# sina-behnam/RTSDS

Measured on AMD Instinct MI355X. Metric: images/sec/node (train step) + inference FPS@1024x512, BiSeNet 19-cls, higher is better.
Workload: dtype bf16; 1 GPU; configs[1]: BiSeNet-R18 seg-only train step (train.py:65-113); model=BiSeNet-ResNet18, global_batch=8, per_gpu_batch=8, image=3x512x1024, num_classes=19, parallelism=dp1

## Files before the change

include/rtsds_hip.h:

```cpp
#ifndef RTSDS_HIP_H
#define RTSDS_HIP_H
#include <stddef.h>
#include <stdint.h>
#ifdef __cplusplus
extern "C" {
#endif

enum { RTSDS_F32 = 0, RTSDS_BF16 = 1, RTSDS_F16 = 2  };
enum {
  RTSDS_OK = 0,
  RTSDS_ERR_SHAPE = 1,
  RTSDS_ERR_UNSUPPORTED = 2,
  RTSDS_ERR_LAUNCH = 3,
  RTSDS_ERR_WORKSPACE = 4
};
enum { RTSDS_ACT_NONE = 0, RTSDS_ACT_RELU = 1, RTSDS_ACT_LEAKY = 2, RTSDS_ACT_SIGMOID = 3 };
#define RTSDS_ACCUMULATE 0x100
#define RTSDS_INPUT_PADDED 0x400
#define RTSDS_WEIGHT_PACKED 0x800

typedef struct {
  int n, h, w, c;
  int ho, wo, k;
  int kh, kw;
  int sh, sw;
  int ph, pw;
  int dh, dw;
  int dtype;
} rtsds_conv_desc;


size_t rtsds_conv2d_fwd_workspace(const rtsds_conv_desc* d);
int rtsds_conv2d_input_pitch(const rtsds_conv_desc* d);
int rtsds_conv2d_fwd_stats_tiles(const rtsds_conv_desc* d);
int rtsds_conv2d_fwd(const rtsds_conv_desc* d, const void* x, const void* w, const float* bias,
                     void* y, int act, float* bn_stats, void* ws, size_t ws_bytes, void* stream);
int rtsds_conv2d_fwd_bn(const rtsds_conv_desc* d, const void* x, const void* w, const float* scale,
                        const float* shift, const void* res, void* y, int act, void* ws, size_t ws_bytes,
                        void* stream);
int rtsds_conv2d_fwd_bn_ld(const rtsds_conv_desc* d, const void* x, const void* w, const float* scale,
                           const float* shift, void* y, long ldy, int act, void* ws, size_t ws_bytes, void* stream);
int rtsds_conv2d_fwd_bn_maxpool(const rtsds_conv_desc* d, const void* x, const void* w, const float* scale,
                                const float* shift, void* y, int act, int hp, int wp, int pool_pad, void* ws,
                                size_t ws_bytes, void* stream);
size_t rtsds_conv2d_dgrad_workspace(const rtsds_conv_desc* d);
size_t rtsds_conv2d_dgrad_pack_bytes(const rtsds_conv_desc* d);
int rtsds_conv2d_dgrad_pack_many(int count, const rtsds_conv_desc* descs, const void* const* w, void* const* wt,
                                 void* stream);
int rtsds_conv2d_dgrad(const rtsds_conv_desc* d, const void* dy, const void* w, void* dx,
                       int accumulate, void* ws, size_t ws_bytes, void* stream);
int rtsds_conv2d_dgrad_act(const rtsds_conv_desc* d, const void* dy, const void* w, void* dx, const void* x_act,
                           int act, void* ws, size_t ws_bytes, void* stream);
int rtsds_conv2d_dgrad_bnstats_tiles(const rtsds_conv_desc* d);
int rtsds_conv2d_dgrad_bnstats(const rtsds_conv_desc* d, const void* dy, const void* w, void* dx, const void* bn_x,
                               const float* gamma, const float* beta, const float* save_mean, const float* save_invstd,
                               int act, float* part, void* ws, size_t ws_bytes, void* stream);
size_t rtsds_conv2d_wgrad_workspace(const rtsds_conv_desc* d);
int rtsds_conv2d_wgrad(const rtsds_conv_desc* d, const void* x, const void* dy, float* dw,
                       float* dbias, int accumulate, void* ws, size_t ws_bytes, void* stream);
typedef struct {
  const float* slab;
  float* dw;
  long slab_stride;
  int nv;
  int cv, cp;
  int splits, accumulate;
} rtsds_split_reduce_desc;
int rtsds_conv2d_wgrad_deferred(const rtsds_conv_desc* d, const void* x, const void* dy, float* dw,
                                float* dbias, int accumulate, void* ws, size_t ws_bytes,
                                rtsds_split_reduce_desc* pending, void* stream);
int rtsds_split_reduce_many(int n, const rtsds_split_reduce_desc* descs, void* stream);
size_t rtsds_imgconv_bn_wgrad_workspace(const rtsds_conv_desc* d);
int rtsds_imgconv_bn_wgrad(const rtsds_conv_desc* d, const void* x, const void* bn_dy, const void* bn_x,
                           const float* coef, int act, float* dw, int accumulate, void* ws, size_t ws_bytes,
                           void* stream);
int rtsds_imgconv_bn_wgrad_deferred(const rtsds_conv_desc* d, const void* x, const void* bn_dy, const void* bn_x,
                                    const float* coef, int act, float* dw, int accumulate, void* ws,
                                    size_t ws_bytes, rtsds_split_reduce_desc* pending, void* stream);

size_t rtsds_bn_workspace(long rows, int c);
int rtsds_bn_fwd(const void* x, const void* res, void* y, long rows, int c, const float* gamma,
                 const float* beta, float* running_mean, float* running_var,
                 long long* num_batches_tracked, float* save_mean,
                 float* save_invstd, float momentum, float eps, int training, int act,
                 const float* stats_part, int stats_nrb, int dtype, void* ws, size_t ws_bytes,
                 void* stream);
int rtsds_bn_fwd_ld(const void* x, const void* res, void* y, long ldy, long rows, int c,
                    const float* gamma, const float* beta, float* running_mean, float* running_var,
                    long long* num_batches_tracked, float* save_mean, float* save_invstd,
                    float momentum, float eps, int training, int act, const float* stats_part,
                    int stats_nrb, int dtype, void* ws, size_t ws_bytes, void* stream);
int rtsds_bn_fold(const float* gamma, const float* beta, const float* running_mean,
                  const float* running_var, const float* conv_bias, float eps, int c, float* scale,
                  float* shift, void* stream);
int rtsds_bn_bwd(const void* dy, const void* x, const void* y, void* dx, void* dres,
                 float* dgamma, float* dbeta, long rows, int c, const float* gamma,
                 const float* beta, const float* save_mean, const float* save_invstd, int training, int act,
                 int accumulate_params, int dtype, void* ws, size_t ws_bytes, void* stream);
int rtsds_bn_bwd_ld(const void* dy, long ldy, const void* x, const void* y, void* dx, void* dres,
                    float* dgamma, float* dbeta, long rows, int c, const float* gamma,
                    const float* beta, const float* save_mean, const float* save_invstd, int training,
                    int act, int accumulate_params, int dtype, void* ws, size_t ws_bytes, void* stream);
int rtsds_bn_bwd_coef(const void* dy, const void* x, float* dgamma, float* dbeta, float* coef, long rows, int c,
                      const float* gamma, const float* beta, const float* save_mean, const float* save_invstd,
                      int training, int act, int accumulate_params, int dtype, void* ws, size_t ws_bytes,
                      void* stream);
int rtsds_bn_bwd_part(const void* dy, const void* x, void* dx, float* dgamma, float* dbeta, long rows, int c,
                      const float* gamma, const float* beta, const float* save_mean, const float* save_invstd,
                      int training, int act, int accumulate_params, const float* part, int nrb, int dtype, void* ws,
                      size_t ws_bytes, void* stream);

int rtsds_bn_relu_maxpool_fwd(const void* x, void* y, uint8_t* idx, int n, int h, int w, int c, int ho, int wo,
                              int p, const float* gamma, const float* beta, float* running_mean,
                              float* running_var, long long* num_batches_tracked, float* save_mean,
                              float* save_invstd, float momentum, float eps, int training,
                              const float* stats_part, int stats_nrb, int dtype, void* ws, size_t ws_bytes,
                              void* stream);
int rtsds_bn_relu_maxpool_bwd(const void* dy_pool, const uint8_t* idx, const void* x, void* dx, float* dgamma,
                              float* dbeta, int n, int h, int w, int c, int ho, int wo, int p,
                              const float* gamma, const float* beta, const float* save_mean,
                              const float* save_invstd, int training, int accumulate_params, int dtype,
                              void* ws, size_t ws_bytes, void* stream);

int rtsds_nchw_to_nhwc(const float* x, void* y, int n, int c, int h, int w, int dtype, void* stream);
int rtsds_nchw_to_nhwc_pad(const float* x, void* y, int n, int c, int h, int w, int pitch, int dtype, void* stream);
int rtsds_cast(const void* src, int src_dtype, void* dst, int dst_dtype, long n, void* stream);
int rtsds_copy_channels(const void* src, int src_ld, int src_off, void* dst, int dst_ld, int dst_off,
                        long rows, int cnt, int accumulate, int dtype, void* stream);

int rtsds_act_fwd(const void* x, void* y, long n, int act, int dtype, void* stream);
int rtsds_act_bwd(const void* dy, const void* y, void* dx, long n, int act, float alpha, int dtype,
                  void* stream);

int rtsds_maxpool_fwd(const void* x, void* y, uint8_t* idx, int n, int h, int w, int c, int ho,
                      int wo, int k, int s, int p, int dtype, void* stream);
int rtsds_maxpool_bwd(const void* dy, const uint8_t* idx, void* dx, int n, int h, int w, int c,
                      int ho, int wo, int k, int s, int p, int dtype, void* stream);
size_t rtsds_gap_workspace(int n, long hw, int c);
int rtsds_gap_fwd(const void* x, void* y, int n, long hw, int c, int dtype, void* ws, size_t ws_bytes,
                  void* stream);
int rtsds_gap_bwd(const void* dy, void* dx, int n, long hw, int c, int accumulate, int dtype, void* stream);

size_t rtsds_ffm_head_eval_workspace(int n, long hw, int c);
int rtsds_ffm_head_eval(const void* f, const void* w1, const float* b1, const void* w2, const float* b2,
                        const void* w3, const float* b3, void* out, int n, long hw, int c, int dtype, void* ws,
                        size_t ws_bytes, void* stream);
int rtsds_chscale_fwd(const void* x, const void* a, void* y, int n, long hw, int c, int mode,
                      int dtype, void* stream);
int rtsds_chscale_bwd(const void* dy, const void* x, const void* a, void* dx, void* da, int n,
                      long hw, int c, int mode, int dtype, void* ws, size_t ws_bytes, void* stream);
int rtsds_chscale2_fwd(const void* x, const void* a, const void* b, void* y, int n, long hw, int c,
                       int dtype, void* stream);
int rtsds_chscale2_bwd(const void* dy, const void* x, const void* a, const void* b, void* dx, void* da,
                       void* db, int n, long hw, int c, int dtype, void* ws, size_t ws_bytes, void* stream);

int rtsds_bilinear_fwd(const void* x, void* y, int n, int hi, int wi, int c, int ho, int wo,
                       float scale_h, float scale_w, int y_ld, int y_off, int dtype, void* stream);
int rtsds_bilinear_fwd_scaled(const void* x, const void* s1, const void* s2, void* y, int n, int hi, int wi,
                              int c, int ho, int wo, float scale_h, float scale_w, int y_ld, int y_off,
                              int dtype, void* stream);
size_t rtsds_bilinear_bwd_workspace(int n, int hi, int wi, int c, int ho, int wo);
int rtsds_bilinear_bwd(const void* dy, void* dx, int n, int hi, int wi, int c, int ho, int wo,
                       float scale_h, float scale_w, int dy_ld, int dy_off, int dtype, void* ws,
                       size_t ws_bytes, void* stream);

int rtsds_adaptive_avgpool_fwd(const void* x, void* y, int n, int hi, int wi, int c, int ho, int wo,
                               int dtype, void* stream);
int rtsds_adaptive_avgpool_bwd(const void* dy, void* dx, int n, int hi, int wi, int c, int ho, int wo,
                               int dtype, void* stream);

int rtsds_softmax_fwd(const void* x, long sn, long sc, long shw, void* y, int y_ld, int n, long hw,
                      int c, int dtype, void* stream);
int rtsds_softmax_bwd(const void* dy, const void* y, int ld, void* dx, long sn, long sc, long shw,
                      int n, long hw, int c, int dtype, void* stream);
size_t rtsds_ce_workspace(void);
int rtsds_ce_finish(const void* ws, float* loss, void* stream);
int rtsds_ce_fwd(const void* x, long sn, long sc, long shw, const int64_t* target, float* loss, int n,
                 long hw, int c, int ignore_index, int dtype, void* ws, size_t ws_bytes, void* stream);
int rtsds_ce_bwd(const void* x, long sn, long sc, long shw, const int64_t* target,
                 const float* grad_loss, const float* count, void* dx, int n, long hw, int c,
                 int ignore_index, int dtype, void* stream);
int rtsds_bce_fwd(const float* x, const float* target, float* loss, int n, void* stream);
int rtsds_bce_bwd(const float* x, const float* target, const float* grad_loss, float* dx, int n,
                  void* stream);

int rtsds_adam_step(float* param, const void* grad, float* exp_avg, float* exp_avg_sq,
                    void* bf16_shadow, long n, float lr, float beta1, float beta2, float eps,
                    float weight_decay, int step, float grad_scale, int grad_dtype, void* stream);

int rtsds_adam_step_dev(float* param, const void* grad, float* exp_avg, float* exp_avg_sq,
                        void* bf16_shadow, long n, const float* hyper, float beta1, float beta2,
                        float eps, float weight_decay, float grad_scale, int grad_dtype, void* stream);

int rtsds_sgd_step(float* param, const void* grad, float* momentum_buf, void* bf16_shadow,
                   long n, const float* hyper, float lr, float momentum, float dampening,
                   float weight_decay, int nesterov, int first, float grad_scale, int grad_dtype, void* stream);

int rtsds_ema_step(float* teacher, const float* student, void* teacher_bf16_shadow, long n, float w,
                   void* stream);
int rtsds_ema_many(int count, float* const* teacher, const float* const* student, const long* numel,
                   float w, void* stream);

int rtsds_argmax(const void* x, long sn, long sc, long shw, int64_t* out, const int64_t* target,
                 unsigned long long* correct, int n, long hw, int c, int dtype, void* stream);
int rtsds_confusion(const int64_t* label, const int64_t* pred, unsigned long long* hist, long total,
                    int nc, void* stream);

#define RTSDS_UPCE_SET_CORRECT 2
size_t rtsds_upce_workspace(int nheads, int n, int hl, int wl, int c, int H, int W, float scale_h,
                            float scale_w);
int rtsds_upce_fwd(int nheads, const void* const* logits, const int64_t* target, int n, int hl,
                   int wl, int c, int H, int W, float scale_h, float scale_w, int ignore_index,
                   float* loss, float* loss_sum, unsigned long long* correct, int want_grad,
                   int dtype, void* ws, size_t ws_bytes, void* stream);
int rtsds_upce_finish(int nheads, const void* ws, float* loss, float* loss_sum, void* stream);
int rtsds_upce_bwd(int nheads, const float* grad_loss, int grad_stride, void* const* dlogits,
                   int n, int hl, int wl, int c, int H, int W, float scale_h, float scale_w,
                   int dtype, const void* ws, size_t ws_bytes, void* stream);

int rtsds_upsoftmax_fwd(const void* x, void* y, int n, int hi, int wi, int c, int ho, int wo,
                        float scale_h, float scale_w, int y_ld, int dtype, void* stream);
size_t rtsds_upsoftmax_bwd_workspace(int n, int hi, int wi, int c, int ho, int wo);
int rtsds_upsoftmax_bwd(const void* dy, int dy_ld, const void* y, int y_ld, void* dx, int n, int hi,
                        int wi, int c, int ho, int wo, float scale_h, float scale_w, int dtype,
                        void* ws, size_t ws_bytes, void* stream);

int rtsds_upsoftmax_acc(const void* x, float* acc, int64_t* pred, int n, int hi, int wi, int c,
                        int ho, int wo, float scale_h, float scale_w, int flip, int accumulate,
                        int dtype, void* stream);

int rtsds_conf_hist(const float* acc, unsigned long long* hist, uint8_t* pred, uint16_t* cbin,
                    long total, int c, int bins, float inv, void* stream);
int rtsds_pseudo_select(const uint8_t* pred, const uint16_t* cbin, const int* tbin, int64_t* out,
                        long total, int c, int ignore_index, void* stream);

int rtsds_upsample_pseudo(const void* x, uint8_t* pred, uint16_t* cbin, const int* tbin, int64_t* labels,
                          int n, int hi, int wi, int c, int ho, int wo, float scale_h, float scale_w,
                          int bins, int ignore_index, int dtype, void* stream);

int rtsds_upsample_paint(const void* x, const uint8_t* frame, const uint8_t* palette, const uint8_t* lut,
                         uint8_t* ids, uint8_t* rgb, int n, int hi, int wi, int c, int ho, int wo,
                         float scale_h, float scale_w, int alpha_q8, int dtype, void* stream);

int rtsds_slide_paint(const void* x, const int* win, int nwin, const uint8_t* frame,
                      const uint8_t* palette, const uint8_t* lut, float* acc, uint8_t* ids,
                      uint8_t* rgb, int nf, int hi, int wi, int c, int hw, int ww, int H, int W,
                      float scale_h, float scale_w, int accumulate, int alpha_q8, int dtype,
                      void* stream);

int rtsds_class_presence(const int64_t* slab, const int* origins, int origin_pitch, unsigned int* present,
                         int n, int hs, int ws, int h, int w, int c, void* stream);
int rtsds_classmix(const void* src, const int64_t* slab, const void* tgt, const uint8_t* pred,
                   const uint16_t* cbin, const int* tbin, const unsigned int* present, const int* perm,
                   int perm_pitch, const int* origins, int origin_pitch, void* out_img, int64_t* out_lab,
                   uint8_t* mask, unsigned int* chosen, int n, int hs, int ws, int h, int w, int c,
                   int pix_bytes, int ignore_index, void* stream);

size_t rtsds_resize_aa_workspace(int c, int h, int w, int ho, int wo);
int rtsds_resize_aa(const void* src, int src_u8, int c, int h, int w, void* dst, int kind, int ho, int wo,
                    int flip, const float* mean, const float* std, int clamp_lo, int clamp_hi, void* ws,
                    size_t ws_bytes, void* stream);
int rtsds_crop_resize_aa(const void* src, int src_u8, int c, int h, int w, int y0, int x0, int hc, int wc,
                         void* dst, int kind, int ho, int wo, int flip, const float* mean, const float* std,
                         int clamp_lo, int clamp_hi, void* ws, size_t ws_bytes, void* stream);
int rtsds_crop_resize_nearest(const void* src, int src_i64, int h, int w, int y0, int x0, int hc, int wc,
                              int64_t* dst, int ho, int wo, int flip, int clamp_lo, int clamp_hi, void* stream);
int rtsds_gaussian_blur(const void* src, int src_u8, float* dst, int c, int h, int w, int kx, int ky,
                        float sigma_x, float sigma_y, void* stream);
int rtsds_gta5_decode(const uint8_t* rgb, int64_t* out, int h, int w, void* stream);
size_t rtsds_color_jitter_workspace(int h, int w);
int rtsds_color_jitter(const void* src, int src_u8, float* dst, int c, int h, int w, const int* order,
                       int mask, float fb, float fc, float fs, float fh, float bound, void* ws,
                       size_t ws_bytes, void* stream);

int rtsds_hist_u8(const uint8_t* img, int c, int h, int w, unsigned int* hist, void* stream);
int rtsds_hist_match(const uint8_t* src, uint8_t* dst, int c, int h, int w, const unsigned int* hist_src,
                     const unsigned int* hist_ref, int strength_q8, uint8_t* lut_out, void* stream);

size_t rtsds_fda_workspace(int h, int w, int b);
int rtsds_fda_spectrum(const uint8_t* img, int c, int h, int w, int b, float* spec, float* amp_norm, void* ws,
                       size_t ws_bytes, void* stream);
int rtsds_fda_apply(const uint8_t* src, void* dst, int dst_u8, int c, int h, int w, int b, const float* spec_src,
                    const float* amp_ref_norm, float strength, void* stream);

int rtsds_graph_split(void* graph, int max_lanes, void** handle, int* n_segments, int* n_lanes);
int rtsds_graph_lanes(void* graph, int max_lanes);
int rtsds_graph_nodes(void* graph);
int rtsds_capture_nodes(void* stream);
int rtsds_graph_split_launch(void* handle, void* stream);
int rtsds_graph_split_destroy(void* handle);

int rtsds_pooled_mlp_bwd(const void* da, const void* a, const void* h, const void* p, const void* w1,
                         const void* w2, float* dw1, float* db1, float* dw2, float* db2, void* dp,
                         int n, int c0, int c1, int c2, int accumulate, int dtype, void* stream);

int rtsds_pooled_mlp_fwd(const void* p, const void* w1, const float* b1, const void* w2, const float* b2, void* h,
                         void* a, int n, int c0, int c1, int c2, int dtype, void* stream);

int rtsds_bn_fwd_gap(const void* x, void* y, float* gap_part, int n, long hw, int c, const float* gamma, const float* beta,
                     float* running_mean, float* running_var, long long* num_batches_tracked, float* save_mean,
                     float* save_invstd, float momentum, float eps, int act, const float* stats_part, int stats_nrb,
                     int dtype, void* ws, size_t ws_bytes, void* stream);
int rtsds_ffm_att_scale(const float* part, const void* f, const void* w1, const float* b1, const void* w2, const float* b2,
                        void* pooled, void* hid, void* att, void* r, int ldr, int n, long hw, int c, int dtype,
                        void* stream);
int rtsds_ffm_att_bwd(const void* dr, const void* f, const void* a, const void* h, const void* p, const void* w1,
                      const void* w2, float* dw1, float* db1, float* dw2, float* db2, void* dp, int n, long hw, int c,
                      int accumulate, int dtype, void* ws, size_t ws_bytes, void* stream);
int rtsds_bn_bwd_ffm(const void* dr, const void* att, const void* dpooled, int n, long hw, const void* x, void* dx,
                     float* dgamma, float* dbeta, int c, const float* gamma, const float* beta, const float* save_mean,
                     const float* save_invstd, int training, int act, int accumulate_params, int dtype, void* ws,
                     size_t ws_bytes, void* stream);

#define RTSDS_ABI_VERSION 23
int rtsds_abi_version(void);

#ifdef __cplusplus
}
#endif
#endif
```

rtsds_amd/_lib.py:

```python
import ctypes
import os

import torch

_HERE = os.path.dirname(os.path.abspath(__file__))
DEFAULT_LIB_PATH = os.path.join(_HERE, "librtsds_hip.so")
ABI_VERSION = 23
LIB_PATH = os.environ.get("RTSDS_LIB") or DEFAULT_LIB_PATH

F32, BF16 = 0, 1
ACT_NONE, ACT_RELU, ACT_LEAKY, ACT_SIGMOID = 0, 1, 2, 3
ACCUMULATE = 0x100
INPUT_PADDED = 0x400
WEIGHT_PACKED = 0x800
UPCE_SET_CORRECT = 2
ERRORS = {1: "bad shape", 2: "unsupported configuration", 3: "HIP launch failure", 4: "workspace too small"}

c_int, c_long, c_float, c_size_t, c_void_p = (ctypes.c_int, ctypes.c_long, ctypes.c_float,
                                              ctypes.c_size_t, ctypes.c_void_p)


class ConvDesc(ctypes.Structure):
    _fields_ = [(n, c_int) for n in ("n", "h", "w", "c", "ho", "wo", "k", "kh", "kw", "sh", "sw",
                                     "ph", "pw", "dh", "dw", "dtype")]


class SplitReduceDesc(ctypes.Structure):
    _fields_ = [("slab", c_void_p), ("dw", c_void_p), ("slab_stride", c_long), ("nv", c_int), ("cv", c_int),
                ("cp", c_int), ("splits", c_int), ("accumulate", c_int)]


P = c_void_p
SIGNATURES = {
    "rtsds_conv2d_fwd_workspace": (c_size_t, [ctypes.POINTER(ConvDesc)]),
    "rtsds_conv2d_input_pitch": (c_int, [ctypes.POINTER(ConvDesc)]),
    "rtsds_conv2d_fwd_stats_tiles": (c_int, [ctypes.POINTER(ConvDesc)]),
    "rtsds_conv2d_fwd": (c_int, [ctypes.POINTER(ConvDesc), P, P, P, P, c_int, P, P, c_size_t, P]),
    "rtsds_conv2d_fwd_bn": (c_int, [ctypes.POINTER(ConvDesc), P, P, P, P, P, P, c_int, P, c_size_t, P]),
    "rtsds_conv2d_fwd_bn_ld": (c_int, [ctypes.POINTER(ConvDesc), P, P, P, P, P, c_long, c_int, P, c_size_t, P]),
    "rtsds_conv2d_fwd_bn_maxpool": (c_int, [ctypes.POINTER(ConvDesc), P, P, P, P, P, c_int, c_int, c_int, c_int, P,
                                            c_size_t, P]),
    "rtsds_conv2d_dgrad_workspace": (c_size_t, [ctypes.POINTER(ConvDesc)]),
    "rtsds_conv2d_dgrad_pack_bytes": (c_size_t, [ctypes.POINTER(ConvDesc)]),
    "rtsds_conv2d_dgrad_pack_many": (c_int, [c_int, ctypes.POINTER(ConvDesc), P, P, P]),
    "rtsds_conv2d_dgrad": (c_int, [ctypes.POINTER(ConvDesc), P, P, P, c_int, P, c_size_t, P]),
    "rtsds_conv2d_dgrad_act": (c_int, [ctypes.POINTER(ConvDesc), P, P, P, P, c_int, P, c_size_t, P]),
    "rtsds_conv2d_dgrad_bnstats_tiles": (c_int, [ctypes.POINTER(ConvDesc)]),
    "rtsds_conv2d_dgrad_bnstats": (c_int, [ctypes.POINTER(ConvDesc), P, P, P, P, P, P, P, P, c_int, P, P, c_size_t, P]),
    "rtsds_conv2d_wgrad_workspace": (c_size_t, [ctypes.POINTER(ConvDesc)]),
    "rtsds_conv2d_wgrad": (c_int, [ctypes.POINTER(ConvDesc), P, P, P, P, c_int, P, c_size_t, P]),
    "rtsds_conv2d_wgrad_deferred": (c_int, [ctypes.POINTER(ConvDesc), P, P, P, P, c_int, P, c_size_t,
                                            ctypes.POINTER(SplitReduceDesc), P]),
    "rtsds_split_reduce_many": (c_int, [c_int, ctypes.POINTER(SplitReduceDesc), P]),
    "rtsds_imgconv_bn_wgrad_workspace": (c_size_t, [ctypes.POINTER(ConvDesc)]),
    "rtsds_imgconv_bn_wgrad": (c_int, [ctypes.POINTER(ConvDesc), P, P, P, P, c_int, P, c_int, P, c_size_t, P]),
    "rtsds_imgconv_bn_wgrad_deferred": (c_int, [ctypes.POINTER(ConvDesc), P, P, P, P, c_int, P, c_int, P, c_size_t,
                                                ctypes.POINTER(SplitReduceDesc), P]),
    "rtsds_bn_workspace": (c_size_t, [c_long, c_int]),
    "rtsds_bn_bwd_coef": (c_int, [P, P, P, P, P, c_long, c_int, P, P, P, P, c_int, c_int, c_int, c_int, P, c_size_t, P]),
    "rtsds_bn_fwd": (c_int, [P, P, P, c_long, c_int, P, P, P, P, P, P, P, c_float, c_float, c_int,
                             c_int, P, c_int, c_int, P, c_size_t, P]),
    "rtsds_bn_fwd_ld": (c_int, [P, P, P, c_long, c_long, c_int, P, P, P, P, P, P, P, c_float, c_float, c_int,
                                c_int, P, c_int, c_int, P, c_size_t, P]),
    "rtsds_bn_fold": (c_int, [P, P, P, P, P, c_float, c_int, P, P, P]),
    "rtsds_pooled_mlp_fwd": (c_int, [P, P, P, P, P, P, P, c_int, c_int, c_int, c_int, c_int, P]),
    "rtsds_pooled_mlp_bwd": (c_int, [P, P, P, P, P, P, P, P, P, P, P, c_int, c_int, c_int, c_int, c_int, c_int, P]),
    "rtsds_bn_fwd_gap": (c_int, [P, P, P, c_int, c_long, c_int, P, P, P, P, P, P, P, c_float, c_float, c_int, P, c_int,
                                 c_int, P, c_size_t, P]),
    "rtsds_ffm_att_scale": (c_int, [P] * 10 + [c_int, c_int, c_long, c_int, c_int, P]),
    "rtsds_ffm_att_bwd": (c_int, [P] * 12 + [c_int, c_long, c_int, c_int, c_int, P, c_size_t, P]),
    "rtsds_bn_bwd_ffm": (c_int, [P, P, P, c_int, c_long, P, P, P, P, c_int, P, P, P, P, c_int, c_int, c_int, c_int,
                                 P, c_size_t, P]),
    "rtsds_bn_bwd_part": (c_int, [P, P, P, P, P, c_long, c_int, P, P, P, P, c_int, c_int, c_int, P, c_int, c_int, P,
                                  c_size_t, P]),
    "rtsds_bn_bwd": (c_int, [P, P, P, P, P, P, P, c_long, c_int, P, P, P, P, c_int, c_int, c_int, c_int,
                             P, c_size_t, P]),
    "rtsds_bn_bwd_ld": (c_int, [P, c_long, P, P, P, P, P, P, c_long, c_int, P, P, P, P, c_int, c_int, c_int, c_int,
                                P, c_size_t, P]),
    "rtsds_bn_relu_maxpool_fwd": (c_int, [P, P, P] + [c_int] * 7 + [P, P, P, P, P, P, P, c_float, c_float, c_int, P,
                                                                   c_int, c_int, P, c_size_t, P]),
    "rtsds_bn_relu_maxpool_bwd": (c_int, [P, P, P, P, P, P] + [c_int] * 7 + [P, P, P, P, c_int, c_int, c_int, P,
                                                                            c_size_t, P]),
    "rtsds_nchw_to_nhwc": (c_int, [P, P, c_int, c_int, c_int, c_int, c_int, P]),
    "rtsds_nchw_to_nhwc_pad": (c_int, [P, P, c_int, c_int, c_int, c_int, c_int, c_int, P]),
    "rtsds_cast": (c_int, [P, c_int, P, c_int, c_long, P]),
    "rtsds_ffm_head_eval_workspace": (c_size_t, [c_int, c_long, c_int]),
    "rtsds_ffm_head_eval": (c_int, [P, P, P, P, P, P, P, P, c_int, c_long, c_int, c_int, P, c_size_t, P]),
    "rtsds_graph_split": (c_int, [P, c_int, P, P, P]),
    "rtsds_graph_split_launch": (c_int, [P, P]),
    "rtsds_graph_lanes": (c_int, [P, c_int]),
    "rtsds_graph_nodes": (c_int, [P]),
    "rtsds_abi_version": (c_int, []),
    "rtsds_capture_nodes": (c_int, [P]),
    "rtsds_graph_split_destroy": (c_int, [P]),
    "rtsds_copy_channels": (c_int, [P, c_int, c_int, P, c_int, c_int, c_long, c_int, c_int, c_int, P]),
    "rtsds_act_fwd": (c_int, [P, P, c_long, c_int, c_int, P]),
    "rtsds_act_bwd": (c_int, [P, P, P, c_long, c_int, c_float, c_int, P]),
    "rtsds_maxpool_fwd": (c_int, [P, P, P] + [c_int] * 10 + [P]),
    "rtsds_maxpool_bwd": (c_int, [P, P, P] + [c_int] * 10 + [P]),
    "rtsds_gap_workspace": (c_size_t, [c_int, c_long, c_int]),
    "rtsds_gap_fwd": (c_int, [P, P, c_int, c_long, c_int, c_int, P, c_size_t, P]),
    "rtsds_gap_bwd": (c_int, [P, P, c_int, c_long, c_int, c_int, c_int, P]),
    "rtsds_chscale_fwd": (c_int, [P, P, P, c_int, c_long, c_int, c_int, c_int, P]),
    "rtsds_chscale_bwd": (c_int, [P, P, P, P, P, c_int, c_long, c_int, c_int, c_int, P, c_size_t, P]),
    "rtsds_chscale2_fwd": (c_int, [P, P, P, P, c_int, c_long, c_int, c_int, P]),
    "rtsds_chscale2_bwd": (c_int, [P, P, P, P, P, P, P, c_int, c_long, c_int, c_int, P, c_size_t, P]),
    "rtsds_bilinear_fwd": (c_int, [P, P] + [c_int] * 6 + [c_float, c_float, c_int, c_int, c_int, P]),
    "rtsds_bilinear_fwd_scaled": (c_int, [P, P, P, P] + [c_int] * 6 + [c_float, c_float, c_int, c_int, c_int, P]),
    "rtsds_bilinear_bwd_workspace": (c_size_t, [c_int] * 6),
    "rtsds_bilinear_bwd": (c_int, [P, P] + [c_int] * 6 + [c_float, c_float, c_int, c_int, c_int, P, c_size_t, P]),
    "rtsds_softmax_fwd": (c_int, [P, c_long, c_long, c_long, P, c_int, c_int, c_long, c_int, c_int, P]),
    "rtsds_softmax_bwd": (c_int, [P, P, c_int, P, c_long, c_long, c_long, c_int, c_long, c_int, c_int,
                                  P]),
    "rtsds_ce_workspace": (c_size_t, []),
    "rtsds_ce_fwd": (c_int, [P, c_long, c_long, c_long, P, P, c_int, c_long, c_int, c_int, c_int, P,
                             c_size_t, P]),
    "rtsds_ce_bwd": (c_int, [P, c_long, c_long, c_long, P, P, P, P, c_int, c_long, c_int, c_int, c_int,
                             P]),
    "rtsds_bce_fwd": (c_int, [P, P, P, c_int, P]),
    "rtsds_bce_bwd": (c_int, [P, P, P, P, c_int, P]),
    "rtsds_adam_step_dev": (c_int, [P, P, P, P, P, c_long, P, c_float, c_float, c_float, c_float, c_float, c_int, P]),
    "rtsds_upsoftmax_fwd": (c_int, [P, P, c_int, c_int, c_int, c_int, c_int, c_int, c_float, c_float, c_int, c_int, P]),
    "rtsds_upsoftmax_bwd_workspace": (c_size_t, [c_int, c_int, c_int, c_int, c_int, c_int]),
    "rtsds_upsoftmax_bwd": (c_int, [P, c_int, P, c_int, P, c_int, c_int, c_int, c_int, c_int, c_int, c_float, c_float,
                                    c_int, P, c_size_t, P]),
    "rtsds_upsoftmax_acc": (c_int, [P, P, P, c_int, c_int, c_int, c_int, c_int, c_int, c_float, c_float, c_int, c_int,
                                    c_int, P]),
    "rtsds_conf_hist": (c_int, [P, P, P, P, c_long, c_int, c_int, c_float, P]),
    "rtsds_pseudo_select": (c_int, [P, P, P, P, c_long, c_int, c_int, P]),
    "rtsds_upsample_pseudo": (c_int, [P, P, P, P, P] + [c_int] * 6 + [c_float, c_float, c_int, c_int, c_int, P]),
    "rtsds_upsample_paint": (c_int, [P, P, P, P, P, P] + [c_int] * 6 + [c_float, c_float, c_int, c_int, P]),
    "rtsds_slide_paint": (c_int, [P, ctypes.POINTER(c_int), c_int, P, P, P, P, P, P] + [c_int] * 8 +
                          [c_float, c_float, c_int, c_int, c_int, P]),
    "rtsds_ema_step": (c_int, [P, P, P, c_long, c_float, P]),
    "rtsds_ema_many": (c_int, [c_int, P, P, P, c_float, P]),
    "rtsds_class_presence": (c_int, [P, P, c_int, P, c_int, c_int, c_int, c_int, c_int, c_int, P]),
    "rtsds_classmix": (c_int, [P, P, P, P, P, P, P, P, c_int, P, c_int, P, P, P, P] + [c_int] * 8 + [P]),
    "rtsds_resize_aa_workspace": (c_size_t, [c_int, c_int, c_int, c_int, c_int]),
    "rtsds_resize_aa": (c_int, [P, c_int, c_int, c_int, c_int, P, c_int, c_int, c_int, c_int, P, P, c_int, c_int,
                                P, c_size_t, P]),
    "rtsds_crop_resize_aa": (c_int, [P] + [c_int] * 8 + [P, c_int, c_int, c_int, c_int, P, P, c_int, c_int,
                                     P, c_size_t, P]),
    "rtsds_crop_resize_nearest": (c_int, [P] + [c_int] * 7 + [P, c_int, c_int, c_int, c_int, c_int, P]),
    "rtsds_gaussian_blur": (c_int, [P, c_int, P, c_int, c_int, c_int, c_int, c_int, c_float, c_float, P]),
    "rtsds_gta5_decode": (c_int, [P, P, c_int, c_int, P]),
    "rtsds_color_jitter_workspace": (c_size_t, [c_int, c_int]),
    "rtsds_color_jitter": (c_int, [P, c_int, P, c_int, c_int, c_int, ctypes.POINTER(c_int), c_int, c_float, c_float,
                                   c_float, c_float, c_float, P, c_size_t, P]),
    "rtsds_hist_u8": (c_int, [P, c_int, c_int, c_int, P, P]),
    "rtsds_hist_match": (c_int, [P, P, c_int, c_int, c_int, P, P, c_int, P, P]),
    "rtsds_fda_workspace": (c_size_t, [c_int, c_int, c_int]),
    "rtsds_fda_spectrum": (c_int, [P, c_int, c_int, c_int, c_int, P, P, P, c_size_t, P]),
    "rtsds_fda_apply": (c_int, [P, P, c_int, c_int, c_int, c_int, c_int, P, P, c_float, P]),
    "rtsds_sgd_step": (c_int, [P, P, P, P, c_long, P, c_float, c_float, c_float, c_float, c_int, c_int,
                               c_float, c_int, P]),
    "rtsds_adam_step": (c_int, [P, P, P, P, P, c_long, c_float, c_float, c_float, c_float, c_float,
                                c_int, c_float, c_int, P]),
    "rtsds_argmax": (c_int, [P, c_long, c_long, c_long, P, P, P, c_int, c_long, c_int, c_int, P]),
    "rtsds_confusion": (c_int, [P, P, P, c_long, c_int, P]),
    "rtsds_adaptive_avgpool_fwd": (c_int, [P, P, c_int, c_int, c_int, c_int, c_int, c_int, c_int, P]),
    "rtsds_adaptive_avgpool_bwd": (c_int, [P, P, c_int, c_int, c_int, c_int, c_int, c_int, c_int, P]),
    "rtsds_upce_finish": (c_int, [c_int, P, P, P, P]),
    "rtsds_ce_finish": (c_int, [P, P, P]),
    "rtsds_upce_workspace": (c_size_t, [c_int, c_int, c_int, c_int, c_int, c_int, c_int, c_float, c_float]),
    "rtsds_upce_fwd": (c_int, [c_int, P, P, c_int, c_int, c_int, c_int, c_int, c_int, c_float, c_float,
                               c_int, P, P, P, c_int, c_int, P, c_size_t, P]),
    "rtsds_upce_bwd": (c_int, [c_int, P, c_int, P, c_int, c_int, c_int, c_int, c_int, c_int, c_float, c_float,
                               c_int, P, c_size_t, P]),
}

_lib = None


def load(path=LIB_PATH):
    global _lib
    if _lib is None:
        if not os.path.exists(path):
            raise RuntimeError(f"rtsds_amd: HIP library not built ({path}); run __graft_entry__.build()")
        lib = ctypes.CDLL(path)
        ver = getattr(lib, "rtsds_abi_version", None)
        if ver is None:
            raise RuntimeError(f"rtsds_amd: {path} predates the ABI version check; rebuild it")
        ver.restype, ver.argtypes = ctypes.c_int, []
        if ver() != ABI_VERSION:
            raise RuntimeError(f"rtsds_amd: {path} has ABI revision {ver()}, this package needs {ABI_VERSION}")
        for name, (res, args) in SIGNATURES.items():
            fn = getattr(lib, name)
            fn.restype, fn.argtypes = res, args
        _lib = lib
    return _lib


class _Lib:
    def __getattr__(self, name):
        fn = getattr(load(), name)

        def call(*args):
            rc = fn(*args)
            if name.endswith(("_workspace", "_tiles", "_pitch", "_bytes")):
                return rc
            if rc != 0:
                raise RuntimeError(f"rtsds_amd: {name} failed: {ERRORS.get(rc, rc)}")
            return rc
        return call


lib = _Lib()
```

rtsds_amd/csrc/bn.hip:

```cpp
#include "bn_dev.h"
#include "chan_dev.h"
#include <type_traits>
#include <algorithm>

static const int kBnMaxRB = 2048;
static const int kBnTinyRows = 64;

template <int VEC> struct BnLayout {
  int tpr, rpi;
  __host__ __device__ BnLayout(int c) {
    tpr = (c + VEC - 1) / VEC;
    if (tpr > 256) tpr = 256;
    rpi = 256 / tpr;
  }
};
template <int VEC> struct BnTile : BnLayout<VEC> {
  int cl, cv, rg, ch0, cvalid;
  bool col, active;
  RT_DEV static int block_channels(int c) { return min(c - (int)blockIdx.y * 256 * VEC, 256 * VEC); }
  RT_DEV BnTile(int c) : BnLayout<VEC>(block_channels(c)) {
    cl = block_channels(c);
    cv = threadIdx.x % this->tpr;
    rg = threadIdx.x / this->tpr;
    ch0 = blockIdx.y * 256 * VEC + cv * VEC;
    cvalid = c - ch0;
    col = cv * VEC < cl;
    active = rg < this->rpi && col;
  }
  RT_DEV long row0() const { return (long)blockIdx.x * this->rpi + rg; }
  RT_DEV long step() const { return (long)gridDim.x * this->rpi; }
};

RT_DEV void bn_coef(float g, float b, float m, float inv, float& sc, float& sh) {
  sc = g * inv;
  sh = fmaf(-m, sc, b);
}

RT_DEV void chan_merge(float& na, float& ma, float& Ma, float nb, float mb, float Mb) {
  if (nb == 0.f) return;
  if (na == 0.f) { na = nb; ma = mb; Ma = Mb; return; }
  const float n = na + nb, d = mb - ma;
  ma += d * (nb / n);
  Ma += Mb + d * d * (na * nb / n);
  na = n;
}

template <typename T, int VEC>
__global__ void __launch_bounds__(256) bn_stats_kernel(const T* __restrict__ x, float* __restrict__ part, long rows, int c) {
  __shared__ float sh[3][256][VEC];
  const BnTile<VEC> t(c);
  const int tid = threadIdx.x, ch0 = t.ch0;
  float cnt = 0.f, shift[VEC], s1[VEC], s2[VEC];
#pragma unroll
  for (int j = 0; j < VEC; ++j) { shift[j] = 0.f; s1[j] = 0.f; s2[j] = 0.f; }
  if (t.active) {
    long r = t.row0();
    const long step = t.step();
    if (r < rows) {
      load_vec<T, VEC>(x + r * c + ch0, shift, t.cvalid);
      cnt = 1.f;
      r += step;
    }
    for (; r < rows; r += step) {
      float v[VEC];
      load_vec<T, VEC>(x + r * c + ch0, v, t.cvalid);
#pragma unroll
      for (int j = 0; j < VEC; ++j) {
        const float d = v[j] - shift[j];
        s1[j] += d;
        s2[j] = fmaf(d, d, s2[j]);
      }
      cnt += 1.f;
    }
  }
#pragma unroll
  for (int j = 0; j < VEC; ++j) {
    const float mean = cnt > 0.f ? shift[j] + s1[j] / cnt : 0.f;
    const float m2 = cnt > 0.f ? s2[j] - s1[j] * s1[j] / cnt : 0.f;
    sh[0][tid][j] = cnt;
    sh[1][tid][j] = mean;
    sh[2][tid][j] = fmaxf(m2, 0.f);
  }
  __syncthreads();
  if (t.rg == 0 && t.col) {
#pragma unroll
    for (int j = 0; j < VEC; ++j) {
      float n = sh[0][tid][j], m = sh[1][tid][j], M = sh[2][tid][j];
      for (int g = 1; g < t.rpi; ++g) {
        const int o = g * t.tpr + t.cv;
        chan_merge(n, m, M, sh[0][o][j], sh[1][o][j], sh[2][o][j]);
      }
      if (ch0 + j < c) {
        *(f32x4*)(part + ((long)(ch0 + j) * gridDim.x + blockIdx.x) * 4) = f32x4{n, m, M, 0.f};
      }
    }
  }
}


RT_DEV void chan_merge_shfl(float& n, float& m, float& M) {
#pragma unroll
  for (int o = 32; o > 0; o >>= 1) {
    const float nb = __shfl_xor(n, o, 64), mb = __shfl_xor(m, o, 64), Mb = __shfl_xor(M, o, 64);
    chan_merge(n, m, M, nb, mb, Mb);
  }
}
RT_DEV bool bn_finalize_body(const float* __restrict__ part, int nrb, int c, long rows, const float* gamma, const float* beta,
                             float* rmean, float* rvar, float* smean, float* sinv, float* scale, float* shift, float momentum,
                             float eps, long long* nbt, float (*wr)[3], float& sc_out, float& sh_out) {
  const int ch = blockIdx.x, lane = threadIdx.x & 63, wave = threadIdx.x >> 6;
  if (nbt && ch == 0 && threadIdx.x == 0) *nbt += 1;
  float g0 = 1.f, b0 = 0.f, rm0 = 0.f, rv0 = 0.f;
  if (threadIdx.x == 0) {
    if (gamma) g0 = gamma[ch];
    if (beta) b0 = beta[ch];
    if (rmean) rm0 = rmean[ch];
    if (rvar) rv0 = rvar[ch];
  }
  float n = 0.f, m = 0.f, M = 0.f;
  for (int b0 = threadIdx.x; b0 < nrb; b0 += 256 * 8) {
    float pn[8], pm[8], pM[8];
#pragma unroll
    for (int u = 0; u < 8; ++u) {
      const int b = min(b0 + 256 * u, nrb - 1);
      const f32x4 p = *(const f32x4*)(part + ((long)ch * nrb + b) * 4);
      pn[u] = b0 + 256 * u < nrb ? p[0] : 0.f;
      pm[u] = p[1];
      pM[u] = p[2];
    }
#pragma unroll
    for (int u = 0; u < 8; ++u) chan_merge(n, m, M, pn[u], pm[u], pM[u]);
  }
  chan_merge_shfl(n, m, M);
  if (lane == 0) { wr[wave][0] = n; wr[wave][1] = m; wr[wave][2] = M; }
  __syncthreads();
  if (threadIdx.x != 0) return false;
  n = wr[0][0]; m = wr[0][1]; M = wr[0][2];
  for (int w = 1; w < 4; ++w) chan_merge(n, m, M, wr[w][0], wr[w][1], wr[w][2]);
  const float var = M / (float)rows;
  const float inv = 1.0f / sqrtf(var + eps);
  smean[ch] = m;
  sinv[ch] = inv;
  if (rmean) rmean[ch] = (1.f - momentum) * rm0 + momentum * m;
  if (rvar) {
    const float unb = rows > 1 ? M / (float)(rows - 1) : var;
    rvar[ch] = (1.f - momentum) * rv0 + momentum * unb;
  }
  bn_coef(g0, b0, m, inv, sc_out, sh_out);
  scale[ch] = sc_out;
  shift[ch] = sh_out;
  return true;
}
__global__ void __launch_bounds__(256) bn_finalize_kernel(const float* __restrict__ part, int nrb, int c, long rows, const float* gamma,
                                   const float* beta, float* rmean, float* rvar, float* smean, float* sinv,
                                   float* scale, float* shift, float momentum, float eps, long long* nbt) {
  __shared__ float wr[4][3];
  float sc, sh;
  bn_finalize_body(part, nrb, c, rows, gamma, beta, rmean, rvar, smean, sinv, scale, shift, momentum, eps, nbt, wr, sc, sh);
}
__global__ void bn_eval_coef_kernel(int c, const float* gamma, const float* beta, const float* rmean, const float* rvar,
                                    float* scale, float* shift, float* smean, float* sinv, float eps) {
  const int ch = blockIdx.x * blockDim.x + threadIdx.x;
  if (ch >= c) return;
  const float inv = 1.0f / sqrtf(rvar[ch] + eps);
  if (smean) smean[ch] = rmean[ch];
  if (sinv) sinv[ch] = inv;
  const float g = gamma ? gamma[ch] : 1.f, b = beta ? beta[ch] : 0.f;
  bn_coef(g, b, rmean[ch], inv, scale[ch], shift[ch]);
}

RT_DEV float act_f(float v, int act) {
  if (act == RTSDS_ACT_RELU) return fmaxf(v, 0.f);
  if (act == RTSDS_ACT_LEAKY) return v > 0.f ? v : 0.2f * v;
  if (act == RTSDS_ACT_SIGMOID) return 1.f / (1.f + expf(-v));
  return v;
}
template <int VEC>
RT_DEV void load_coef(const float* __restrict__ p, int ch0, int c, float* v) {
  if constexpr (VEC % 4 == 0) {
#pragma unroll
    for (int q = 0; q < VEC / 4; ++q) {
      const f32x4 t = *(const f32x4*)(p + ch0 + 4 * q);
#pragma unroll
      for (int e = 0; e < 4; ++e) v[4 * q + e] = t[e];
    }
  } else {
#pragma unroll
    for (int j = 0; j < VEC; ++j) v[j] = p[min(ch0 + j, c - 1)];
  }
}

template <typename T>
__global__ void __launch_bounds__(256) bn_finalize_apply_kernel(const float* __restrict__ part, int nrb, int c, long rows,
                                                                 const float* gamma, const float* beta, float* rmean, float* rvar,
                                                                 float* smean, float* sinv, float* scale, float* shift,
                                                                 float momentum, float eps, long long* nbt, const T* __restrict__ x,
                                                                 const T* __restrict__ res, T* __restrict__ y, long ldy, int act) {
  __shared__ float wr[4][3];
  __shared__ float cs[2];
  float sc, sh;
  if (bn_finalize_body(part, nrb, c, rows, gamma, beta, rmean, rvar, smean, sinv, scale, shift, momentum, eps, nbt, wr, sc, sh)) {
    cs[0] = sc;
    cs[1] = sh;
  }
  __syncthreads();
  const int ch = blockIdx.x;
  for (long r = threadIdx.x; r < rows; r += 256) {
    float a = fmaf(to_f(x[r * c + ch]), cs[0], cs[1]);
    if (res) a += to_f(res[r * c + ch]);
    y[r * ldy + ch] = from_f<T>(act_f(a, act));
  }
}

template <typename T, int VEC, int ACT>
__global__ void __launch_bounds__(256) bn_apply_kernel(const T* __restrict__ x, const T* __restrict__ res, T* __restrict__ y,
                                                        const float* __restrict__ scale, const float* __restrict__ shift,
                                                        long rows, int c, int act_rt, long ldy) {
  const int act = ACT >= 0 ? ACT : act_rt;
  const BnTile<VEC> t(c);
  if (!t.active) return;
  float sc[VEC], sh[VEC];
  load_coef<VEC>(scale, t.ch0, c, sc);
  load_coef<VEC>(shift, t.ch0, c, sh);
  const int ch0 = t.ch0, cvalid = t.cvalid;
  const long step = t.step();
  long r = t.row0();
  for (; r + step < rows; r += 2 * step) {
    float v0[VEC], v1[VEC], r0[VEC], r1[VEC];
    load_vec<T, VEC>(x + r * c + ch0, v0, cvalid);
    load_vec<T, VEC>(x + (r + step) * c + ch0, v1, cvalid);
    if (res) {
      load_vec<T, VEC>(res + r * c + ch0, r0, cvalid);
      load_vec<T, VEC>(res + (r + step) * c + ch0, r1, cvalid);
    }
#pragma unroll
    for (int j = 0; j < VEC; ++j) {
      float a = fmaf(v0[j], sc[j], sh[j]), b = fmaf(v1[j], sc[j], sh[j]);
      if (res) { a += r0[j]; b += r1[j]; }
      v0[j] = act_f(a, act);
      v1[j] = act_f(b, act);
    }
    store_vec<T, VEC>(y + r * ldy + ch0, v0, cvalid);
    store_vec<T, VEC>(y + (r + step) * ldy + ch0, v1, cvalid);
  }
  if (r < rows) {
    float v0[VEC], r0[VEC];
    load_vec<T, VEC>(x + r * c + ch0, v0, cvalid);
    if (res) load_vec<T, VEC>(res + r * c + ch0, r0, cvalid);
#pragma unroll
    for (int j = 0; j < VEC; ++j) {
      float a = fmaf(v0[j], sc[j], sh[j]);
      if (res) a += r0[j];
      v0[j] = act_f(a, act);
    }
    store_vec<T, VEC>(y + r * ldy + ch0, v0, cvalid);
  }
}

template <typename T>
struct BnApplyLoad {
  const T* x;
  T* y;
  float sc, sh;
  int act;
  RT_DEV float at(long o) const {
    const T v = from_f<T>(act_f(fmaf(to_f(x[o]), sc, sh), act));
    y[o] = v;
    return to_f(v);
  }
};
template <typename T>
__global__ void __launch_bounds__(256) bn_apply_gap_kernel(const T* __restrict__ x, T* __restrict__ y, const float* __restrict__ scale,
                                                            const float* __restrict__ shift, float* __restrict__ part, long hw, int c,
                                                            int act) {
  __shared__ float red[256];
  const int ch = threadIdx.x % c;
  chan_part_body<T, 1, false>(BnApplyLoad<T>{x, y, scale[ch], shift[ch], act}, (const T*)nullptr, part, hw, c, red);
}

template <typename T>
struct GradDirect {
  static constexpr bool kDirect = true;
  const T* dy;
  int c;
  template <int VEC> RT_DEV void load(long r, int ch0, float* g, int cvalid) const { load_vec<T, VEC>(dy + r * c + ch0, g, cvalid); }
};
template <typename T>
struct GradPool {
  static constexpr bool kDirect = false;
  const T* dyp;
  const uint8_t* idx;
  int c, h, w, ho, wo, p;
  FastDiv f_w, f_h;
  template <int VEC> RT_DEV void load(long r, int ch0, float* g, int cvalid) const {
    static_assert(VEC == 8 && sizeof(T) == 2, "pooled gradient source: bf16 vectors of 8 channels");
    typedef typename VecT<T>::v16 V16;
    const uint32_t q = fdiv((uint32_t)r, f_w), img = fdiv(q, f_h);
    const int iw = (int)((uint32_t)r - q * w), ih = (int)(q - img * h);
    const int oh_lo = max(0, (ih + p - 1) / 2), ow_lo = max(0, (iw + p - 1) / 2);
    V16 gv[4];
    unsigned long long ib[4];
#pragma unroll
    for (int t = 0; t < 4; ++t) {
      const int oh = min(oh_lo + (t >> 1), ho - 1), ow = min(ow_lo + (t & 1), wo - 1);
      const long o = (((long)img * ho + oh) * wo + ow) * c + ch0;
      gv[t] = *(const V16*)(dyp + o);
      ib[t] = *(const unsigned long long*)(idx + o);
    }
#pragma unroll
    for (int j = 0; j < VEC; ++j) g[j] = 0.f;
#pragma unroll
    for (int t = 0; t < 4; ++t) {
      const int oh = oh_lo + (t >> 1), ow = ow_lo + (t & 1);
      const int a = ih - (oh * 2 - p), b = iw - (ow * 2 - p);
      if (oh >= ho || ow >= wo || a < 0 || a >= 3 || b < 0 || b >= 3) continue;
      const unsigned want = (unsigned)(a * 3 + b);
#pragma unroll
      for (int j = 0; j < VEC; ++j)
        if (((ib[t] >> (8 * j)) & 0xff) == want) g[j] += to_f(gv[t][j]);
    }
  }
};

template <typename T>
struct GradScalePool {
  static constexpr bool kDirect = false;
  const T *dr, *att, *dp;
  int c;
  long hw;
  float inv;
  template <int VEC> RT_DEV void load(long r, int ch0, float* g, int cvalid) const {
    static_assert(VEC == 1, "scale + pool gradient source: narrow class maps, one channel per thread");
    if (cvalid <= 0) { g[0] = 0.f; return; }
    const long v = (r / hw) * c + ch0;
    const T s = from_f<T>(to_f(dr[r * c + ch0]) * (to_f(att[v]) + 1.f));
    const T p = from_f<T>(to_f(dp[v]) * inv);
    g[0] = to_f(from_f<T>(to_f(s) + to_f(p)));
  }
};

template <int VEC>
RT_DEV void bn_bwd_coef(int ch0, int c, const float* gamma, const float* beta, const float* mean, const float* sinv,
                        BnDx<VEC>& k) {
#pragma unroll
  for (int j = 0; j < VEC; ++j) {
    const int ch = min(ch0 + j, c - 1);
    k.mu[j] = mean[ch];
    bn_coef(gamma ? gamma[ch] : 1.f, beta ? beta[ch] : 0.f, k.mu[j], sinv[ch], k.sc[j], k.sh[j]);
  }
}

constexpr int kBnU = 2;
template <typename T, int VEC, bool HAS_Y, class GS>
RT_DEV void bn_bwd_sums(const GS& gs, const T* __restrict__ x, const T* __restrict__ y, T* __restrict__ gout, long r0,
                        long step, long rows, int c, const BnTile<VEC>& t, const BnDx<VEC>& k, int act, float* sg,
                        float* sgx, float (*g_last)[VEC], float (*xv_last)[VEC]) {
  const int ch0 = t.ch0;
  for (long r = r0; r < rows; r += kBnU * step) {
    float g[kBnU][VEC], xv[kBnU][VEC], yv[HAS_Y ? kBnU : 1][VEC];
#pragma unroll
    for (int u = 0; u < kBnU; ++u) {
      const long rr = min(r + u * step, rows - 1);
      gs.template load<VEC>(rr, ch0, g[u], t.cvalid);
      load_vec<T, VEC>(x + rr * c + ch0, xv[u], t.cvalid);
      if constexpr (HAS_Y) load_vec<T, VEC>(y + rr * c + ch0, yv[u], t.cvalid);
    }
#pragma unroll
    for (int u = 0; u < kBnU; ++u)
      if (r + u * step >= rows) {
#pragma unroll
        for (int j = 0; j < VEC; ++j) g[u][j] = 0.f;
      }
#pragma unroll
    for (int u = 0; u < kBnU; ++u) {
      bn_mask<VEC, HAS_Y>(g[u], yv[HAS_Y ? u : 0], xv[u], k.sc, k.sh, act);
      if (HAS_Y && gout && r + u * step < rows) store_vec<T, VEC>(gout + (r + u * step) * c + ch0, g[u], t.cvalid);
#pragma unroll
      for (int j = 0; j < VEC; ++j) {
        sg[j] += g[u][j];
        sgx[j] = fmaf(g[u][j], xv[u][j] - k.mu[j], sgx[j]);
        if (g_last) { g_last[u][j] = g[u][j]; xv_last[u][j] = xv[u][j]; }
      }
    }
  }
}

template <int VEC>
RT_DEV bool bn_bwd_block_sum(const BnTile<VEC>& t, float (*red)[256][VEC], float* sg, float* sgx) {
  const int tid = threadIdx.x;
  if ((t.tpr & (t.tpr - 1)) == 0 && t.tpr <= 64) {
    const int lane = tid & 63, wave = tid >> 6;
    for (int o = t.tpr; o < 64; o <<= 1) {
#pragma unroll
      for (int j = 0; j < VEC; ++j) {
        sg[j] += __shfl_xor(sg[j], o, 64);
        sgx[j] += __shfl_xor(sgx[j], o, 64);
      }
    }
    if (lane < t.tpr) {
#pragma unroll
      for (int j = 0; j < VEC; ++j) { red[0][wave * 64 + lane][j] = sg[j]; red[1][wave * 64 + lane][j] = sgx[j]; }
    }
    __syncthreads();
    if (tid >= t.tpr || tid * VEC >= t.cl) return false;
#pragma unroll
    for (int j = 0; j < VEC; ++j) {
      sg[j] = (red[0][tid][j] + red[0][64 + tid][j]) + (red[0][128 + tid][j] + red[0][192 + tid][j]);
      sgx[j] = (red[1][tid][j] + red[1][64 + tid][j]) + (red[1][128 + tid][j] + red[1][192 + tid][j]);
    }
    return true;
  }
#pragma unroll
  for (int j = 0; j < VEC; ++j) { red[0][tid][j] = sg[j]; red[1][tid][j] = sgx[j]; }
  __syncthreads();
  if (t.rg != 0 || !t.col) return false;
#pragma unroll
  for (int j = 0; j < VEC; ++j) {
    float a = red[0][tid][j], b = red[1][tid][j];
    for (int gi = 1; gi < t.rpi; ++gi) {
      a += red[0][gi * t.tpr + t.cv][j];
      b += red[1][gi * t.tpr + t.cv][j];
    }
    sg[j] = a;
    sgx[j] = b;
  }
  return true;
}

struct BnBwdOps {
  float inv = 0.f, g = 1.f, bt = 0.f, mu = 0.f, dg0 = 0.f, db0 = 0.f;
};
RT_DEV BnBwdOps bn_bwd_ops(int ch, const float* gamma, const float* beta, const float* smean, const float* sinv,
                           const float* dgamma, const float* dbeta, int accumulate) {
  BnBwdOps o;
  o.inv = sinv[ch];
  o.mu = smean[ch];
  if (gamma) o.g = gamma[ch];
  if (beta) o.bt = beta[ch];
  if (accumulate && dgamma) o.dg0 = dgamma[ch];
  if (accumulate && dbeta) o.db0 = dbeta[ch];
  return o;
}
RT_DEV void bn_bwd_tail(const BnBwdOps& o, float sg, float sgx, int ch, long rows, int training, int accumulate,
                        float* dgamma, float* dbeta, float& A, float& B, float& C) {
  const float inv = o.inv;
  if (dgamma) dgamma[ch] = accumulate ? o.dg0 + sgx * inv : sgx * inv;
  if (dbeta) dbeta[ch] = accumulate ? o.db0 + sg : sg;
  const float a = o.g * inv;
  const float invn = 1.f / (float)rows;
  A = a;
  B = training ? -a * inv * inv * sgx * invn : 0.f;
  C = training ? -a * sg * invn : 0.f;
}
RT_DEV void bn_bwd_coef_rows(const BnBwdOps& o, float sg, float sgx, int ch, int c, long rows, int training, int accumulate,
                             float* dgamma, float* dbeta, float* coef) {
  bn_bwd_tail(o, sg, sgx, ch, rows, training, accumulate, dgamma, dbeta, coef[ch], coef[c + ch], coef[2 * c + ch]);
  coef[3 * c + ch] = o.mu;
  bn_coef(o.g, o.bt, o.mu, o.inv, coef[4 * c + ch], coef[5 * c + ch]);
}

template <typename T, int VEC>
RT_DEV void bn_bwd_row_store(T* __restrict__ dx, T* __restrict__ dres, long off, const BnDx<VEC>& k, int cvalid, const float* g,
                             float* xv) {
#pragma unroll
  for (int j = 0; j < VEC; ++j) xv[j] = bn_bwd_dx<VEC>(k, j, g[j], xv[j]);
  if (dx) store_vec<T, VEC>(dx + off, xv, cvalid);
  if (dres) store_vec<T, VEC>(dres + off, g, cvalid);
}
template <typename T, int VEC, class GS>
RT_DEV void bn_bwd_row(const GS& gs, const T* __restrict__ x, const T* __restrict__ y, T* __restrict__ dx, T* __restrict__ dres,
                       long r, int c, const BnTile<VEC>& t, const BnDx<VEC>& k, int act) {
  const long off = r * c + t.ch0;
  float g[VEC], xv[VEC];
  gs.template load<VEC>(r, t.ch0, g, t.cvalid);
  load_vec<T, VEC>(x + off, xv, t.cvalid);
  bn_row_mask<T, VEC>(g, y ? y + off : nullptr, xv, k, act, t.cvalid);
  bn_bwd_row_store<T, VEC>(dx, dres, off, k, t.cvalid, g, xv);
}

template <typename T, int VEC, bool HAS_Y, class GS, int ACT>
__global__ void __launch_bounds__(256) bn_bwd_stats_kernel(const GS gs, const T* __restrict__ x,
                                                            const T* __restrict__ y, const float* __restrict__ gamma,
                                                            const float* __restrict__ beta, const float* __restrict__ mean,
                                                            const float* __restrict__ sinv, float* __restrict__ part,
                                                            long rows, int c, int act_rt, T* __restrict__ gout) {
  const int act = ACT >= 0 ? ACT : act_rt;
  __shared__ float red[2][256][VEC];
  const BnTile<VEC> t(c);
  BnDx<VEC> k;
  float sg[VEC], sgx[VEC];
#pragma unroll
  for (int j = 0; j < VEC; ++j) { sg[j] = 0.f; sgx[j] = 0.f; }
  if (t.active) {
    bn_bwd_coef<VEC>(t.ch0, c, gamma, beta, mean, sinv, k);
    bn_bwd_sums<T, VEC, HAS_Y>(gs, x, y, gout, t.row0(), t.step(), rows, c, t, k, act, sg, sgx, nullptr, nullptr);
  }
  if (!bn_bwd_block_sum<VEC>(t, red, sg, sgx)) return;
#pragma unroll
  for (int j = 0; j < VEC; ++j)
    if (t.ch0 + j < c) *(float2*)(part + ((long)blockIdx.x * c + t.ch0 + j) * 2) = make_float2(sg[j], sgx[j]);
}

template <typename T, int VEC, bool HAS_Y, class GS, int ACT>
__global__ void __launch_bounds__(256) bn_bwd_tiny_kernel(const GS gs, const T* __restrict__ x, const T* __restrict__ y,
                                                           const float* __restrict__ gamma, const float* __restrict__ beta,
                                                           const float* __restrict__ mean, const float* __restrict__ sinv,
                                                           float* __restrict__ dgamma, float* __restrict__ dbeta, T* __restrict__ dx,
                                                           T* __restrict__ dres, long rows, int c, int act_rt, int training,
                                                           int accumulate) {
  const int act = ACT >= 0 ? ACT : act_rt;
  __shared__ float red[2][256][VEC];
  __shared__ float cf[3][256 * VEC];
  const BnTile<VEC> t(c);
  const bool one_pass = rows <= kBnU * (long)t.rpi;
  BnDx<VEC> k;
  float sg[VEC], sgx[VEC], g[kBnU][VEC], xv[kBnU][VEC];
  BnBwdOps ops[VEC];
#pragma unroll
  for (int j = 0; j < VEC; ++j) {
    sg[j] = 0.f;
    sgx[j] = 0.f;
    ops[j] = bn_bwd_ops(min(t.ch0 + j, c - 1), gamma, beta, mean, sinv, dgamma, dbeta, accumulate);
  }
  if (t.active) {
    bn_bwd_coef<VEC>(t.ch0, c, gamma, beta, mean, sinv, k);
    bn_bwd_sums<T, VEC, HAS_Y>(gs, x, y, (T*)nullptr, t.rg, t.rpi, rows, c, t, k, act, sg, sgx, g, xv);
  }
  if (bn_bwd_block_sum<VEC>(t, red, sg, sgx)) {
#pragma unroll
    for (int j = 0; j < VEC; ++j) {
      const int ch = t.ch0 + j, o = t.cv * VEC + j;
      if (ch >= c) continue;
      bn_bwd_tail(ops[j], 0.f + sg[j], 0.f + sgx[j], ch, rows, training, accumulate, dgamma, dbeta, cf[0][o], cf[1][o],
                  cf[2][o]);
    }
  }
  __syncthreads();
  if (!t.active || (!dx && !dres)) return;
#pragma unroll
  for (int j = 0; j < VEC; ++j) {
    k.a[j] = cf[0][t.cv * VEC + j];
    k.b[j] = cf[1][t.cv * VEC + j];
    k.k[j] = cf[2][t.cv * VEC + j];
  }
  if (one_pass) {
#pragma unroll
    for (int u = 0; u < kBnU; ++u) {
      const long r = t.rg + u * (long)t.rpi, off = r * c + t.ch0;
      if (r < rows) bn_bwd_row_store<T, VEC>(dx, dres, off, k, t.cvalid, g[u], xv[u]);
    }
    return;
  }
  for (long r = t.rg; r < rows; r += t.rpi) bn_bwd_row<T, VEC>(gs, x, HAS_Y ? y : (const T*)nullptr, dx, dres, r, c, t, k, act);
}

__global__ void __launch_bounds__(256) bn_bwd_finalize_kernel(const float* __restrict__ part, int nrb, int c, long rows, const float* gamma,
                                       const float* beta, const float* smean, const float* sinv, float* dgamma, float* dbeta,
                                       float* coef, int training, int accumulate) {
  __shared__ float wr[4][2];
  const int ch = blockIdx.x, lane = threadIdx.x & 63, wave = threadIdx.x >> 6;
  BnBwdOps ops;
  if (threadIdx.x == 0) ops = bn_bwd_ops(ch, gamma, beta, smean, sinv, dgamma, dbeta, accumulate);
  float sg = 0.f, sgx = 0.f;
  for (int b0 = threadIdx.x; b0 < nrb; b0 += 256 * 8) {
    float pg[8], px[8];
#pragma unroll
    for (int u = 0; u < 8; ++u) {
      const int b = min(b0 + 256 * u, nrb - 1);
      const bool ok = b0 + 256 * u < nrb;
      const float2 pr = *(const float2*)(part + ((long)ch * nrb + b) * 2);
      const float g = pr.x, gx = pr.y;
      pg[u] = ok ? g : 0.f;
      px[u] = ok ? gx : 0.f;
    }
#pragma unroll
    for (int u = 0; u < 8; ++u) { sg += pg[u]; sgx += px[u]; }
  }
  sg = wave_sum(sg);
  sgx = wave_sum(sgx);
  if (lane == 0) { wr[wave][0] = sg; wr[wave][1] = sgx; }
  __syncthreads();
  if (threadIdx.x != 0) return;
  sg = (wr[0][0] + wr[1][0]) + (wr[2][0] + wr[3][0]);
  sgx = (wr[0][1] + wr[1][1]) + (wr[2][1] + wr[3][1]);
  bn_bwd_coef_rows(ops, sg, sgx, ch, c, rows, training, accumulate, dgamma, dbeta, coef);
}

__global__ void __launch_bounds__(256) bn_bwd_finalize_rb_kernel(const float* __restrict__ part, int nrb, int c, long rows,
                                                                  const float* gamma, const float* beta, const float* smean,
                                                                  const float* sinv, float* dgamma, float* dbeta, float* coef,
                                                                  int training, int accumulate) {
  __shared__ float wr[16][16][2];
  const int cl = threadIdx.x & 15, q = threadIdx.x >> 4, ch = blockIdx.x * 16 + cl;
  const int chc = min(ch, c - 1);
  BnBwdOps ops;
  if (q == 0) ops = bn_bwd_ops(chc, gamma, beta, smean, sinv, dgamma, dbeta, accumulate);
  float sg = 0.f, sgx = 0.f;
  for (int b0 = q; b0 < nrb; b0 += 16 * 8) {
    float2 pv[8];
#pragma unroll
    for (int u = 0; u < 8; ++u) {
      const int b = min(b0 + 16 * u, nrb - 1);
      pv[u] = *(const float2*)(part + ((long)b * c + chc) * 2);
    }
#pragma unroll
    for (int u = 0; u < 8; ++u)
      if (b0 + 16 * u < nrb) { sg += pv[u].x; sgx += pv[u].y; }
  }
  wr[q][cl][0] = sg;
  wr[q][cl][1] = sgx;
  __syncthreads();
  if (q != 0 || ch >= c) return;
  float t0[8], t1[8];
#pragma unroll
  for (int i = 0; i < 8; ++i) { t0[i] = wr[2 * i][cl][0] + wr[2 * i + 1][cl][0]; t1[i] = wr[2 * i][cl][1] + wr[2 * i + 1][cl][1]; }
#pragma unroll
  for (int i = 0; i < 4; ++i) { t0[i] = t0[2 * i] + t0[2 * i + 1]; t1[i] = t1[2 * i] + t1[2 * i + 1]; }
  sg = (t0[0] + t0[1]) + (t0[2] + t0[3]);
  sgx = (t1[0] + t1[1]) + (t1[2] + t1[3]);
  bn_bwd_coef_rows(ops, sg, sgx, ch, c, rows, training, accumulate, dgamma, dbeta, coef);
}

template <typename T, int VEC, class GS, int ACT>
__global__ void __launch_bounds__(256) bn_bwd_apply_kernel(const GS gs, const T* __restrict__ x,
                                                            const T* __restrict__ y, T* __restrict__ dx, T* __restrict__ dres,
                                                            const float* __restrict__ coef, long rows, int c, int act_rt) {
  const int act = ACT >= 0 ? ACT : act_rt;
  const BnTile<VEC> t(c);
  if (!t.active) return;
  BnDx<VEC> k;
  load_coef<VEC>(coef, t.ch0, c, k.a);
  load_coef<VEC>(coef + c, t.ch0, c, k.b);
  load_coef<VEC>(coef + 2 * c, t.ch0, c, k.k);
  load_coef<VEC>(coef + 3 * c, t.ch0, c, k.mu);
  if (act && !y) {
    load_coef<VEC>(coef + 4 * c, t.ch0, c, k.sc);
    load_coef<VEC>(coef + 5 * c, t.ch0, c, k.sh);
  }
  const long step = t.step();
  long r = t.row0();
  const int ch0 = t.ch0, cvalid = t.cvalid;
  for (; r + step < rows; r += 2 * step) {
    const long o0 = r * c + ch0, o1 = o0 + step * c;
    float g0[VEC], x0[VEC], g1[VEC], x1[VEC];
    gs.template load<VEC>(r, ch0, g0, cvalid);
    load_vec<T, VEC>(x + o0, x0, cvalid);
    gs.template load<VEC>(r + step, ch0, g1, cvalid);
    load_vec<T, VEC>(x + o1, x1, cvalid);
    bn_row_mask<T, VEC>(g0, y ? y + o0 : nullptr, x0, k, act, cvalid);
    bn_row_mask<T, VEC>(g1, y ? y + o1 : nullptr, x1, k, act, cvalid);
#pragma unroll
    for (int j = 0; j < VEC; ++j) {
      x0[j] = bn_bwd_dx<VEC>(k, j, g0[j], x0[j]);
      x1[j] = bn_bwd_dx<VEC>(k, j, g1[j], x1[j]);
    }
    if (dx) {
      store_vec<T, VEC>(dx + o0, x0, cvalid);
      store_vec<T, VEC>(dx + o1, x1, cvalid);
    }
    if (dres) {
      store_vec<T, VEC>(dres + o0, g0, cvalid);
      store_vec<T, VEC>(dres + o1, g1, cvalid);
    }
  }
  if (r < rows) bn_bwd_row<T, VEC>(gs, x, y, dx, dres, r, c, t, k, act);
}

template <typename F>
static void with_act(int act, F f) {
  if (act == RTSDS_ACT_NONE) f(std::integral_constant<int, RTSDS_ACT_NONE>());
  else if (act == RTSDS_ACT_RELU) f(std::integral_constant<int, RTSDS_ACT_RELU>());
  else f(std::integral_constant<int, -1>());
}
template <typename T_, int VEC_> struct BnKind {
  typedef T_ T;
  static constexpr int VEC = VEC_;
};
template <typename F>
static int bn_dispatch(int dtype, int c, F f) {
  if (dtype == RTSDS_BF16) {
    if (c % 8 == 0) f(BnKind<bf16, 8>());
    else f(BnKind<bf16, 1>());
  } else if (dtype == RTSDS_F32) {
    if (c % 4 == 0) f(BnKind<float, 4>());
    else f(BnKind<float, 1>());
  } else return RTSDS_ERR_UNSUPPORTED;
  return RTSDS_OK;
}

template <int VEC>
static long bn_need(long rows, int c) {
  const BnLayout<VEC> L(c);
  return (rows + L.rpi - 1) / L.rpi;
}
template <int VEC>
static int bn_rb(long rows, int c) {
  const long need = bn_need<VEC>(rows, c);
  long rb = std::min<long>(need, kBnMaxRB);
  rb = std::max<long>(1, std::min<long>(rb, (need + 7) / 8));
  return (int)rb;
}
static constexpr auto kBnApplyMaxRB = (1L << 24);
template <int VEC>
static int bn_apply_rb(long rows, int c) {
  const long need = bn_need<VEC>(rows, c);
  return (int)std::max<long>(1, std::min<long>((need + 1) / 2, kBnApplyMaxRB));
}
static constexpr auto kBnBwdRBMax = 512;
static constexpr auto kBnBwdRBDiv = 8;
template <int VEC>
static int bn_bwd_rb(long rows, int c) {
  const long need = bn_need<VEC>(rows, c);
  long rb = std::min<long>(need, kBnBwdRBMax);
  rb = std::max<long>(1, std::min<long>(rb, (need + kBnBwdRBDiv - 1) / kBnBwdRBDiv));
  return (int)rb;
}
template <int VEC>
static dim3 bn_grid(int rb, int c) { return dim3(rb, rt_cdiv(c, 256 * VEC)); }

static size_t bn_part_floats(long rows, int c) { return (size_t)bn_rb<1>(rows, c) * c * 4; }

static size_t al64f(size_t n) { return (n + 63) & ~(size_t)63; }
struct BnWs {
  float *part, *coef;
};
static BnWs bn_ws(void* ws, long rows, int c) {
  BnWs w;
  w.part = (float*)ws;
  w.coef = w.part + al64f(bn_part_floats(rows, c));
  return w;
}
extern "C" size_t rtsds_bn_workspace(long rows, int c) {
  if (rows <= 0 || c <= 0) return 256;
  return (al64f(bn_part_floats(rows, c)) + al64f((size_t)c * 8)) * 4 + 256;
}

struct BnArgs {
  long rows = 0;
  int c = 0, training = 0, act = 0, accumulate = 0;
  const void *x = nullptr, *res = nullptr, *dy = nullptr, *ykept = nullptr;
  void *y = nullptr, *dx = nullptr, *dres = nullptr;
  long ldy = 0;
  const float *gamma = nullptr, *beta = nullptr;
  float *rmean = nullptr, *rvar = nullptr, *dgamma = nullptr, *dbeta = nullptr;
  float *smean = nullptr, *sinv = nullptr;
  long long* nbt = nullptr;
  float momentum = 0.f, eps = 0.f;
  const float* pre = nullptr;
  int pre_nrb = 0;
  bool coef_only = false;
  BnWs w = {nullptr, nullptr};
  hipStream_t st = nullptr;
  BnArgs(long rows_, int c_, void* ws, void* stream)
      : rows(rows_), c(c_), w(bn_ws(ws, rows_, c_)), st((hipStream_t)stream) {}
  void affine(const float* g, const float* b, const float* sm, const float* si) {
    gamma = g, beta = b, smean = const_cast<float*>(sm), sinv = const_cast<float*>(si);
  }
};

template <typename T, int VEC>
static void bn_fwd_coefs(const BnArgs& a, bool apply_too = false) {
  const int c = a.c;
  float *scale = a.w.coef, *shift = a.w.coef + c;
  if (!a.training) {
    hipLaunchKernelGGL(bn_eval_coef_kernel, dim3(rt_cdiv(c, 256)), dim3(256), 0, a.st, c, a.gamma, a.beta, a.rmean, a.rvar, scale,
                       shift, a.smean, a.sinv, a.eps);
    return;
  }
  int rb = a.pre_nrb;
  const float* part = a.pre;
  if (!part) {
    rb = bn_rb<VEC>(a.rows, c);
    hipLaunchKernelGGL((bn_stats_kernel<T, VEC>), bn_grid<VEC>(rb, c), dim3(256), 0, a.st, (const T*)a.x, a.w.part, a.rows, c);
    part = a.w.part;
  }
  if (apply_too)
    hipLaunchKernelGGL(bn_finalize_apply_kernel<T>, dim3(c), dim3(256), 0, a.st, part, rb, c, a.rows, a.gamma, a.beta, a.rmean,
                       a.rvar, a.smean, a.sinv, scale, shift, a.momentum, a.eps, a.nbt, (const T*)a.x, (const T*)a.res, (T*)a.y,
                       a.ldy, a.act);
  else
    hipLaunchKernelGGL(bn_finalize_kernel, dim3(c), dim3(256), 0, a.st, part, rb, c, a.rows, a.gamma, a.beta, a.rmean, a.rvar,
                       a.smean, a.sinv, scale, shift, a.momentum, a.eps, a.nbt);
}
template <typename T, int VEC>
static void bn_fwd_launch(const BnArgs& a) {
  const bool tiny = a.training && a.rows <= kBnTinyRows;
  bn_fwd_coefs<T, VEC>(a, tiny);
  if (tiny) return;
  with_act(a.act, [&](auto av) {
    hipLaunchKernelGGL((bn_apply_kernel<T, VEC, decltype(av)::value>), bn_grid<VEC>(bn_apply_rb<VEC>(a.rows, a.c), a.c), dim3(256),
                       0, a.st, (const T*)a.x, (const T*)a.res, (T*)a.y, a.w.coef, a.w.coef + a.c, a.rows, a.c, a.act, a.ldy);
  });
}
static int bn_fwd_args(BnArgs& a, const float* gamma, const float* beta, float* running_mean, float* running_var,
                       long long* num_batches_tracked, float* save_mean, float* save_invstd, float momentum, float eps,
                       int training, const float* stats_part, int stats_nrb) {
  if (!training && (!running_mean || !running_var)) return RTSDS_ERR_UNSUPPORTED;
  if (training && (!save_mean || !save_invstd)) return RTSDS_ERR_UNSUPPORTED;
  a.affine(gamma, beta, save_mean, save_invstd);
  a.rmean = running_mean, a.rvar = running_var, a.nbt = training ? num_batches_tracked : nullptr;
  a.momentum = momentum, a.eps = eps, a.training = training;
  a.pre = stats_part, a.pre_nrb = stats_nrb;
  return RTSDS_OK;
}

extern "C" int rtsds_bn_fwd_ld(const void* x, const void* res, void* y, long ldy, long rows, int c, const float* gamma,
                               const float* beta, float* running_mean, float* running_var, long long* num_batches_tracked,
                               float* save_mean, float* save_invstd, float momentum, float eps, int training, int act,
                               const float* stats_part, int stats_nrb, int dtype, void* ws, size_t ws_bytes, void* stream) {
  if (rows <= 0 || c <= 0 || ldy < c) return RTSDS_ERR_SHAPE;
  if (ldy != c && !(dtype == RTSDS_BF16 && c % 8 == 0 && ldy % 8 == 0)) return RTSDS_ERR_UNSUPPORTED;
  if (ws_bytes < rtsds_bn_workspace(rows, c)) return RTSDS_ERR_WORKSPACE;
  BnArgs a(rows, c, ws, stream);
  if (int rc = bn_fwd_args(a, gamma, beta, running_mean, running_var, num_batches_tracked, save_mean, save_invstd, momentum, eps,
                           training, stats_part, stats_nrb))
    return rc;
  if (c > 65535 * 256) return RTSDS_ERR_UNSUPPORTED;
  a.x = x, a.res = res, a.y = y, a.ldy = ldy, a.act = act;
  if (int rc = bn_dispatch(dtype, c, [&](auto k) { bn_fwd_launch<typename decltype(k)::T, decltype(k)::VEC>(a); })) return rc;
  RET_LAUNCH();
}

extern "C" int rtsds_bn_fwd(const void* x, const void* res, void* y, long rows, int c, const float* gamma, const float* beta,
                            float* running_mean, float* running_var, long long* num_batches_tracked, float* save_mean,
                            float* save_invstd, float momentum,
                            float eps, int training, int act, const float* stats_part, int stats_nrb, int dtype, void* ws,
                            size_t ws_bytes, void* stream) {
  return rtsds_bn_fwd_ld(x, res, y, c, rows, c, gamma, beta, running_mean, running_var, num_batches_tracked, save_mean,
                         save_invstd, momentum, eps, training, act, stats_part, stats_nrb, dtype, ws, ws_bytes, stream);
}

template <typename T, int VEC, class GS>
static void bn_bwd_launch(const GS& gs, const BnArgs& a) {
  const T *x = (const T*)a.x, *y = (const T*)a.ykept;
  T *dx = (T*)a.dx, *dres = (T*)a.dres;
  const long rows = a.rows;
  const int c = a.c, act = a.act;
  const int rb = a.pre ? a.pre_nrb : bn_bwd_rb<VEC>(rows, c);
  const bool g_out = !a.pre && y && act == RTSDS_ACT_RELU && dres && dx && GS::kDirect;
  if (!a.pre && rb == 1 && GS::kDirect && !g_out && !a.coef_only) {
    with_bool(y && act, [&](auto hy) {
      with_act(act, [&](auto av) {
        hipLaunchKernelGGL((bn_bwd_tiny_kernel<T, VEC, decltype(hy)::value, GS, decltype(av)::value>), bn_grid<VEC>(1, c), dim3(256),
                           0, a.st, gs, x, y, a.gamma, a.beta, a.smean, a.sinv, a.dgamma, a.dbeta, dx, dres, rows, c, act,
                           a.training, a.accumulate);
      });
    });
    return;
  }
  if (a.pre)
    hipLaunchKernelGGL(bn_bwd_finalize_kernel, dim3(c), dim3(256), 0, a.st, a.pre, rb, c, rows, a.gamma, a.beta, a.smean, a.sinv,
                       a.dgamma, a.dbeta, a.w.coef, a.training, a.accumulate);
  else {
    with_bool(y && act, [&](auto hy) {
      with_act(act, [&](auto av) {
        hipLaunchKernelGGL((bn_bwd_stats_kernel<T, VEC, decltype(hy)::value, GS, decltype(av)::value>), bn_grid<VEC>(rb, c), dim3(256),
                           0, a.st, gs, x, y, a.gamma, a.beta, a.smean, a.sinv, a.w.part, rows, c, act,
                           g_out ? dres : (T*)nullptr);
      });
    });
    hipLaunchKernelGGL(bn_bwd_finalize_rb_kernel, dim3(rt_cdiv(c, 16)), dim3(256), 0, a.st, a.w.part, rb, c, rows, a.gamma, a.beta,
                       a.smean, a.sinv, a.dgamma, a.dbeta, a.w.coef, a.training, a.accumulate);
  }
  const dim3 grid = bn_grid<VEC>(bn_apply_rb<VEC>(rows, c), c);
  if (g_out) {
    const GradDirect<T> gg{dres, c};
    hipLaunchKernelGGL((bn_bwd_apply_kernel<T, VEC, GradDirect<T>, RTSDS_ACT_NONE>), grid, dim3(256), 0, a.st, gg, x,
                       (const T*)nullptr, dx, (T*)nullptr, a.w.coef, rows, c, 0);
  } else if (dx || dres) {
    with_act(act, [&](auto av) {
      hipLaunchKernelGGL((bn_bwd_apply_kernel<T, VEC, GS, decltype(av)::value>), grid, dim3(256), 0, a.st, gs, x, y, dx, dres,
                         a.w.coef, rows, c, act);
    });
  }
}
template <typename T, int VEC>
static void bn_bwd_launch(const BnArgs& a) {
  const GradDirect<T> gs{(const T*)a.dy, (int)(a.ldy ? a.ldy : a.c)};
  bn_bwd_launch<T, VEC, GradDirect<T>>(gs, a);
}
static void bn_bwd_args(BnArgs& a, const void* x, void* dx, float* dgamma, float* dbeta, const float* gamma, const float* beta,
                        const float* save_mean, const float* save_invstd, int training, int act, int accumulate) {
  a.affine(gamma, beta, save_mean, save_invstd);
  a.x = x, a.dx = dx, a.dgamma = dgamma, a.dbeta = dbeta;
  a.training = training, a.act = act, a.accumulate = accumulate;
}

extern "C" int rtsds_bn_bwd_part(const void* dy, const void* x, void* dx, float* dgamma, float* dbeta, long rows, int c,
                                 const float* gamma, const float* beta, const float* save_mean, const float* save_invstd,
                                 int training, int act, int accumulate_params, const float* part, int nrb, int dtype, void* ws,
                                 size_t ws_bytes, void* stream) {
  if (rows <= 0 || c <= 0 || nrb <= 0 || !part) return RTSDS_ERR_SHAPE;
  if (ws_bytes < rtsds_bn_workspace(rows, c)) return RTSDS_ERR_WORKSPACE;
  if (dtype != RTSDS_BF16 || c % 8 != 0) return RTSDS_ERR_UNSUPPORTED;
  if (!(act == RTSDS_ACT_NONE || act == RTSDS_ACT_RELU || act == RTSDS_ACT_LEAKY)) return RTSDS_ERR_UNSUPPORTED;
  BnArgs a(rows, c, ws, stream);
  bn_bwd_args(a, x, dx, dgamma, dbeta, gamma, beta, save_mean, save_invstd, training, act, accumulate_params);
  a.dy = dy, a.pre = part, a.pre_nrb = nrb;
  bn_bwd_launch<bf16, 8>(a);
  RET_LAUNCH();
}

extern "C" int rtsds_bn_bwd_ld(const void* dy, long ldy, const void* x, const void* y, void* dx, void* dres, float* dgamma,
                               float* dbeta, long rows, int c, const float* gamma, const float* beta, const float* save_mean,
                               const float* save_invstd, int training, int act, int accumulate_params, int dtype, void* ws,
                               size_t ws_bytes, void* stream) {
  if (rows <= 0 || c <= 0 || ldy < c || ldy > (1L << 30)) return RTSDS_ERR_SHAPE;
  if (ldy != c && !(dtype == RTSDS_BF16 && c % 8 == 0 && ldy % 8 == 0)) return RTSDS_ERR_UNSUPPORTED;
  if (ws_bytes < rtsds_bn_workspace(rows, c)) return RTSDS_ERR_WORKSPACE;
  if (!y && !(act == RTSDS_ACT_NONE || act == RTSDS_ACT_RELU || act == RTSDS_ACT_LEAKY)) return RTSDS_ERR_UNSUPPORTED;
  if (!y && act && dres) return RTSDS_ERR_UNSUPPORTED;
  BnArgs a(rows, c, ws, stream);
  bn_bwd_args(a, x, dx, dgamma, dbeta, gamma, beta, save_mean, save_invstd, training, act, accumulate_params);
  a.dy = dy, a.ldy = ldy, a.ykept = y, a.dres = dres;
  if (int rc = bn_dispatch(dtype, c, [&](auto k) { bn_bwd_launch<typename decltype(k)::T, decltype(k)::VEC>(a); })) return rc;
  RET_LAUNCH();
}
extern "C" int rtsds_bn_bwd_coef(const void* dy, const void* x, float* dgamma, float* dbeta, float* coef, long rows, int c,
                                 const float* gamma, const float* beta, const float* save_mean, const float* save_invstd,
                                 int training, int act, int accumulate_params, int dtype, void* ws, size_t ws_bytes,
                                 void* stream) {
  if (rows <= 0 || c <= 0 || !coef || ((size_t)coef & 15)) return RTSDS_ERR_SHAPE;
  if (ws_bytes < rtsds_bn_workspace(rows, c)) return RTSDS_ERR_WORKSPACE;
  if (!(act == RTSDS_ACT_NONE || act == RTSDS_ACT_RELU || act == RTSDS_ACT_LEAKY)) return RTSDS_ERR_UNSUPPORTED;
  BnArgs a(rows, c, ws, stream);
  bn_bwd_args(a, x, nullptr, dgamma, dbeta, gamma, beta, save_mean, save_invstd, training, act, accumulate_params);
  a.dy = dy, a.w.coef = coef, a.coef_only = true;
  if (int rc = bn_dispatch(dtype, c, [&](auto k) { bn_bwd_launch<typename decltype(k)::T, decltype(k)::VEC>(a); })) return rc;
  RET_LAUNCH();
}
extern "C" int rtsds_bn_bwd(const void* dy, const void* x, const void* y, void* dx, void* dres, float* dgamma, float* dbeta,
                            long rows, int c, const float* gamma, const float* beta, const float* save_mean,
                            const float* save_invstd, int training, int act, int accumulate_params, int dtype, void* ws,
                            size_t ws_bytes, void* stream) {
  return rtsds_bn_bwd_ld(dy, c, x, y, dx, dres, dgamma, dbeta, rows, c, gamma, beta, save_mean, save_invstd, training, act,
                         accumulate_params, dtype, ws, ws_bytes, stream);
}

extern "C" int rtsds_bn_fwd_gap(const void* x, void* y, float* gap_part, int n, long hw, int c, const float* gamma, const float* beta,
                                float* running_mean, float* running_var, long long* num_batches_tracked, float* save_mean,
                                float* save_invstd, float momentum, float eps, int act, const float* stats_part, int stats_nrb,
                                int dtype, void* ws, size_t ws_bytes, void* stream) {
  if (n <= 0 || n > 65535 || hw <= 0 || c <= 0 || !x || !y || !gap_part) return RTSDS_ERR_SHAPE;
  const long rows = (long)n * hw;
  if (c > 256 || c % (dtype == RTSDS_BF16 ? 8 : 4) == 0) return RTSDS_ERR_UNSUPPORTED;
  if (ws_bytes < rtsds_bn_workspace(rows, c)) return RTSDS_ERR_WORKSPACE;
  BnArgs a(rows, c, ws, stream);
  if (int rc = bn_fwd_args(a, gamma, beta, running_mean, running_var, num_batches_tracked, save_mean, save_invstd, momentum, eps,
                           1, stats_part, stats_nrb))
    return rc;
  a.x = x, a.y = y, a.ldy = c, a.act = act;
  DISPATCH_T(dtype, {
    bn_fwd_coefs<T, 1>(a);
    hipLaunchKernelGGL(bn_apply_gap_kernel<T>, dim3(chan_slices(n, hw), n, 1), dim3(256), 0, a.st, (const T*)x, (T*)y, a.w.coef,
                       a.w.coef + c, gap_part, hw, c, act);
  });
  RET_LAUNCH();
}
extern "C" int rtsds_bn_bwd_ffm(const void* dr, const void* att, const void* dpooled, int n, long hw, const void* x, void* dx,
                                float* dgamma, float* dbeta, int c, const float* gamma, const float* beta, const float* save_mean,
                                const float* save_invstd, int training, int act, int accumulate_params, int dtype, void* ws,
                                size_t ws_bytes, void* stream) {
  if (n <= 0 || hw <= 0 || c <= 0 || !dr || !att || !dpooled || !x) return RTSDS_ERR_SHAPE;
  const long rows = (long)n * hw;
  if (c % (dtype == RTSDS_BF16 ? 8 : 4) == 0) return RTSDS_ERR_UNSUPPORTED;
  if (!(act == RTSDS_ACT_NONE || act == RTSDS_ACT_RELU || act == RTSDS_ACT_LEAKY)) return RTSDS_ERR_UNSUPPORTED;
  if (ws_bytes < rtsds_bn_workspace(rows, c)) return RTSDS_ERR_WORKSPACE;
  BnArgs a(rows, c, ws, stream);
  bn_bwd_args(a, x, dx, dgamma, dbeta, gamma, beta, save_mean, save_invstd, training, act, accumulate_params);
  DISPATCH_T(dtype, {
    const GradScalePool<T> gs{(const T*)dr, (const T*)att, (const T*)dpooled, c, hw, 1.f / (float)hw};
    bn_bwd_launch<T, 1, GradScalePool<T>>(gs, a);
  });
  RET_LAUNCH();
}

template <typename T>
__global__ void __launch_bounds__(256) bn_relu_pool_fwd_kernel(const T* __restrict__ x, const float* __restrict__ scale,
                                                              const float* __restrict__ shift, T* __restrict__ y,
                                                              uint8_t* __restrict__ idx, int h, int w, int c, int ho, int wo, int p,
                                                              long total, FastDiv f_cv, FastDiv f_wo, FastDiv f_ho) {
  typedef typename VecT<T>::v16 V16;
  constexpr int V = VecT<T>::N;
  const int cv = c / V;
  const int nwg = gridDim.x, bx = blockIdx.x, xcd = bx & 7, qq = nwg >> 3, rr = nwg & 7;
  const long lb = (xcd < rr ? xcd * (qq + 1) : rr * (qq + 1) + (xcd - rr) * qq) + (bx >> 3);
  for (long i = lb * blockDim.x + threadIdx.x; i < total; i += (long)gridDim.x * blockDim.x) {
    const uint32_t ii = (uint32_t)i, q0 = fdiv(ii, f_cv), q1 = fdiv(q0, f_wo), img = fdiv(q1, f_ho);
    const int ch = (int)(ii - q0 * cv) * V;
    const int ow = (int)(q0 - q1 * wo), oh = (int)(q1 - img * ho);
    const int h0 = oh * 2 - p, w0 = ow * 2 - p;
    V16 v[9];
#pragma unroll
    for (int t = 0; t < 9; ++t) {
      const int hh = min(max(h0 + t / 3, 0), h - 1), ww = min(max(w0 + t % 3, 0), w - 1);
      v[t] = *(const V16*)(x + (((long)img * h + hh) * w + ww) * c + ch);
    }
    float sc[V], sh[V];
    load_coef<V>(scale, ch, c, sc);
    load_coef<V>(shift, ch, c, sh);
    float best[V];
    int bi[V];
#pragma unroll
    for (int j = 0; j < V; ++j) { best[j] = -INFINITY; bi[j] = -1; }
#pragma unroll
    for (int t = 0; t < 9; ++t) {
      const int hh = h0 + t / 3, ww = w0 + t % 3;
      if ((unsigned)hh >= (unsigned)h || (unsigned)ww >= (unsigned)w) continue;
#pragma unroll
      for (int j = 0; j < V; ++j) {
        const float f = to_f(from_f<T>(fmaxf(fmaf(to_f(v[t][j]), sc[j], sh[j]), 0.f)));
        if (bi[j] < 0 || f > best[j] || (f != f && best[j] == best[j])) { best[j] = f; bi[j] = t; }
      }
    }
    V16 o;
    const long oi = (((long)img * ho + oh) * wo + ow) * c + ch;
    unsigned long long ib = 0;
#pragma unroll
    for (int j = 0; j < V; ++j) {
      o[j] = from_f<T>(best[j]);
      ib |= (unsigned long long)(bi[j] < 0 ? 0 : bi[j]) << (8 * j);
    }
    *(V16*)(y + oi) = o;
    *(unsigned long long*)(idx + oi) = ib;
  }
}
static bool bn_pool_ok(int n, int h, int w, int c, int ho, int wo, int p, int dtype) {
  return dtype == RTSDS_BF16 && c % 8 == 0 && n > 0 && ho > 0 && wo > 0 && (p == 0 || p == 1) &&
         (long)n * h * w * c < (1L << 31) && (long)n * ho * wo * c < (1L << 31);
}
extern "C" int rtsds_bn_relu_maxpool_fwd(const void* x, void* y, uint8_t* idx, int n, int h, int w, int c, int ho, int wo, int p,
                                         const float* gamma, const float* beta, float* running_mean, float* running_var,
                                         long long* num_batches_tracked, float* save_mean, float* save_invstd, float momentum,
                                         float eps, int training, const float* stats_part, int stats_nrb, int dtype, void* ws,
                                         size_t ws_bytes, void* stream) {
  const long rows = (long)n * h * w;
  if (!bn_pool_ok(n, h, w, c, ho, wo, p, dtype)) return RTSDS_ERR_UNSUPPORTED;
  if (ws_bytes < rtsds_bn_workspace(rows, c)) return RTSDS_ERR_WORKSPACE;
  BnArgs a(rows, c, ws, stream);
  if (int rc = bn_fwd_args(a, gamma, beta, running_mean, running_var, num_batches_tracked, save_mean, save_invstd, momentum, eps,
                           training, stats_part, stats_nrb))
    return rc;
  a.x = x;
  bn_fwd_coefs<bf16, 8>(a);
  hipStream_t st = a.st;
  const float *scale = a.w.coef, *shift = a.w.coef + c;
  const long total = (long)n * ho * wo * (c / 8);
  const int blocks = (int)std::max<long>(1, std::min<long>((total + 255) / 256, 1L << 20));
  hipLaunchKernelGGL(bn_relu_pool_fwd_kernel<bf16>, dim3(blocks), dim3(256), 0, st, (const bf16*)x, scale, shift, (bf16*)y, idx, h, w, c, ho, wo, p, total, fastdiv_make(c / 8), fastdiv_make(wo),
                     fastdiv_make(ho));
  RET_LAUNCH();
}
extern "C" int rtsds_bn_relu_maxpool_bwd(const void* dy_pool, const uint8_t* idx, const void* x, void* dx, float* dgamma,
                                         float* dbeta, int n, int h, int w, int c, int ho, int wo, int p, const float* gamma,
                                         const float* beta, const float* save_mean, const float* save_invstd, int training,
                                         int accumulate_params, int dtype, void* ws, size_t ws_bytes, void* stream) {
  const long rows = (long)n * h * w;
  if (!bn_pool_ok(n, h, w, c, ho, wo, p, dtype)) return RTSDS_ERR_UNSUPPORTED;
  if (ws_bytes < rtsds_bn_workspace(rows, c)) return RTSDS_ERR_WORKSPACE;
  const GradPool<bf16> gs{(const bf16*)dy_pool, idx, c, h, w, ho, wo, p, fastdiv_make(w), fastdiv_make(h)};
  BnArgs a(rows, c, ws, stream);
  bn_bwd_args(a, x, dx, dgamma, dbeta, gamma, beta, save_mean, save_invstd, training, RTSDS_ACT_RELU, accumulate_params);
  bn_bwd_launch<bf16, 8, GradPool<bf16>>(gs, a);
  RET_LAUNCH();
}

__global__ void bn_fold_kernel(const float* __restrict__ gamma, const float* __restrict__ beta,
                               const float* __restrict__ rm, const float* __restrict__ rv,
                               const float* __restrict__ bias, float eps, int c, float* __restrict__ scale,
                               float* __restrict__ shift) {
  const int i = blockIdx.x * blockDim.x + threadIdx.x;
  if (i >= c) return;
  const float s = (gamma ? gamma[i] : 1.f) / sqrtf(rv[i] + eps);
  scale[i] = s;
  shift[i] = fmaf((bias ? bias[i] : 0.f) - rm[i], s, beta ? beta[i] : 0.f);
}

extern "C" int rtsds_bn_fold(const float* gamma, const float* beta, const float* running_mean,
                             const float* running_var, const float* conv_bias, float eps, int c, float* scale,
                             float* shift, void* stream) {
  if (c <= 0) return RTSDS_ERR_SHAPE;
  if (!running_mean || !running_var || !scale || !shift) return RTSDS_ERR_UNSUPPORTED;
  hipLaunchKernelGGL(bn_fold_kernel, dim3(rt_cdiv(c, 256)), dim3(256), 0, (hipStream_t)stream, gamma, beta, running_mean,
                     running_var, conv_bias, eps, c, scale, shift);
  RET_LAUNCH();
}
```

rtsds_amd/csrc/bn_dev.h:

```cpp
#pragma once
#include "common.h"

template <typename T, int VEC>
RT_DEV void load_vec(const T* p, float* v, int cvalid) {
  static_assert(VEC == 1 || VEC == VecT<T>::N, "VEC");
  if constexpr (VEC == VecT<T>::N) {
    typename VecT<T>::v16 t = *(const typename VecT<T>::v16*)p;
#pragma unroll
    for (int j = 0; j < VEC; ++j) v[j] = to_f(t[j]);
  } else {
    v[0] = cvalid > 0 ? to_f(p[0]) : 0.f;
  }
}
template <typename T, int VEC>
RT_DEV void store_vec(T* p, const float* v, int cvalid) {
  if constexpr (VEC == VecT<T>::N) {
    typename VecT<T>::v16 t;
#pragma unroll
    for (int j = 0; j < VEC; ++j) t[j] = from_f<T>(v[j]);
    *(typename VecT<T>::v16*)p = t;
  } else {
    if (cvalid > 0) p[0] = from_f<T>(v[0]);
  }
}

RT_DEV float act_grad(float y, int act) {
  if (act == RTSDS_ACT_RELU) return y > 0.f ? 1.f : 0.f;
  if (act == RTSDS_ACT_LEAKY) return y > 0.f ? 1.f : 0.2f;
  if (act == RTSDS_ACT_SIGMOID) return y * (1.f - y);
  return 1.f;
}

template <int VEC, bool HAS_Y>
RT_DEV void bn_mask(float* g, const float* yv, const float* xv, const float* sc, const float* sh, int act) {
  if (!act) return;
#pragma unroll
  for (int j = 0; j < VEC; ++j) {
    if constexpr (HAS_Y) g[j] *= act_grad(yv[j], act);
    else g[j] = fmaf(xv[j], sc[j], sh[j]) > 0.f ? g[j] : (act == RTSDS_ACT_LEAKY ? 0.2f * g[j] : 0.f);
  }
}

template <int VEC> struct BnDx {
  float a[VEC], b[VEC], k[VEC], mu[VEC], sc[VEC], sh[VEC];
};

template <typename T, int VEC>
RT_DEV void bn_row_mask(float* g, const T* __restrict__ y, const float* xv, const BnDx<VEC>& k, int act, int cvalid) {
  if (!act) return;
  if (y) {
    float yv[VEC];
    load_vec<T, VEC>(y, yv, cvalid);
    bn_mask<VEC, true>(g, yv, xv, k.sc, k.sh, act);
  } else {
    bn_mask<VEC, false>(g, nullptr, xv, k.sc, k.sh, act);
  }
}
template <int VEC>
RT_DEV float bn_bwd_dx(const BnDx<VEC>& k, int j, float g, float x) { return fmaf(k.a[j], g, fmaf(k.b[j], x - k.mu[j], k.k[j])); }
```

rtsds_amd/functional.py:

```python
import ctypes

import numpy as np
import torch

from ._lib import ACT_RELU, ACT_SIGMOID, INPUT_PADDED, UPCE_SET_CORRECT, WEIGHT_PACKED, ConvDesc, SplitReduceDesc, lib
from .runtime import (CL, bump_params_epoch, collective, dcode, dp_world, empty_nhwc, nhwc, params_epoch,
                      register_fold, require_hip, side_enabled, side_fork, stream, workspace)

_P = lambda t: None if t is None else t.data_ptr()

CONV_PROFILE = None


def _conv_flops(d):
    return 2.0 * d.n * d.ho * d.wo * d.k * d.c * d.kh * d.kw


class _Timed:
    def __init__(self, d, tag="fwd"):
        self.d, self.tag = d, tag

    def __enter__(self):
        if CONV_PROFILE is not None:
            self.e0 = torch.cuda.Event(enable_timing=True)
            self.e1 = torch.cuda.Event(enable_timing=True)
            self.e0.record()
        return self

    def __exit__(self, *exc):
        if CONV_PROFILE is not None:
            self.e1.record()
            CONV_PROFILE.append((self.e0, self.e1, _conv_flops(self.d), self.tag, self.d))


def _sink(p):
    ref = getattr(p, "_rt_arena", None) if p is not None else None
    if ref is None:
        return None
    arena, i = ref
    return arena.sink(i)


def _sinks(*params):
    out = []
    for p in params:
        if p is None:
            out.append(None)
            continue
        s = _sink(p)
        if s is None:
            return None
        out.append(s)
    return out


def _bn_param_grads(ctx, c, device):
    need_g, need_b = ctx.needs_input_grad[1], ctx.needs_input_grad[2]
    sinks = _sinks(ctx.gamma if need_g else None, ctx.beta if need_b else None) if (need_g or need_b) else None
    if sinks is not None:
        return sinks[0], sinks[1], 1
    dg = torch.empty(c, dtype=torch.float32, device=device) if need_g else None
    db = torch.empty(c, dtype=torch.float32, device=device) if need_b else None
    return dg, db, 0


def _conv_desc(x, k, kh, kw, stride, padding, dilation):
    n, c, h, w = x.shape
    ho = (h + 2 * padding[0] - dilation[0] * (kh - 1) - 1) // stride[0] + 1
    wo = (w + 2 * padding[1] - dilation[1] * (kw - 1) - 1) // stride[1] + 1
    d = ConvDesc(n, h, w, c, ho, wo, k, kh, kw, stride[0], stride[1], padding[0], padding[1],
                 dilation[0], dilation[1], dcode(x))
    return d


def is_padded_input(x, d=None):
    cp = getattr(x, "_rt_cpad", None)
    ok = cp is not None and x.dim() == 4 and x.stride(1) == 1 and x.stride(3) == cp and \
        x.stride(2) == cp * x.shape[3] and x.stride(0) == cp * x.shape[2] * x.shape[3]
    return ok and (d is None or lib.rtsds_conv2d_input_pitch(ctypes.byref(d)) == cp)


def detach_padded(x):
    y = x.detach()
    if getattr(x, "_rt_cpad", None) is not None:
        y._rt_cpad = x._rt_cpad
    return y


_DPACK = {"on": True}


def set_dgrad_packs(on):
    _DPACK["on"] = bool(on)


class _DPack:
    __slots__ = ("arena", "key", "desc", "buf", "valid")


def _desc_key(d):
    return tuple(getattr(d, f) for f, _ in ConvDesc._fields_)


def _dgrad_weight(weight, wq, d):
    if not _DPACK["on"] or wq.dtype != torch.bfloat16 or weight is None:
        return wq, 0
    ref = getattr(weight, "_rt_arena", None)
    if ref is None:
        return wq, 0
    pk = getattr(weight, "_rt_dpack", None)
    if pk is not None and pk.arena is ref[0]:
        if pk.key == _desc_key(d) and pk.buf is not None and pk.valid is not None and \
                pk.valid == getattr(weight, "_rt_shadow_key", None) and wq is getattr(weight, "_rt_shadow", None):
            return pk.buf, WEIGHT_PACKED
        return wq, 0
    pk = _DPack()
    pk.arena, pk.key, pk.valid = ref[0], _desc_key(d), None
    pk.desc = ConvDesc(*pk.key)
    nb = lib.rtsds_conv2d_dgrad_pack_bytes(ctypes.byref(d))
    pk.buf = torch.empty(nb // 2, dtype=torch.bfloat16, device=wq.device) if nb else None
    weight._rt_dpack = pk
    if nb:
        ref[0].dpacks.append(weight)
    return wq, 0


class GradJoin:

    __slots__ = ("left", "buf", "first")

    def __init__(self, n, first_returns=False):
        self.left = n
        self.buf = None
        self.first = first_returns

    def put(self, g):
        if self.first:
            if self.buf is None:
                self.buf = g
                return g
            return None
        self.buf = g
        self.left -= 1
        return g if self.left == 0 else None


def _join_add(join, g):
    if join is None:
        return g
    if join.buf is not None:
        if join.first:
            join.buf.add_(g)
            return join.put(join.buf)
        g.add_(join.buf)
    return join.put(g)


DEFER_WGRAD_REDUCE = True
_deferred = []


def flush_wgrad_reduce():
    global _deferred
    items, _deferred = _deferred, []
    if not items:
        return
    cur = torch.cuda.current_stream(items[0][1].device)
    for st in {it[2] for it in items}:
        if st != cur:
            cur.wait_stream(st)
    batch, seen = [], set()
    for desc, _ws, _st in items + [(None, None, None)]:
        if desc is None or desc.dw in seen or len(batch) == 16:
            if batch:
                arr = (SplitReduceDesc * len(batch))(*batch)
                lib.rtsds_split_reduce_many(len(batch), arr, cur.cuda_stream)
            batch, seen = [], set()
        if desc is not None:
            batch.append(desc)
            seen.add(desc.dw)
    for _desc, ws, st in items:
        if st != cur:
            ws.record_stream(cur)


def _wgrad_into_arena(d, x, g, sinks, xflag, ws):
    if DEFER_WGRAD_REDUCE and CONV_PROFILE is None and x.dtype == torch.bfloat16:
        pend = SplitReduceDesc()
        lib.rtsds_conv2d_wgrad_deferred(ctypes.byref(d), _P(x), _P(g), _P(sinks[0]), _P(sinks[1]), 1 | xflag,
                                        _P(ws), ws.numel(), ctypes.byref(pend), stream())
        if pend.nv > 0:
            _deferred.append((pend, ws, torch.cuda.current_stream(ws.device)))
            torch.autograd.Variable._execution_engine.queue_callback(flush_wgrad_reduce)
        return
    with _Timed(d, "wgrad"):
        lib.rtsds_conv2d_wgrad(ctypes.byref(d), _P(x), _P(g), _P(sinks[0]), _P(sinks[1]), 1 | xflag,
                               _P(ws), ws.numel(), stream())


class ConvFn(torch.autograd.Function):

    @staticmethod
    def forward(ctx, x, weight, bias, wq, stride, padding, dilation, act, stats, join=None, fold=(0, False),
                bn_link=None, wg_link=None):
        require_hip(x, weight)
        k, _, kh, kw = weight.shape
        padded = hasattr(x, "_rt_cpad") and is_padded_input(x, _conv_desc(x, k, kh, kw, stride, padding, dilation))
        if not padded:
            x = nhwc(x)
        d = _conv_desc(x, k, kh, kw, stride, padding, dilation)
        y = empty_nhwc(d.n, k, d.ho, d.wo, x.dtype, x.device)
        ws = workspace(lib.rtsds_conv2d_fwd_workspace(ctypes.byref(d)), x.device)
        flag = INPUT_PADDED if padded else 0
        with _Timed(d, "fwd"):
            lib.rtsds_conv2d_fwd(ctypes.byref(d), _P(x), _P(wq), _P(bias), _P(y), act | flag, _P(stats), _P(ws),
                                        ws.numel(), stream())
        ctx.xflag = flag
        ctx.in_act, ctx.out_folded = fold
        ctx.bn_link = bn_link if join is None and not fold[0] else None
        if ctx.in_act and join is not None:
            raise RuntimeError("rtsds_amd: a conv whose input gradient is masked cannot join other readers")
        ctx.d, ctx.act, ctx.has_bias = d, act, bias is not None
        ctx.params = (weight, bias)
        ctx.wg_link = None
        if wg_link is not None:
            wg_link.conv_ok = bool(
                IMG_WGRAD_LINK and not ctx.needs_input_grad[0] and ctx.needs_input_grad[1] and bias is None and not act
                and not fold[0] and not fold[1]
                and lib.rtsds_imgconv_bn_wgrad_workspace(ctypes.byref(d)) > 0)
            if wg_link.conv_ok:
                ctx.wg_link = wg_link
        ctx.join = join
        ctx.save_for_backward(x, wq, y if act else None)
        return y

    @staticmethod
    def backward(ctx, dy):
        x, wq, y = ctx.saved_tensors
        d = ctx.d
        dy = nhwc(dy)
        if dy.dtype != x.dtype:
            dy = cast(dy, x.dtype)
        link = ctx.wg_link
        if link is not None and link.bn is not None:
            (bx, coef, bact), link.bn = link.bn, None
            return (None, _img_bn_wgrad(d, x, dy, bx, coef, bact, ctx.params[0], ctx.xflag)) + (None,) * 11
        if ctx.act and not ctx.out_folded:
            g = torch.empty_like(dy)
            lib.rtsds_act_bwd(_P(dy), _P(y), _P(g), dy.numel(), ctx.act, 1.0, dcode(dy), stream())
        else:
            g = dy
        dx = dw = db = None
        wg_side = None
        if ctx.needs_input_grad[1] and side_enabled(d.n * d.ho * d.wo) and CONV_PROFILE is None:
            weight, bias = ctx.params
            sinks = _sinks(weight, bias if ctx.needs_input_grad[2] else None)
            if sinks is not None:
                ws = workspace(lib.rtsds_conv2d_wgrad_workspace(ctypes.byref(d)), x.device)
                side = side_fork(x, g, ws)
                lib.rtsds_conv2d_wgrad(ctypes.byref(d), _P(x), _P(g), _P(sinks[0]), _P(sinks[1]), 1 | ctx.xflag,
                                       _P(ws), ws.numel(), side.cuda_stream)
                wg_side = True
        if ctx.needs_input_grad[0]:
            join = ctx.join
            acc = join is not None and join.buf is not None
            dx = join.buf if acc else empty_nhwc(d.n, d.c, d.h, d.w, x.dtype, x.device)
            ws = workspace(lib.rtsds_conv2d_dgrad_workspace(ctypes.byref(d)), x.device)
            link = ctx.bn_link
            wd, wpk = _dgrad_weight(ctx.params[0], wq, d)
            tiles = 0
            if link is not None and link.src is not None and not acc and g.dtype == torch.bfloat16:
                tiles = lib.rtsds_conv2d_dgrad_bnstats_tiles(ctypes.byref(d))
            with _Timed(d, "dgrad"):
                if tiles:
                    bx, bsm, bsi, bg, bb, bact = link.src
                    part = torch.empty(d.c * tiles * 2, dtype=torch.float32, device=x.device)
                    lib.rtsds_conv2d_dgrad_bnstats(ctypes.byref(d), _P(g), _P(wd), _P(dx), _P(bx), _P(bg), _P(bb),
                                                   _P(bsm), _P(bsi), bact | wpk, _P(part), _P(ws), ws.numel(), stream())
                    link.part, link.nrb = part, tiles
                elif ctx.in_act:
                    lib.rtsds_conv2d_dgrad_act(ctypes.byref(d), _P(g), _P(wd), _P(dx), _P(x), ctx.in_act | wpk,
                                               _P(ws), ws.numel(), stream())
                else:
                    lib.rtsds_conv2d_dgrad(ctypes.byref(d), _P(g), _P(wd), _P(dx), (1 if acc else 0) | wpk, _P(ws),
                                           ws.numel(), stream())
            if join is not None:
                dx = join.put(dx)
        if (ctx.needs_input_grad[1] or ctx.needs_input_grad[2]) and not wg_side:
            weight, bias = ctx.params
            sinks = _sinks(weight, bias if ctx.needs_input_grad[2] else None) if ctx.needs_input_grad[1] else None
            ws = workspace(lib.rtsds_conv2d_wgrad_workspace(ctypes.byref(d)), x.device)
            if sinks is not None:
                _wgrad_into_arena(d, x, g, sinks, ctx.xflag, ws)
                dw = None
                db = None
            else:
                dw = torch.empty((d.k, d.c, d.kh, d.kw), dtype=torch.float32, device=x.device,
                                 memory_format=CL)
                db = torch.empty(d.k, dtype=torch.float32, device=x.device) if ctx.has_bias else None
                with _Timed(d, "wgrad"):
                    lib.rtsds_conv2d_wgrad(ctypes.byref(d), _P(x), _P(g), _P(dw), _P(db), ctx.xflag, _P(ws),
                                                  ws.numel(), stream())
                if not ctx.needs_input_grad[1]:
                    dw = None
        return dx, dw, db, None, None, None, None, None, None, None, None, None, None


def _img_bn_wgrad(d, x, g, bx, coef, act, weight, xflag):
    ws = workspace(lib.rtsds_imgconv_bn_wgrad_workspace(ctypes.byref(d)), x.device)
    sinks = _sinks(weight)
    if sinks is not None and DEFER_WGRAD_REDUCE and CONV_PROFILE is None:
        pend = SplitReduceDesc()
        lib.rtsds_imgconv_bn_wgrad_deferred(ctypes.byref(d), _P(x), _P(g), _P(bx), _P(coef), act, _P(sinks[0]),
                                            1 | xflag, _P(ws), ws.numel(), ctypes.byref(pend), stream())
        _deferred.append((pend, ws, torch.cuda.current_stream(ws.device)))
        torch.autograd.Variable._execution_engine.queue_callback(flush_wgrad_reduce)
        return None
    dw = sinks[0] if sinks is not None else torch.empty((d.k, d.c, d.kh, d.kw), dtype=torch.float32,
                                                         device=x.device, memory_format=CL)
    with _Timed(d, "wgrad"):
        lib.rtsds_imgconv_bn_wgrad(ctypes.byref(d), _P(x), _P(g), _P(bx), _P(coef), act, _P(dw),
                                   (1 if sinks is not None else 0) | xflag, _P(ws), ws.numel(), stream())
    return None if sinks is not None else dw


def conv2d(x, weight, bias, wq, stride=(1, 1), padding=(0, 0), dilation=(1, 1), act=0, bn_stats=False,
           join=None, in_act=0, fold_out=False, bn_link=None, wg_link=None):
    stats = nrb = None
    if bn_stats and act == 0:
        n, _, h, w = x.shape
        k, _, kh, kw = weight.shape
        d = _conv_desc(x, k, kh, kw, stride, padding, dilation)
        nrb = lib.rtsds_conv2d_fwd_stats_tiles(ctypes.byref(d))
        stats = torch.empty(nrb * k * 4, dtype=torch.float32, device=x.device)
    y = ConvFn.apply(x, weight, bias, wq, tuple(stride), tuple(padding), tuple(dilation), act, stats, join,
                     (in_act, bool(fold_out and act in (1, 2))), bn_link, wg_link)
    if stats is not None:
        y._rt_bn_stats = (stats, nrb)
    return y


def _bn_fold(gamma, beta, running_mean, running_var, bias, eps, k):
    ts = (gamma, beta, running_mean, running_var, bias)

    def key():
        return (params_epoch(), float(eps)) + tuple((t.data_ptr(), t._version) if t is not None else None for t in ts)

    ent = getattr(running_mean, "_rt_fold", None)
    if ent is None or ent[1].numel() != 2 * k or ent[1].device != running_mean.device:
        ent = [None, torch.empty(2 * k, dtype=torch.float32, device=running_mean.device)]
        running_mean._rt_fold = ent
    ss = ent[1]

    def refresh():
        kk = key()
        if ent[0] != kk:
            lib.rtsds_bn_fold(_P(gamma), _P(beta), _P(running_mean), _P(running_var), _P(bias), float(eps), k,
                              _P(ss), ss.data_ptr() + 4 * k, stream())
            ent[0] = kk

    refresh()
    register_fold(refresh)
    return ss


def conv_bn_eval(x, weight, bias, wq, stride, padding, dilation, gamma, beta, running_mean, running_var,
                 eps, act=0, residual=None, out=None):
    require_hip(x, weight)
    k, _, kh, kw = weight.shape
    flag = INPUT_PADDED if hasattr(x, "_rt_cpad") and \
        is_padded_input(x, _conv_desc(x, k, kh, kw, stride, padding, dilation)) else 0
    if not flag:
        x = nhwc(x)
    d = _conv_desc(x, k, kh, kw, stride, padding, dilation)
    ss = _bn_fold(gamma, beta, running_mean, running_var, bias, eps, k)
    if residual is not None:
        residual = nhwc(residual)
        if residual.dtype != x.dtype or tuple(residual.shape) != (d.n, k, d.ho, d.wo):
            raise RuntimeError("rtsds_amd.conv_bn_eval: residual must match the conv output")
    ws = workspace(lib.rtsds_conv2d_fwd_workspace(ctypes.byref(d)), x.device)
    if out is not None and residual is None:
        buf, off = out
        if _slice_target(buf, off, (d.n, k, d.ho, d.wo), x.dtype):
            try:
                with _Timed(d, "fwd"):
                    lib.rtsds_conv2d_fwd_bn_ld(ctypes.byref(d), _P(x), _P(wq), _P(ss), ss.data_ptr() + 4 * k,
                                               buf.data_ptr() + off * buf.element_size(), buf.shape[1], act | flag,
                                               _P(ws), ws.numel(), stream())
                return buf[:, off:off + k]
            except RuntimeError as e:
                if "unsupported" not in str(e):
                    raise
    y = empty_nhwc(d.n, k, d.ho, d.wo, x.dtype, x.device)
    with _Timed(d, "fwd"):
        lib.rtsds_conv2d_fwd_bn(ctypes.byref(d), _P(x), _P(wq), _P(ss), ss.data_ptr() + 4 * k, _P(residual), _P(y),
                                act | flag, _P(ws), ws.numel(), stream())
    return y


def conv_bn_maxpool_eval(x, weight, bias, wq, stride, padding, dilation, gamma, beta, running_mean, running_var, eps,
                         act, pool_k, pool_s, pool_p, ceil_mode):
    require_hip(x, weight)
    if pool_k != 3 or pool_s != 2 or x.dtype != torch.bfloat16:
        return None
    k, _, kh, kw = weight.shape
    flag = INPUT_PADDED if hasattr(x, "_rt_cpad") and \
        is_padded_input(x, _conv_desc(x, k, kh, kw, stride, padding, dilation)) else 0
    if not flag:
        x = nhwc(x)
    d = _conv_desc(x, k, kh, kw, stride, padding, dilation)
    hp, wp = pool_out(d.ho, 3, 2, pool_p, ceil_mode), pool_out(d.wo, 3, 2, pool_p, ceil_mode)
    ss = _bn_fold(gamma, beta, running_mean, running_var, bias, eps, k)
    y = empty_nhwc(d.n, k, hp, wp, x.dtype, x.device)
    ws = workspace(lib.rtsds_conv2d_fwd_workspace(ctypes.byref(d)), x.device)
    try:
        with _Timed(d, "fwd"):
            lib.rtsds_conv2d_fwd_bn_maxpool(ctypes.byref(d), _P(x), _P(wq), _P(ss), ss.data_ptr() + 4 * k, _P(y),
                                            act | flag, hp, wp, pool_p, _P(ws), ws.numel(), stream())
    except RuntimeError as e:
        if "unsupported" in str(e):
            return None
        raise
    return y


class ConvSumFn(torch.autograd.Function):

    @staticmethod
    def forward(ctx, x, geoms, *wb):
        require_hip(x)
        x = nhwc(x)
        m = len(geoms)
        weights, biases, wqs = wb[:m], wb[m:2 * m], wb[2 * m:]
        descs = []
        y = None
        for i, (stride, padding, dilation) in enumerate(geoms):
            k, _, kh, kw = weights[i].shape
            d = _conv_desc(x, k, kh, kw, stride, padding, dilation)
            if y is None:
                y = empty_nhwc(d.n, k, d.ho, d.wo, x.dtype, x.device)
            ws = workspace(lib.rtsds_conv2d_fwd_workspace(ctypes.byref(d)), x.device)
            with _Timed(d, "fwd"):
                lib.rtsds_conv2d_fwd(ctypes.byref(d), _P(x), _P(wqs[i]), _P(biases[i]), _P(y),
                                     0x100 if i else 0, None, _P(ws), ws.numel(), stream())
            descs.append(d)
        ctx.descs = descs
        ctx.params = tuple(weights) + tuple(biases)
        ctx.has_bias = [b is not None for b in biases]
        ctx.save_for_backward(x, *wqs)
        return y

    @staticmethod
    def backward(ctx, dy):
        x, *wqs = ctx.saved_tensors
        dy = nhwc(dy)
        m = len(wqs)
        dx = None
        dws, dbs = [None] * m, [None] * m
        for i, d in enumerate(ctx.descs):
            if ctx.needs_input_grad[0]:
                if dx is None:
                    dx = empty_nhwc(d.n, d.c, d.h, d.w, x.dtype, x.device)
                ws = workspace(lib.rtsds_conv2d_dgrad_workspace(ctypes.byref(d)), x.device)
                wd, wpk = _dgrad_weight(ctx.params[i], wqs[i], d)
                with _Timed(d, "dgrad"):
                    lib.rtsds_conv2d_dgrad(ctypes.byref(d), _P(dy), _P(wd), _P(dx), (1 if i else 0) | wpk,
                                           _P(ws), ws.numel(), stream())
            if ctx.needs_input_grad[2 + i] or ctx.needs_input_grad[2 + m + i]:
                w_i, b_i = ctx.params[i], ctx.params[m + i]
                sinks = (_sinks(w_i, b_i if ctx.needs_input_grad[2 + m + i] else None)
                         if ctx.needs_input_grad[2 + i] else None)
                ws = workspace(lib.rtsds_conv2d_wgrad_workspace(ctypes.byref(d)), x.device)
                if sinks is not None:
                    with _Timed(d, "wgrad"):
                        lib.rtsds_conv2d_wgrad(ctypes.byref(d), _P(x), _P(dy), _P(sinks[0]), _P(sinks[1]),
                                               1, _P(ws), ws.numel(), stream())
                    continue
                dw = torch.empty((d.k, d.c, d.kh, d.kw), dtype=torch.float32, device=x.device,
                                 memory_format=CL)
                db = torch.empty(d.k, dtype=torch.float32, device=x.device) if ctx.has_bias[i] else None
                with _Timed(d, "wgrad"):
                    lib.rtsds_conv2d_wgrad(ctypes.byref(d), _P(x), _P(dy), _P(dw), _P(db), 0, _P(ws),
                                           ws.numel(), stream())
                dws[i] = dw if ctx.needs_input_grad[2 + i] else None
                dbs[i] = db
        return (dx, None, *dws, *dbs, *([None] * m))


BN_BWD_LINK = True


class BnBwdLink:

    __slots__ = ("src", "part", "nrb")

    def __init__(self):
        self.src = None
        self.part = None
        self.nrb = 0


IMG_WGRAD_LINK = True


class ImgWgradLink:

    __slots__ = ("conv_ok", "bn")

    def __init__(self):
        self.conv_ok = False
        self.bn = None

    def take(self, x, training, act):
        if IMG_WGRAD_LINK and self.conv_ok and training and act in (0, 1, 2) and x.dtype == torch.bfloat16 \
                and not getattr(x, "_backward_hooks", None):
            return self
        return None


def _bn_bwd_coef(ctx_link, dy, x, dg, db, rows, c, gamma, beta, sm, si, training, act, acc):
    coef = torch.empty(6 * c, dtype=torch.float32, device=x.device)
    ws = workspace(lib.rtsds_bn_workspace(rows, c), x.device)
    lib.rtsds_bn_bwd_coef(_P(dy), _P(x), _P(dg), _P(db), _P(coef), rows, c, _P(gamma), _P(beta), _P(sm), _P(si),
                          training, act, acc, dcode(x), _P(ws), ws.numel(), stream())
    ctx_link.bn = (x, coef, act)


class BatchNormFn(torch.autograd.Function):

    @staticmethod
    def forward(ctx, x, gamma, beta, res, running_mean, running_var, training, momentum, eps, act,
                stats, stats_nrb, nbt, res_join=None, link=None, out=None, wg_link=None):
        require_hip(x)
        x = nhwc(x)
        if res is not None:
            res = nhwc(res)
        n, c, h, w = x.shape
        rows = n * h * w
        keep_y = res is not None or act == ACT_SIGMOID
        ld = c
        if out is not None and not keep_y and x.dtype == torch.bfloat16 and \
                _slice_target(out[0], out[1], x.shape, x.dtype, vec16=True):
            buf, off = out
            ld = buf.shape[1]
            y = buf[:, off:off + c]
        else:
            y = torch.empty_like(x, memory_format=CL)
        sm = torch.empty(c, dtype=torch.float32, device=x.device)
        si = torch.empty(c, dtype=torch.float32, device=x.device)
        ws = workspace(lib.rtsds_bn_workspace(rows, c), x.device)
        lib.rtsds_bn_fwd_ld(_P(x), _P(res), _P(y), ld, rows, c, _P(gamma), _P(beta), _P(running_mean),
                            _P(running_var), _P(nbt), _P(sm), _P(si), float(momentum), float(eps), int(training),
                            act, _P(stats) if training else None, int(stats_nrb or 0), dcode(x), _P(ws),
                            ws.numel(), stream())
        ctx.meta = (rows, c, int(training), act, res is not None)
        ctx.gamma, ctx.beta = gamma, beta
        ctx.res_join = res_join
        ctx.save_for_backward(x, y if keep_y else None, gamma, beta, sm, si)
        ctx.link = None
        if link is not None and BN_BWD_LINK and training and res is None and act in (0, 1, 2) \
                and x.dtype == torch.bfloat16 and c % 8 == 0:
            link.src, link.part = (x, sm, si, gamma, beta, act), None
            ctx.link = link
        ctx.wg_link = wg_link if res is None else None
        return y

    @staticmethod
    def backward(ctx, dy):
        x, y, gamma, beta, sm, si = ctx.saved_tensors
        rows, c, training, act, has_res = ctx.meta
        ldy = _channel_slice_pitch(dy) if ctx.link is None else 0
        if not ldy:
            dy = nhwc(dy)
            ldy = c
        need_dx, need_r = ctx.needs_input_grad[0], ctx.needs_input_grad[3]
        if ctx.wg_link is not None and need_dx and ldy == c and dy.dtype == x.dtype:
            dg, db, acc = _bn_param_grads(ctx, c, x.device)
            _bn_bwd_coef(ctx.wg_link, dy, x, dg, db, rows, c, gamma, beta, sm, si, training, act, acc)
            if acc:
                dg = db = None
            return (dy, dg, db) + (None,) * 14
        dx = torch.empty_like(x, memory_format=CL) if need_dx else None
        dres = torch.empty_like(x, memory_format=CL) if (has_res and need_r) else None
        dg, db, acc = _bn_param_grads(ctx, c, x.device)
        ws = workspace(lib.rtsds_bn_workspace(rows, c), x.device)
        link = ctx.link
        if link is not None and link.part is not None and dy.dtype == x.dtype:
            lib.rtsds_bn_bwd_part(_P(dy), _P(x), _P(dx), _P(dg), _P(db), rows, c, _P(gamma), _P(beta), _P(sm),
                                  _P(si), training, act, acc, _P(link.part), link.nrb, dcode(x), _P(ws), ws.numel(),
                                  stream())
        else:
            lib.rtsds_bn_bwd_ld(_P(dy), ldy, _P(x), _P(y), _P(dx), _P(dres), _P(dg), _P(db), rows, c,
                                _P(gamma), _P(beta), _P(sm), _P(si), training, act, acc, dcode(x), _P(ws), ws.numel(),
                                stream())
        if link is not None:
            link.src = link.part = None
        if acc:
            dg = db = None
        if dres is not None:
            dres = _join_add(ctx.res_join, dres)
        return dx, dg, db, dres, None, None, None, None, None, None, None, None, None, None, None, None, None


def _nhwc_pitch(t):
    n, c, h, w = t.shape
    ld = t.stride(3)
    if t.stride(1) != 1 or ld < c or (h > 1 and t.stride(2) != w * ld) or (n > 1 and t.stride(0) != h * w * ld):
        return 0
    return ld


def _slice_target(buf, off, shape, dtype, vec16=False):
    n, c, h, w = shape
    if buf.dim() != 4 or buf.dtype != dtype or (buf.shape[0], buf.shape[2], buf.shape[3]) != (n, h, w):
        return False
    ld = buf.shape[1]
    if off < 0 or off + c > ld or _nhwc_pitch(buf) != ld:
        return False
    if vec16:
        vec = 16 // buf.element_size()
        if off % vec or c % vec or ld % vec or (buf.data_ptr() + off * buf.element_size()) % 16:
            return False
    return True


def _channel_slice_pitch(t):
    if t.dim() != 4 or t.dtype != torch.bfloat16:
        return 0
    ld = _nhwc_pitch(t)
    if ld <= t.shape[1] or t.shape[1] % 8 or ld % 8 or t.data_ptr() % 16:
        return 0
    return ld


def _bn_epilogue_stats(x, training, running_mean):
    st = getattr(x, "_rt_bn_stats", None) if training else None
    if training and running_mean is not None:
        bump_params_epoch()
    return st if st is not None else (None, None)


def batch_norm(x, gamma, beta, running_mean, running_var, training, momentum, eps, act=0,
               residual=None, num_batches_tracked=None, res_join=None, link=None, out=None, wg_link=None):
    stats, nrb = _bn_epilogue_stats(x, training, running_mean)
    if wg_link is not None:
        wg_link = wg_link.take(x, training and residual is None, act)
    return BatchNormFn.apply(x, gamma, beta, residual, running_mean, running_var, training,
                             momentum, eps, act, stats, nrb, num_batches_tracked, res_join, link, out, wg_link)


def pack_input(x, dtype):
    require_hip(x)
    if x.dtype == dtype and x.dim() == 4 and (x.is_contiguous(memory_format=CL) and x.shape[1] > 1 or is_padded_input(x)):
        return x
    if x.requires_grad and torch.is_grad_enabled():
        return PackInputFn.apply(x, dtype)
    return _pack(x, dtype)


class PackInputFn(torch.autograd.Function):
    @staticmethod
    def forward(ctx, x, dtype):
        ctx.xdtype = x.dtype
        return _pack(x, dtype)

    @staticmethod
    def backward(ctx, dy):
        return cast(nhwc(dy), ctx.xdtype), None


def pack_input_into(x, y):
    require_hip(x)
    xf = (x if x.dtype == torch.float32 else cast(x, torch.float32)).contiguous()
    n, c, h, w = xf.shape
    if tuple(y.shape) != (n, c, h, w):
        raise RuntimeError("rtsds_amd.pack_input_into: shape mismatch")
    if is_padded_input(y):
        lib.rtsds_nchw_to_nhwc_pad(_P(xf), _P(y), n, c, h, w, y._rt_cpad, 0 if y.dtype == torch.float32 else 1, stream())
    elif y.is_contiguous(memory_format=CL):
        lib.rtsds_nchw_to_nhwc(_P(xf), _P(y), n, c, h, w, 0 if y.dtype == torch.float32 else 1, stream())
    else:
        raise RuntimeError("rtsds_amd.pack_input_into: y is not a packed input")
    return y


def _pack(x, dtype):
    xf = x if x.dtype == torch.float32 else cast(x, torch.float32)
    xf = xf.contiguous()
    n, c, h, w = xf.shape
    if c == 3 and dtype == torch.bfloat16:
        buf = torch.empty((n, h, w, 4), dtype=dtype, device=x.device)
        lib.rtsds_nchw_to_nhwc_pad(_P(xf), _P(buf), n, c, h, w, 4, 1, stream())
        y = buf.permute(0, 3, 1, 2)[:, :3]
        y._rt_cpad = 4
        return y
    y = empty_nhwc(n, c, h, w, dtype, x.device)
    lib.rtsds_nchw_to_nhwc(_P(xf), _P(y), n, c, h, w, 0 if dtype == torch.float32 else 1, stream())
    return y


def cast(t, dtype):
    if t.dtype == dtype:
        return t
    out = torch.empty_like(t, dtype=dtype)
    if not (t.is_contiguous() or t.is_contiguous(memory_format=CL)):
        raise RuntimeError("rtsds_amd.cast: dense tensor required")
    if out.stride() != t.stride():
        raise RuntimeError("rtsds_amd.cast: layout mismatch")
    lib.rtsds_cast(_P(t), dcode(t), _P(out), dcode(out), t.numel(), stream())
    return out


class CatFn(torch.autograd.Function):

    @staticmethod
    def forward(ctx, joins, *xs):
        xs = [nhwc(x) for x in xs]
        n, _, h, w = xs[0].shape
        ct = sum(x.shape[1] for x in xs)
        y = empty_nhwc(n, ct, h, w, xs[0].dtype, xs[0].device)
        off = 0
        for x in xs:
            c = x.shape[1]
            lib.rtsds_copy_channels(_P(x), c, 0, _P(y), ct, off, n * h * w, c, 0, dcode(x), stream())
            off += c
        ctx.split = [x.shape[1] for x in xs]
        ctx.joins = joins
        return y

    @staticmethod
    def backward(ctx, dy):
        dy = nhwc(dy)
        n, ct, h, w = dy.shape
        outs, off = [None], 0
        for i, c in enumerate(ctx.split):
            if ctx.needs_input_grad[1 + i]:
                join = ctx.joins[i] if ctx.joins else None
                acc = join is not None and join.buf is not None
                g = join.buf if acc else empty_nhwc(n, c, h, w, dy.dtype, dy.device)
                lib.rtsds_copy_channels(_P(dy), ct, off, _P(g), c, 0, n * h * w, c, 1 if acc else 0, dcode(dy),
                                        stream())
                outs.append(join.put(g) if join is not None else g)
            else:
                outs.append(None)
            off += c
        return tuple(outs)


class CatResizeFn(torch.autograd.Function):

    @staticmethod
    def forward(ctx, size, joins, into, x0, *xs):
        xs = [nhwc(x) for x in xs]
        ct = x0.shape[1] + sum(x.shape[1] for x in xs)
        ctx.x0_in_place = into is not None and tuple(into.shape[1:]) == (ct,) + tuple(x0.shape[2:]) and \
            x0.data_ptr() == into.data_ptr() and _channel_slice_pitch(x0) == ct
        if not ctx.x0_in_place:
            x0 = nhwc(x0)
        n, c0, h, w = x0.shape
        if (h, w) != (int(size[0]), int(size[1])):
            raise RuntimeError("rtsds_amd.concat_resized: x0 must have the target size")
        y = into if ctx.x0_in_place else empty_nhwc(n, ct, h, w, x0.dtype, x0.device)
        if not ctx.x0_in_place:
            lib.rtsds_copy_channels(_P(x0), c0, 0, _P(y), ct, 0, n * h * w, c0, 0, dcode(x0), stream())
        off, geos = c0, []
        for x in xs:
            _, c, hi, wi = x.shape
            ho, wo, sh, sw = upsample_geometry(x, size=size)
            lib.rtsds_bilinear_fwd(_P(x), _P(y), n, hi, wi, c, ho, wo, sh, sw, ct, off, dcode(x), stream())
            geos.append((off, c, hi, wi, ho, wo, sh, sw))
            off += c
        ctx.meta = (n, c0, h, w, ct, geos)
        ctx.joins = joins
        return y

    @staticmethod
    def backward(ctx, dy):
        n, c0, h, w, ct, geos = ctx.meta
        dy = nhwc(dy)
        grads = [None, None, None, None]
        if ctx.needs_input_grad[3]:
            if ctx.x0_in_place:
                grads[3] = dy[:, :c0]
            else:
                g0 = empty_nhwc(n, c0, h, w, dy.dtype, dy.device)
                lib.rtsds_copy_channels(_P(dy), ct, 0, _P(g0), c0, 0, n * h * w, c0, 0, dcode(dy), stream())
                grads[3] = g0
        for k, (off, c, hi, wi, ho, wo, sh, sw) in enumerate(geos):
            if not ctx.needs_input_grad[4 + k]:
                grads.append(None)
                continue
            dx = empty_nhwc(n, c, hi, wi, dy.dtype, dy.device)
            ws = workspace(lib.rtsds_bilinear_bwd_workspace(n, hi, wi, c, ho, wo), dy.device)
            lib.rtsds_bilinear_bwd(_P(dy), _P(dx), n, hi, wi, c, ho, wo, sh, sw, ct, off, dcode(dy), _P(ws),
                                   ws.numel(), stream())
            grads.append(_join_add(ctx.joins[k], dx) if ctx.joins else dx)
        return tuple(grads)


def concat_resized(x0, xs, size, joins=None, into=None):
    return CatResizeFn.apply((int(size[0]), int(size[1])), tuple(joins) if joins else None, into, x0, *xs)


def concat_resized_scaled_eval(x0, parts, size, into=None):
    n, c0, h, w = x0.shape
    ps = []
    for x, scales in parts:
        x = nhwc(x)
        if len(scales) > 2 or x.shape[-2] > h or x.shape[-1] > w:
            return None
        ss = [(s if s.dtype == x.dtype else cast(s, x.dtype)).contiguous() for s in scales]
        ps.append((x, ss + [None] * (2 - len(ss))))
    ct = c0 + sum(x.shape[1] for x, _ in ps)
    if into is not None and _slice_target(into, 0, (n, ct, h, w), x0.dtype) and into.shape[1] == ct:
        y = into
        in_place = x0.data_ptr() == into.data_ptr() and x0.stride() == into.stride()
    else:
        y, in_place = empty_nhwc(n, ct, h, w, x0.dtype, x0.device), False
    if not in_place:
        x0 = nhwc(x0)
    off = c0
    for x, (s1, s2) in ps:
        _, c, hi, wi = x.shape
        ho, wo, sh, sw = upsample_geometry(x, size=size)
        try:
            lib.rtsds_bilinear_fwd_scaled(_P(x), _P(s1), _P(s2), _P(y), n, hi, wi, c, ho, wo, sh, sw, ct, off, dcode(x), stream())
        except RuntimeError as e:
            if "unsupported" in str(e):
                return None
            raise
        off += c
    if not in_place:
        lib.rtsds_copy_channels(_P(x0), c0, 0, _P(y), ct, 0, n * h * w, c0, 0, dcode(x0), stream())
    return y


def ffm_head_eval(feature, w1, b1, w2, b2, w3, b3):
    f = nhwc(feature)
    n, c, h, w = f.shape
    out = empty_nhwc(n, c, h, w, f.dtype, f.device)
    ws = [t.reshape(c, c).contiguous() for t in (w1, w2, w3)]
    bs = [None if b is None else b.float().contiguous() for b in (b1, b2, b3)]
    wk = workspace(lib.rtsds_ffm_head_eval_workspace(n, h * w, c), f.device)
    lib.rtsds_ffm_head_eval(_P(f), _P(ws[0]), _P(bs[0]), _P(ws[1]), _P(bs[1]), _P(ws[2]), _P(bs[2]), _P(out), n, h * w, c,
                            dcode(f), _P(wk), wk.numel(), stream())
    return out


def cat(xs, joins=None):
    return CatFn.apply(joins, *xs)


class ActFn(torch.autograd.Function):

    @staticmethod
    def forward(ctx, x, act):
        require_hip(x)
        x = x.contiguous(memory_format=CL) if x.dim() == 4 else x.contiguous()
        y = torch.empty_like(x)
        lib.rtsds_act_fwd(_P(x), _P(y), x.numel(), act, dcode(x), stream())
        ctx.act = act
        ctx.save_for_backward(y)
        return y

    @staticmethod
    def backward(ctx, dy):
        (y,) = ctx.saved_tensors
        dy = dy.contiguous(memory_format=CL) if dy.dim() == 4 else dy.contiguous()
        dx = torch.empty_like(y)
        lib.rtsds_act_bwd(_P(dy), _P(y), _P(dx), y.numel(), ctx.act, 1.0, dcode(y), stream())
        return dx, None


def relu(x):
    return ActFn.apply(x, 1)


def leaky_relu(x):
    return ActFn.apply(x, 2)


def sigmoid(x):
    return ActFn.apply(x, 3)


class GradReverseFn(torch.autograd.Function):

    @staticmethod
    def forward(ctx, x, alpha):
        ctx.alpha = float(alpha)
        return x.view_as(x)

    @staticmethod
    def backward(ctx, dy):
        dy = dy.contiguous(memory_format=CL) if dy.dim() == 4 else dy.contiguous()
        dx = torch.empty_like(dy)
        lib.rtsds_act_bwd(_P(dy), None, _P(dx), dy.numel(), 0, -ctx.alpha, dcode(dy), stream())
        return dx, None


def pool_out(size, k, s, p, ceil_mode):
    num = size + 2 * p - (k - 1) - 1 + ((s - 1) if ceil_mode else 0)
    o = num // s + 1
    if ceil_mode and (o - 1) * s >= size + p:
        o -= 1
    return o


class MaxPoolFn(torch.autograd.Function):
    @staticmethod
    def forward(ctx, x, k, s, p, ceil_mode):
        require_hip(x)
        x = nhwc(x)
        n, c, h, w = x.shape
        ho, wo = pool_out(h, k, s, p, ceil_mode), pool_out(w, k, s, p, ceil_mode)
        y = empty_nhwc(n, c, ho, wo, x.dtype, x.device)
        need = ctx.needs_input_grad[0] or not (k == 3 and c % (8 if x.dtype == torch.bfloat16 else 4) == 0)
        idx = torch.empty((n, ho, wo, c), dtype=torch.uint8, device=x.device) if need else None
        lib.rtsds_maxpool_fwd(_P(x), _P(y), _P(idx), n, h, w, c, ho, wo, k, s, p, dcode(x), stream())
        ctx.geo = (n, h, w, c, ho, wo, k, s, p)
        ctx.dtype = x.dtype
        ctx.save_for_backward(idx)
        return y

    @staticmethod
    def backward(ctx, dy):
        (idx,) = ctx.saved_tensors
        n, h, w, c, ho, wo, k, s, p = ctx.geo
        dy = nhwc(dy)
        dx = empty_nhwc(n, c, h, w, dy.dtype, dy.device)
        lib.rtsds_maxpool_bwd(_P(dy), _P(idx), _P(dx), n, h, w, c, ho, wo, k, s, p, dcode(dy), stream())
        return dx, None, None, None, None


def max_pool2d(x, k, s, p, ceil_mode=False):
    return MaxPoolFn.apply(x, k, s, p, ceil_mode)


class BnReluMaxPoolFn(torch.autograd.Function):

    @staticmethod
    def forward(ctx, x, gamma, beta, running_mean, running_var, training, momentum, eps, stats, stats_nrb, nbt,
                p, ceil_mode, wg_link=None):
        require_hip(x)
        x = nhwc(x)
        n, c, h, w = x.shape
        ho, wo = pool_out(h, 3, 2, p, ceil_mode), pool_out(w, 3, 2, p, ceil_mode)
        y = empty_nhwc(n, c, ho, wo, x.dtype, x.device)
        idx = torch.empty((n, ho, wo, c), dtype=torch.uint8, device=x.device)
        sm = torch.empty(c, dtype=torch.float32, device=x.device)
        si = torch.empty(c, dtype=torch.float32, device=x.device)
# ... 974 lines not shown
```

rtsds_amd/models/bisenet/build_contextpath.py:

```python
import torch
from torch import nn

from rtsds_amd import functional as F
from rtsds_amd.functional import BnBwdLink
from rtsds_amd.nn import BatchNorm2d, Conv2d, MaxPool2d, ReLU, conv_bn, conv_bn_relu_maxpool, grad_join
from rtsds_amd.runtime import grad_cut


class BasicBlock(nn.Module):
    expansion = 1

    def __init__(self, inplanes, planes, stride=1, downsample=None):
        super().__init__()
        self.conv1 = Conv2d(inplanes, planes, 3, stride, 1, bias=False)
        self.bn1 = BatchNorm2d(planes)
        self.relu = ReLU(inplace=True)
        self.conv2 = Conv2d(planes, planes, 3, 1, 1, bias=False)
        self.bn2 = BatchNorm2d(planes)
        self.downsample = downsample
        self.stride = stride

    def forward(self, x):
        join = grad_join(x, 2)
        skip = x
        if self.downsample is not None:
            skip = conv_bn(self.downsample[0], self.downsample[1], x, join=join)
        link = BnBwdLink()
        t = conv_bn(self.conv1, self.bn1, x, "relu", join=join, out_link=link)
        return conv_bn(self.conv2, self.bn2, t, "relu", skip,
                       res_join=join if self.downsample is None else None, in_link=link)


class Bottleneck(nn.Module):
    expansion = 4

    def __init__(self, inplanes, planes, stride=1, downsample=None):
        super().__init__()
        self.conv1 = Conv2d(inplanes, planes, 1, bias=False)
        self.bn1 = BatchNorm2d(planes)
        self.conv2 = Conv2d(planes, planes, 3, stride, 1, bias=False)
        self.bn2 = BatchNorm2d(planes)
        self.conv3 = Conv2d(planes, planes * 4, 1, bias=False)
        self.bn3 = BatchNorm2d(planes * 4)
        self.relu = ReLU(inplace=True)
        self.downsample = downsample
        self.stride = stride

    def forward(self, x):
        join = grad_join(x, 2)
        skip = x
        if self.downsample is not None:
            skip = conv_bn(self.downsample[0], self.downsample[1], x, join=join)
        l1, l2 = BnBwdLink(), BnBwdLink()
        t = conv_bn(self.conv1, self.bn1, x, "relu", join=join, out_link=l1)
        t = conv_bn(self.conv2, self.bn2, t, "relu", in_link=l1, out_link=l2)
        return conv_bn(self.conv3, self.bn3, t, "relu", skip,
                       res_join=join if self.downsample is None else None, in_link=l2)


class ResNet(nn.Module):

    def __init__(self, block, layers, num_classes=1000):
        super().__init__()
        self.inplanes = 64
        self.conv1 = Conv2d(3, 64, 7, 2, 3, bias=False)
        self.bn1 = BatchNorm2d(64)
        self.relu = ReLU(inplace=True)
        self.maxpool = MaxPool2d(3, 2, 1)
        self.layer1 = self._stage(block, 64, layers[0], 1)
        self.layer2 = self._stage(block, 128, layers[1], 2)
        self.layer3 = self._stage(block, 256, layers[2], 2)
        self.layer4 = self._stage(block, 512, layers[3], 2)
        self.avgpool = nn.AdaptiveAvgPool2d((1, 1))
        self.fc = nn.Linear(512 * block.expansion, num_classes)
        for m in self.modules():
            if isinstance(m, nn.Conv2d):
                nn.init.kaiming_normal_(m.weight, mode="fan_out", nonlinearity="relu")
            elif isinstance(m, nn.BatchNorm2d):
                nn.init.ones_(m.weight)
                nn.init.zeros_(m.bias)

    def _stage(self, block, planes, count, stride):
        down = None
        if stride != 1 or self.inplanes != planes * block.expansion:
            down = nn.Sequential(Conv2d(self.inplanes, planes * block.expansion, 1, stride, bias=False),
                                 BatchNorm2d(planes * block.expansion))
        mods = [block(self.inplanes, planes, stride, down)]
        self.inplanes = planes * block.expansion
        for _ in range(1, count):
            mods.append(block(self.inplanes, planes))
        return nn.Sequential(*mods)


class _ContextPath(nn.Module):
    def __init__(self, trunk):
        super().__init__()
        self.features = trunk
        self.conv1 = trunk.conv1
        self.bn1 = trunk.bn1
        self.relu = trunk.relu
        self.maxpool1 = trunk.maxpool
        self.layer1, self.layer2 = trunk.layer1, trunk.layer2
        self.layer3, self.layer4 = trunk.layer3, trunk.layer4

    fork_after = 1

    def forward(self, x, mid=None, tail_join=None):
        if mid is not None and self.fork_after < 0:
            mid()
        t = conv_bn_relu_maxpool(self.conv1, self.bn1, self.maxpool1, x)
        for i, layer in enumerate((self.layer1, self.layer2)):
            if mid is not None and self.fork_after == i:
                mid()
            t = layer(t)
        if mid is not None and self.fork_after >= 2:
            mid()
        f3 = grad_cut(self.layer3(t))
        f4 = self.layer4(f3)
        return f3, f4, F.global_avg_pool(f4, tail_join)


class resnet18(_ContextPath):
    def __init__(self, pretrained=True):
        super().__init__(ResNet(BasicBlock, [2, 2, 2, 2]))


class resnet101(_ContextPath):
    def __init__(self, pretrained=True):
        super().__init__(ResNet(Bottleneck, [3, 4, 23, 3]))


def build_contextpath(name):
    builders = {"resnet18": resnet18, "resnet101": resnet101}
    if name not in builders:
        raise KeyError(name)
    return builders[name](pretrained=True)
```

rtsds_amd/models/deeplabv2/deeplabv2.py:

```python
import torch
import torch.nn as nn

from rtsds_amd import functional as F
from rtsds_amd.functional import BnBwdLink
from rtsds_amd.nn import BatchNorm2d, Conv2d, MaxPool2d, ReLU, conv_bn, conv_bn_relu_maxpool, grad_join, to_input
from rtsds_amd.nn import _shadow
from rtsds_amd.runtime import grad_cut

affine_par = True


def _freeze(bn):
    for p in bn.parameters():
        p.requires_grad = False
    return bn


class Bottleneck(nn.Module):
    expansion = 4

    def __init__(self, inplanes, planes, stride=1, dilation=1, downsample=None):
        super(Bottleneck, self).__init__()
        self.conv1 = Conv2d(inplanes, planes, kernel_size=1, stride=stride, bias=False)
        self.bn1 = _freeze(BatchNorm2d(planes, affine=affine_par))
        self.conv2 = Conv2d(planes, planes, kernel_size=3, stride=1, padding=dilation, bias=False,
                            dilation=dilation)
        self.bn2 = _freeze(BatchNorm2d(planes, affine=affine_par))
        self.conv3 = Conv2d(planes, planes * 4, kernel_size=1, bias=False)
        self.bn3 = _freeze(BatchNorm2d(planes * 4, affine=affine_par))
        self.relu = ReLU(inplace=True)
        self.downsample = downsample
        self.stride = stride

    def forward(self, x):
        join = grad_join(x, 2)
        skip = x if self.downsample is None else conv_bn(self.downsample[0], self.downsample[1], x, join=join)
        l1, l2 = BnBwdLink(), BnBwdLink()
        t = conv_bn(self.conv1, self.bn1, x, "relu", join=join, out_link=l1)
        t = conv_bn(self.conv2, self.bn2, t, "relu", in_link=l1, out_link=l2)
        return conv_bn(self.conv3, self.bn3, t, "relu", skip,
                       res_join=join if self.downsample is None else None, in_link=l2)


class ClassifierModule(nn.Module):

    def __init__(self, inplanes, dilation_series, padding_series, num_classes):
        super(ClassifierModule, self).__init__()
        self.conv2d_list = nn.ModuleList()
        for dilation, padding in zip(dilation_series, padding_series):
            self.conv2d_list.append(Conv2d(inplanes, num_classes, kernel_size=3, stride=1,
                                           padding=padding, dilation=dilation, bias=True))
        for m in self.conv2d_list:
            m.weight.data.normal_(0, 0.01)

    def forward(self, x):
        convs = list(self.conv2d_list)
        geoms = tuple((c.stride, c.padding, c.dilation) for c in convs)
        ws = [c.weight for c in convs]
        bs = [c.bias for c in convs]
        wqs = [_shadow(c.weight, x.dtype) for c in convs]
        return F.ConvSumFn.apply(x, geoms, *ws, *bs, *wqs)


class ResNetMulti(nn.Module):
    accepts_packed_input = True

    def __init__(self, block, layers, num_classes):
        self.inplanes = 64
        super(ResNetMulti, self).__init__()
        self.conv1 = Conv2d(3, 64, kernel_size=7, stride=2, padding=3, bias=False)
        self.bn1 = _freeze(BatchNorm2d(64, affine=affine_par))
        self.relu = ReLU(inplace=True)
        self.maxpool = MaxPool2d(kernel_size=3, stride=2, padding=1, ceil_mode=True)
        self.layer1 = self._make_layer(block, 64, layers[0])
        self.layer2 = self._make_layer(block, 128, layers[1], stride=2)
        self.layer3 = self._make_layer(block, 256, layers[2], stride=1, dilation=2)
        self.layer4 = self._make_layer(block, 512, layers[3], stride=1, dilation=4)
        self.layer6 = ClassifierModule(2048, [6, 12, 18, 24], [6, 12, 18, 24], num_classes)
        for m in self.modules():
            if isinstance(m, nn.Conv2d):
                m.weight.data.normal_(0, 0.01)
            elif isinstance(m, nn.BatchNorm2d):
                m.weight.data.fill_(1)
                m.bias.data.zero_()
        self.multi_level = False

    def _make_layer(self, block, planes, blocks, stride=1, dilation=1):
        down = nn.Sequential(
            Conv2d(self.inplanes, planes * block.expansion, kernel_size=1, stride=stride, bias=False),
            _freeze(BatchNorm2d(planes * block.expansion, affine=affine_par)))
        layers = [block(self.inplanes, planes, stride, dilation=dilation, downsample=down)]
        self.inplanes = planes * block.expansion
        for _ in range(1, blocks):
            layers.append(block(self.inplanes, planes, dilation=dilation))
        return nn.Sequential(*layers)

    def forward_lowres(self, x, main_only=False):
        _, _, H, W = x.size()
        t = to_input(x)
        t = conv_bn_relu_maxpool(self.conv1, self.bn1, self.maxpool, t)
        t = grad_cut(self.layer2(self.layer1(t)))
        for i, blk in enumerate(self.layer3):
            t = blk(t)
            if i == len(self.layer3) // 2:
                t = grad_cut(t)
        t = self.layer4(grad_cut(t))
        t = self.layer6(t)
        return [(t, F.upsample_geometry(t, size=(H, W)))]

    def forward(self, x):
        (t, geo), = self.forward_lowres(x)
        t = F.interpolate_geometry(t, geo)
        if self.training == True:
            return t, None, None
        return t

    def get_1x_lr_params_no_scale(self):
        for mod in (self.conv1, self.bn1, self.layer1, self.layer2, self.layer3, self.layer4):
            for m in mod.modules():
                for p in m.parameters(recurse=False):
                    if p.requires_grad:
                        yield p

    def get_10x_lr_params(self):
        for p in self.layer6.parameters():
            yield p

    def optim_parameters(self, lr):
        return [{"params": self.get_1x_lr_params_no_scale(), "lr": lr},
                {"params": self.get_10x_lr_params(), "lr": 10 * lr}]


def get_deeplab_v2(num_classes=19, pretrain=True,
                   pretrain_model_path="DeepLab_resnet_pretrained_imagenet.pth"):
    model = ResNetMulti(Bottleneck, [3, 4, 23, 3], num_classes)
    if pretrain:
        print("Deeplab pretraining loading...")
        saved = torch.load(pretrain_model_path, map_location="cpu", weights_only=True)
        new_params = model.state_dict().copy()
        for k in saved:
            new_params[".".join(k.split(".")[1:])] = saved[k]
        model.load_state_dict(new_params, strict=False)
    return model
```

rtsds_amd/nn.py:

```python
import torch
from torch import nn

from . import functional as F
from ._lib import lib
from .runtime import CL, compute_dtype

ACT = {None: 0, "relu": 1, "leaky": 2, "sigmoid": 3}


def _shadow(w, dtype):
    if dtype == torch.float32:
        return w.detach() if w.is_contiguous(memory_format=CL) else w.detach().contiguous(memory_format=CL)
    sh = getattr(w, "_rt_shadow", None)
    key = (w.data_ptr(), w._version)
    if sh is not None and getattr(w, "_rt_shadow_key", None) == key and sh.device == w.device:
        return sh
    if sh is None or sh.shape != w.shape or sh.device != w.device:
        sh = torch.empty(w.shape, dtype=torch.bfloat16, device=w.device, memory_format=CL)
    src = w.detach()
    if not src.is_contiguous(memory_format=CL):
        src = src.contiguous(memory_format=CL)
    lib.rtsds_cast(src.data_ptr(), 0, sh.data_ptr(), 1, src.numel(), torch.cuda.current_stream().cuda_stream)
    w._rt_shadow, w._rt_shadow_key = sh, key
    return sh


class Conv2d(nn.Conv2d):
    def __init__(self, *args, **kwargs):
        super().__init__(*args, **kwargs)
        if self.groups != 1 or self.padding_mode != "zeros":
            raise NotImplementedError("rtsds_amd.Conv2d: groups=1, zero padding only")
        self.weight.data = self.weight.data.contiguous(memory_format=CL)

    def _apply(self, fn, *a, **k):
        out = super()._apply(fn, *a, **k)
        if not self.weight.is_contiguous(memory_format=CL):
            self.weight.data = self.weight.data.contiguous(memory_format=CL)
        return out

    def forward(self, x, act=None, bn_stats=False, join=None, in_act=None, fold_out=False, bn_link=None, wg_link=None):
        wq = _shadow(self.weight, x.dtype)
        return F.conv2d(x, self.weight, self.bias, wq, self.stride, self.padding, self.dilation,
                        ACT[act], bn_stats, join, ACT[in_act], fold_out, bn_link, wg_link)


class BatchNorm2d(nn.BatchNorm2d):
    def forward(self, x, act=None, residual=None, res_join=None, link=None, out=None, wg_link=None):
        training = self.training or not self.track_running_stats
        if training and x.shape[0] * x.shape[2] * x.shape[3] == 1:
            raise ValueError(f"Expected more than 1 value per channel when training, got input size {tuple(x.shape)}")
        if self.momentum is None:
            raise NotImplementedError("rtsds_amd.BatchNorm2d: cumulative moving average (momentum=None)")
        rm = self.running_mean if self.track_running_stats else None
        rv = self.running_var if self.track_running_stats else None
        nbt = self.num_batches_tracked if (self.training and self.track_running_stats) else None
        return F.batch_norm(x, self.weight, self.bias, rm, rv, training, self.momentum, self.eps,
                            ACT[act], residual, nbt, res_join, link, out, wg_link)


class ReLU(nn.Module):
    def __init__(self, inplace=False):
        super().__init__()
        self.inplace = inplace

    def forward(self, x):
        return F.relu(x)


class LeakyReLU(nn.Module):
    def __init__(self, negative_slope=0.2):
        super().__init__()
        if negative_slope != 0.2:
            raise NotImplementedError("rtsds_amd.LeakyReLU: slope 0.2 (model.py:62,73)")
        self.negative_slope = negative_slope

    def forward(self, x):
        return F.leaky_relu(x)


class Sigmoid(nn.Module):
    def forward(self, x):
        return F.sigmoid(x)


class AdaptiveAvgPool2d(nn.Module):
    def __init__(self, output_size=(1, 1)):
        super().__init__()
        osz = (output_size, output_size) if isinstance(output_size, int) else tuple(output_size)
        if osz != (1, 1):
            raise NotImplementedError("rtsds_amd.AdaptiveAvgPool2d: output (1, 1) only")
        self.output_size = output_size

    def forward(self, x):
        return F.global_avg_pool(x)


class MaxPool2d(nn.Module):
    def __init__(self, kernel_size, stride=None, padding=0, ceil_mode=False):
        super().__init__()
        self.kernel_size, self.stride = kernel_size, stride or kernel_size
        self.padding, self.ceil_mode = padding, ceil_mode

    def forward(self, x):
        return F.max_pool2d(x, self.kernel_size, self.stride, self.padding, self.ceil_mode)


def _no_grad_needed(conv, bn, x, residual):
    if not torch.is_grad_enabled():
        return True
    ts = [x, residual, conv.weight, conv.bias, bn.weight, bn.bias]
    return not any(t is not None and t.requires_grad for t in ts)


def _img_wgrad_link(conv, x):
    if conv.in_channels == 3 and conv.bias is None and torch.is_grad_enabled() and not x.requires_grad \
            and conv.weight.requires_grad:
        return F.ImgWgradLink()
    return None


def conv_bn(conv, bn, x, act=None, residual=None, join=None, res_join=None, in_link=None, out_link=None, out=None):
    use_batch = bn.training or not bn.track_running_stats
    if not use_batch and bn.momentum is not None and _no_grad_needed(conv, bn, x, residual):
        wq = _shadow(conv.weight, x.dtype)
        return F.conv_bn_eval(x, conv.weight, conv.bias, wq, conv.stride, conv.padding, conv.dilation,
                              bn.weight, bn.bias, bn.running_mean, bn.running_var, bn.eps, ACT[act], residual, out=out)
    wg = _img_wgrad_link(conv, x) if use_batch and residual is None and join is None else None
    return bn(conv(x, bn_stats=use_batch, join=join, bn_link=in_link, wg_link=wg), act=act, residual=residual,
              res_join=res_join, link=out_link, out=out, wg_link=wg)


def conv_bn_relu_maxpool(conv, bn, pool, x):
    use_batch = bn.training or not bn.track_running_stats
    k = pool.kernel_size if isinstance(pool.kernel_size, int) else pool.kernel_size[0]
    s = pool.stride if isinstance(pool.stride, int) else pool.stride[0]
    p = pool.padding if isinstance(pool.padding, int) else pool.padding[0]
    if use_batch and bn.momentum is not None and x.dtype == torch.bfloat16 and conv.out_channels % 8 == 0 \
            and k == 3 and s == 2 and p in (0, 1):
        wg = _img_wgrad_link(conv, x)
        y = conv(x, bn_stats=True, wg_link=wg)
        if F.bn_relu_maxpool_ok(y, k, s, p):
            rm = bn.running_mean if bn.track_running_stats else None
            rv = bn.running_var if bn.track_running_stats else None
            nbt = bn.num_batches_tracked if (bn.training and bn.track_running_stats) else None
            return F.bn_relu_maxpool(y, bn.weight, bn.bias, rm, rv, True, bn.momentum, bn.eps, p, pool.ceil_mode, nbt,
                                     wg_link=wg)
        return pool(bn(y, act="relu", wg_link=wg))
    if not use_batch and bn.momentum is not None and _no_grad_needed(conv, bn, x, None) and k == 3 and s == 2:
        y = F.conv_bn_maxpool_eval(x, conv.weight, conv.bias, _shadow(conv.weight, x.dtype), conv.stride, conv.padding,
                                   conv.dilation, bn.weight, bn.bias, bn.running_mean, bn.running_var, bn.eps,
                                   ACT["relu"], k, s, p, pool.ceil_mode)
        if y is not None:
            return y
    return pool(conv_bn(conv, bn, x, "relu"))


def grad_join(x, n):
    return F.GradJoin(n) if (torch.is_grad_enabled() and x.requires_grad) else None


def to_input(x):
    return F.pack_input(x, compute_dtype())
```

Measured before the change: 1840 images/s.

## Fuse downsample BN with residual-block tail BN and store ReLU mask as bits

Adds a paired batch-norm path for ResNet blocks that have a downsample branch. The downsample BN normalisation, the main-branch BN, the residual add and the ReLU now run in one apply kernel, and the paired finalize and backward kernels handle both BNs together. The ReLU mask is saved as packed bits rather than the full output tensor for backward. The aim is to avoid materialising the normalised skip tensor and to cut launches and memory traffic, at the cost of more complex kernels and a rounding step on the skip value inside the fused path.

```diff
diff --git a/include/rtsds_hip.h b/include/rtsds_hip.h
--- a/include/rtsds_hip.h
+++ b/include/rtsds_hip.h
@@ -110,6 +110,34 @@
                       int training, int act, int accumulate_params, const float* part, int nrb, int dtype, void* ws,
                       size_t ws_bytes, void* stream);
 
+size_t rtsds_bn_bits_bytes(long rows, int c, int dtype);
+int rtsds_bn_fwd_bits(const void* x, const void* res, void* y, uint8_t* bits, long rows, int c, const float* gamma,
+                      const float* beta, float* running_mean, float* running_var, long long* num_batches_tracked,
+                      float* save_mean, float* save_invstd, float momentum, float eps, const float* stats_part,
+                      int stats_nrb, int dtype, void* ws, size_t ws_bytes, void* stream);
+int rtsds_bn_bwd_bits(const void* dy, long ldy, const void* x, const uint8_t* bits, void* dx, void* dres, float* dgamma,
+                      float* dbeta, long rows, int c, const float* gamma, const float* beta, const float* save_mean,
+                      const float* save_invstd, int accumulate_params, int dtype, void* ws, size_t ws_bytes,
+                      void* stream);
+typedef struct rtsds_bn_params {
+  const float *gamma, *beta;
+  float *running_mean, *running_var;
+  long long* num_batches_tracked;
+  float *save_mean, *save_invstd;
+  float momentum, eps;
+  const float* stats_part;
+  int stats_nrb;
+  int accumulate;
+  float *dgamma, *dbeta;
+} rtsds_bn_params;
+size_t rtsds_bn_pair_workspace(long rows, int c);
+int rtsds_bn_pair_fwd(const void* xa, const void* xb, void* y, uint8_t* bits, long rows, int c,
+                      const rtsds_bn_params* pa, const rtsds_bn_params* pb, int dtype, void* ws, size_t ws_bytes,
+                      void* stream);
+int rtsds_bn_pair_bwd(const void* dy, long ldy, const void* xa, const void* xb, const uint8_t* bits, void* dxa,
+                      void* dxb, long rows, int c, const rtsds_bn_params* pa, const rtsds_bn_params* pb, int dtype,
+                      void* ws, size_t ws_bytes, void* stream);
+
 int rtsds_bn_relu_maxpool_fwd(const void* x, void* y, uint8_t* idx, int n, int h, int w, int c, int ho, int wo,
                               int p, const float* gamma, const float* beta, float* running_mean,
                               float* running_var, long long* num_batches_tracked, float* save_mean,
@@ -312,7 +340,7 @@
                      const float* save_invstd, int training, int act, int accumulate_params, int dtype, void* ws,
                      size_t ws_bytes, void* stream);
 
-#define RTSDS_ABI_VERSION 23
+#define RTSDS_ABI_VERSION 24
 int rtsds_abi_version(void);
 
 #ifdef __cplusplus
diff --git a/rtsds_amd/_lib.py b/rtsds_amd/_lib.py
--- a/rtsds_amd/_lib.py
+++ b/rtsds_amd/_lib.py
@@ -5,7 +5,7 @@
 
 _HERE = os.path.dirname(os.path.abspath(__file__))
 DEFAULT_LIB_PATH = os.path.join(_HERE, "librtsds_hip.so")
-ABI_VERSION = 23
+ABI_VERSION = 24
 LIB_PATH = os.environ.get("RTSDS_LIB") or DEFAULT_LIB_PATH
 
 F32, BF16 = 0, 1
@@ -28,6 +28,13 @@
 class SplitReduceDesc(ctypes.Structure):
     _fields_ = [("slab", c_void_p), ("dw", c_void_p), ("slab_stride", c_long), ("nv", c_int), ("cv", c_int),
                 ("cp", c_int), ("splits", c_int), ("accumulate", c_int)]
+
+
+class BnParams(ctypes.Structure):
+    _fields_ = [("gamma", c_void_p), ("beta", c_void_p), ("running_mean", c_void_p), ("running_var", c_void_p),
+                ("num_batches_tracked", c_void_p), ("save_mean", c_void_p), ("save_invstd", c_void_p),
+                ("momentum", c_float), ("eps", c_float), ("stats_part", c_void_p), ("stats_nrb", c_int),
+                ("accumulate", c_int), ("dgamma", c_void_p), ("dbeta", c_void_p)]
 
 
 P = c_void_p
@@ -77,6 +84,15 @@
                              P, c_size_t, P]),
     "rtsds_bn_bwd_ld": (c_int, [P, c_long, P, P, P, P, P, P, c_long, c_int, P, P, P, P, c_int, c_int, c_int, c_int,
                                 P, c_size_t, P]),
+    "rtsds_bn_bits_bytes": (c_size_t, [c_long, c_int, c_int]),
+    "rtsds_bn_fwd_bits": (c_int, [P, P, P, P, c_long, c_int, P, P, P, P, P, P, P, c_float, c_float, P, c_int, c_int, P,
+                                  c_size_t, P]),
+    "rtsds_bn_bwd_bits": (c_int, [P, c_long, P, P, P, P, P, P, c_long, c_int, P, P, P, P, c_int, c_int, P, c_size_t, P]),
+    "rtsds_bn_pair_workspace": (c_size_t, [c_long, c_int]),
+    "rtsds_bn_pair_fwd": (c_int, [P, P, P, P, c_long, c_int, ctypes.POINTER(BnParams), ctypes.POINTER(BnParams), c_int, P,
+                                  c_size_t, P]),
+    "rtsds_bn_pair_bwd": (c_int, [P, c_long, P, P, P, P, P, c_long, c_int, ctypes.POINTER(BnParams),
+                                  ctypes.POINTER(BnParams), c_int, P, c_size_t, P]),
     "rtsds_bn_relu_maxpool_fwd": (c_int, [P, P, P] + [c_int] * 7 + [P, P, P, P, P, P, P, c_float, c_float, c_int, P,
                                                                    c_int, c_int, P, c_size_t, P]),
     "rtsds_bn_relu_maxpool_bwd": (c_int, [P, P, P, P, P, P] + [c_int] * 7 + [P, P, P, P, c_int, c_int, c_int, P,
diff --git a/rtsds_amd/csrc/bn.hip b/rtsds_amd/csrc/bn.hip
--- a/rtsds_amd/csrc/bn.hip
+++ b/rtsds_amd/csrc/bn.hip
@@ -157,6 +157,21 @@
   __shared__ float wr[4][3];
   float sc, sh;
   bn_finalize_body(part, nrb, c, rows, gamma, beta, rmean, rvar, smean, sinv, scale, shift, momentum, eps, nbt, wr, sc, sh);
+}
+struct BnFin {
+  const float* part;
+  int nrb;
+  const float *gamma, *beta;
+  float *rmean, *rvar, *smean, *sinv, *scale, *shift;
+  float momentum, eps;
+  long long* nbt;
+};
+__global__ void __launch_bounds__(256) bn_finalize_pair_kernel(BnFin fa, BnFin fb, int c, long rows) {
+  __shared__ float wr[4][3];
+  const BnFin f = blockIdx.y ? fb : fa;
+  float sc, sh;
+  bn_finalize_body(f.part, f.nrb, c, rows, f.gamma, f.beta, f.rmean, f.rvar, f.smean, f.sinv, f.scale, f.shift, f.momentum, f.eps,
+                   f.nbt, wr, sc, sh);
 }
 __global__ void bn_eval_coef_kernel(int c, const float* gamma, const float* beta, const float* rmean, const float* rvar,
                                     float* scale, float* shift, float* smean, float* sinv, float eps) {
@@ -254,6 +269,58 @@
       v0[j] = act_f(a, act);
     }
     store_vec<T, VEC>(y + r * ldy + ch0, v0, cvalid);
+  }
+}
+
+template <typename T, int VEC, bool PAIR>
+RT_DEV void bn_res_row(float* v, const float* rv, const float* sc, const float* sh, const float* sc2, const float* sh2) {
+#pragma unroll
+  for (int j = 0; j < VEC; ++j) {
+    float r = rv[j];
+    if constexpr (PAIR) r = to_f(from_f<T>(fmaf(r, sc2[j], sh2[j])));
+    float a = fmaf(v[j], sc[j], sh[j]);
+    a += r;
+    v[j] = fmaxf(a, 0.f);
+  }
+}
+template <typename T, int VEC, bool PAIR>
+__global__ void __launch_bounds__(256) bn_apply_bits_kernel(const T* __restrict__ x, const T* __restrict__ res, T* __restrict__ y,
+                                                             uint8_t* __restrict__ bits, const float* __restrict__ scale,
+                                                             const float* __restrict__ shift, const float* __restrict__ scale2,
+                                                             const float* __restrict__ shift2, long rows, int c) {
+  static_assert(VEC == VecT<T>::N, "whole 16-byte channel vectors");
+  const BnTile<VEC> t(c);
+  if (!t.active) return;
+  float sc[VEC], sh[VEC], sc2[PAIR ? VEC : 1], sh2[PAIR ? VEC : 1];
+  load_coef<VEC>(scale, t.ch0, c, sc);
+  load_coef<VEC>(shift, t.ch0, c, sh);
+  if constexpr (PAIR) {
+    load_coef<VEC>(scale2, t.ch0, c, sc2);
+    load_coef<VEC>(shift2, t.ch0, c, sh2);
+  }
+  const int ch0 = t.ch0, cvalid = t.cvalid;
+  const long step = t.step(), nv = c / VEC, bv = ch0 / VEC;
+  long r = t.row0();
+  for (; r + step < rows; r += 2 * step) {
+    float v0[VEC], v1[VEC], r0[VEC], r1[VEC];
+    load_vec<T, VEC>(x + r * c + ch0, v0, cvalid);
+    load_vec<T, VEC>(x + (r + step) * c + ch0, v1, cvalid);
+    load_vec<T, VEC>(res + r * c + ch0, r0, cvalid);
+    load_vec<T, VEC>(res + (r + step) * c + ch0, r1, cvalid);
+    bn_res_row<T, VEC, PAIR>(v0, r0, sc, sh, sc2, sh2);
+    bn_res_row<T, VEC, PAIR>(v1, r1, sc, sh, sc2, sh2);
+    store_vec<T, VEC>(y + r * c + ch0, v0, cvalid);
+    store_vec<T, VEC>(y + (r + step) * c + ch0, v1, cvalid);
+    bits[r * nv + bv] = (uint8_t)bn_y_bits<T, VEC>(v0);
+    bits[(r + step) * nv + bv] = (uint8_t)bn_y_bits<T, VEC>(v1);
+  }
+  if (r < rows) {
+    float v0[VEC], r0[VEC];
+    load_vec<T, VEC>(x + r * c + ch0, v0, cvalid);
+    load_vec<T, VEC>(res + r * c + ch0, r0, cvalid);
+    bn_res_row<T, VEC, PAIR>(v0, r0, sc, sh, sc2, sh2);
+    store_vec<T, VEC>(y + r * c + ch0, v0, cvalid);
+    bits[r * nv + bv] = (uint8_t)bn_y_bits<T, VEC>(v0);
   }
 }
 
@@ -351,19 +418,24 @@
 }
 
 constexpr int kBnU = 2;
-template <typename T, int VEC, bool HAS_Y, class GS>
+template <typename T, int VEC, bool HAS_Y, class GS, bool YBITS = false, bool PAIR = false>
 RT_DEV void bn_bwd_sums(const GS& gs, const T* __restrict__ x, const T* __restrict__ y, T* __restrict__ gout, long r0,
                         long step, long rows, int c, const BnTile<VEC>& t, const BnDx<VEC>& k, int act, float* sg,
-                        float* sgx, float (*g_last)[VEC], float (*xv_last)[VEC]) {
+                        float* sgx, float (*g_last)[VEC], float (*xv_last)[VEC], const uint8_t* __restrict__ ybits = nullptr,
+                        const T* __restrict__ x2 = nullptr, const float* mu2 = nullptr, float* sgx2 = nullptr) {
+  static_assert(HAS_Y || !YBITS, "mask bits stand in for y");
   const int ch0 = t.ch0;
   for (long r = r0; r < rows; r += kBnU * step) {
-    float g[kBnU][VEC], xv[kBnU][VEC], yv[HAS_Y ? kBnU : 1][VEC];
+    float g[kBnU][VEC], xv[kBnU][VEC], yv[HAS_Y ? kBnU : 1][VEC], x2v[PAIR ? kBnU : 1][VEC];
+    unsigned yb[YBITS ? kBnU : 1];
 #pragma unroll
     for (int u = 0; u < kBnU; ++u) {
       const long rr = min(r + u * step, rows - 1);
       gs.template load<VEC>(rr, ch0, g[u], t.cvalid);
       load_vec<T, VEC>(x + rr * c + ch0, xv[u], t.cvalid);
-      if constexpr (HAS_Y) load_vec<T, VEC>(y + rr * c + ch0, yv[u], t.cvalid);
+      if constexpr (YBITS) yb[u] = ybits[rr * (c / VEC) + ch0 / VEC];
+      else if constexpr (HAS_Y) load_vec<T, VEC>(y + rr * c + ch0, yv[u], t.cvalid);
+      if constexpr (PAIR) load_vec<T, VEC>(x2 + rr * c + ch0, x2v[u], t.cvalid);
     }
 #pragma unroll
     for (int u = 0; u < kBnU; ++u)
@@ -373,12 +445,14 @@
       }
 #pragma unroll
     for (int u = 0; u < kBnU; ++u) {
+      if constexpr (YBITS) bn_bits_y<VEC>(yb[u], yv[u]);
       bn_mask<VEC, HAS_Y>(g[u], yv[HAS_Y ? u : 0], xv[u], k.sc, k.sh, act);
       if (HAS_Y && gout && r + u * step < rows) store_vec<T, VEC>(gout + (r + u * step) * c + ch0, g[u], t.cvalid);
 #pragma unroll
       for (int j = 0; j < VEC; ++j) {
         sg[j] += g[u][j];
         sgx[j] = fmaf(g[u][j], xv[u][j] - k.mu[j], sgx[j]);
+        if constexpr (PAIR) sgx2[j] = fmaf(g[u][j], x2v[u][j] - mu2[j], sgx2[j]);
         if (g_last) { g_last[u][j] = g[u][j]; xv_last[u][j] = xv[u][j]; }
       }
     }
@@ -499,6 +573,48 @@
 #pragma unroll
   for (int j = 0; j < VEC; ++j)
     if (t.ch0 + j < c) *(float2*)(part + ((long)blockIdx.x * c + t.ch0 + j) * 2) = make_float2(sg[j], sgx[j]);
+}
+
+template <typename T, int VEC, class GS, bool PAIR>
+__global__ void __launch_bounds__(256) bn_bwd_stats_bits_kernel(const GS gs, const T* __restrict__ x,
+                                                                 const uint8_t* __restrict__ bits, const float* __restrict__ gamma,
+                                                                 const float* __restrict__ beta, const float* __restrict__ mean,
+                                                                 const float* __restrict__ sinv, float* __restrict__ part,
+                                                                 long rows, int c, T* __restrict__ gout,
+                                                                 const T* __restrict__ x2, const float* __restrict__ mean2,
+                                                                 float* __restrict__ part2) {
+  __shared__ float red[2][256][VEC];
+  const BnTile<VEC> t(c);
+  BnDx<VEC> k;
+  float sg[VEC], sgx[VEC], sg2[PAIR ? VEC : 1], sgx2[PAIR ? VEC : 1], mu2[PAIR ? VEC : 1];
+#pragma unroll
+  for (int j = 0; j < VEC; ++j) { sg[j] = 0.f; sgx[j] = 0.f; }
+  if constexpr (PAIR) {
+#pragma unroll
+    for (int j = 0; j < VEC; ++j) { sgx2[j] = 0.f; mu2[j] = mean2[min(t.ch0 + j, c - 1)]; }
+  }
+  if (t.active) {
+    bn_bwd_coef<VEC>(t.ch0, c, gamma, beta, mean, sinv, k);
+    bn_bwd_sums<T, VEC, true, GS, true, PAIR>(gs, x, (const T*)nullptr, gout, t.row0(), t.step(), rows, c, t, k, RTSDS_ACT_RELU, sg,
+                                              sgx, nullptr, nullptr, bits, x2, mu2, sgx2);
+  }
+  if constexpr (PAIR) {
+#pragma unroll
+    for (int j = 0; j < VEC; ++j) sg2[j] = sg[j];
+  }
+  const bool owner = bn_bwd_block_sum<VEC>(t, red, sg, sgx);
+  if (owner) {
+#pragma unroll
+    for (int j = 0; j < VEC; ++j)
+      if (t.ch0 + j < c) *(float2*)(part + ((long)blockIdx.x * c + t.ch0 + j) * 2) = make_float2(sg[j], sgx[j]);
+  }
+  if constexpr (PAIR) {
+    __syncthreads();
+    if (!bn_bwd_block_sum<VEC>(t, red, sg2, sgx2)) return;
+#pragma unroll
+    for (int j = 0; j < VEC; ++j)
+      if (t.ch0 + j < c) *(float2*)(part2 + ((long)blockIdx.x * c + t.ch0 + j) * 2) = make_float2(sg2[j], sgx2[j]);
+  }
 }
 
 template <typename T, int VEC, bool HAS_Y, class GS, int ACT>
@@ -586,11 +702,9 @@
   bn_bwd_coef_rows(ops, sg, sgx, ch, c, rows, training, accumulate, dgamma, dbeta, coef);
 }
 
-__global__ void __launch_bounds__(256) bn_bwd_finalize_rb_kernel(const float* __restrict__ part, int nrb, int c, long rows,
-                                                                  const float* gamma, const float* beta, const float* smean,
-                                                                  const float* sinv, float* dgamma, float* dbeta, float* coef,
-                                                                  int training, int accumulate) {
-  __shared__ float wr[16][16][2];
+RT_DEV void bn_bwd_finalize_rb_body(const float* __restrict__ part, int nrb, int c, long rows, const float* gamma,
+                                    const float* beta, const float* smean, const float* sinv, float* dgamma, float* dbeta,
+                                    float* coef, int training, int accumulate, float (*wr)[16][2]) {
   const int cl = threadIdx.x & 15, q = threadIdx.x >> 4, ch = blockIdx.x * 16 + cl;
   const int chc = min(ch, c - 1);
   BnBwdOps ops;
@@ -619,6 +733,23 @@
   sg = (t0[0] + t0[1]) + (t0[2] + t0[3]);
   sgx = (t1[0] + t1[1]) + (t1[2] + t1[3]);
   bn_bwd_coef_rows(ops, sg, sgx, ch, c, rows, training, accumulate, dgamma, dbeta, coef);
+}
+__global__ void __launch_bounds__(256) bn_bwd_finalize_rb_kernel(const float* __restrict__ part, int nrb, int c, long rows,
+                                                                  const float* gamma, const float* beta, const float* smean,
+                                                                  const float* sinv, float* dgamma, float* dbeta, float* coef,
+                                                                  int training, int accumulate) {
+  __shared__ float wr[16][16][2];
+  bn_bwd_finalize_rb_body(part, nrb, c, rows, gamma, beta, smean, sinv, dgamma, dbeta, coef, training, accumulate, wr);
+}
+struct BnBwdFin {
+  const float *part, *gamma, *beta, *smean, *sinv;
+  float *dgamma, *dbeta, *coef;
+  int accumulate;
+};
+__global__ void __launch_bounds__(256) bn_bwd_finalize_pair_kernel(BnBwdFin fa, BnBwdFin fb, int nrb, int c, long rows) {
+  __shared__ float wr[16][16][2];
+  const BnBwdFin f = blockIdx.y ? fb : fa;
+  bn_bwd_finalize_rb_body(f.part, nrb, c, rows, f.gamma, f.beta, f.smean, f.sinv, f.dgamma, f.dbeta, f.coef, 1, f.accumulate, wr);
 }
 
 template <typename T, int VEC, class GS, int ACT>
@@ -664,6 +795,65 @@
     }
   }
   if (r < rows) bn_bwd_row<T, VEC>(gs, x, y, dx, dres, r, c, t, k, act);
+}
+
+template <typename T, int VEC>
+RT_DEV void bn_bwd_pair_row(T* __restrict__ dxa, T* __restrict__ dxb, long off, const BnDx<VEC>& ka, const BnDx<VEC>& kb,
+                            int cvalid, unsigned yb, float* g, float* xa, float* xb) {
+  float yv[VEC];
+  bn_bits_y<VEC>(yb, yv);
+  bn_mask<VEC, true>(g, yv, xa, ka.sc, ka.sh, RTSDS_ACT_RELU);
+#pragma unroll
+  for (int j = 0; j < VEC; ++j) {
+    xa[j] = bn_bwd_dx<VEC>(ka, j, g[j], xa[j]);
+    xb[j] = bn_bwd_dx<VEC>(kb, j, g[j], xb[j]);
+  }
+  store_vec<T, VEC>(dxa + off, xa, cvalid);
+  store_vec<T, VEC>(dxb + off, xb, cvalid);
+}
+template <int VEC>
+RT_DEV void bn_bwd_load_abk(const float* __restrict__ coef, int ch0, int c, BnDx<VEC>& k) {
+  load_coef<VEC>(coef, ch0, c, k.a);
+  load_coef<VEC>(coef + c, ch0, c, k.b);
+  load_coef<VEC>(coef + 2 * c, ch0, c, k.k);
+  load_coef<VEC>(coef + 3 * c, ch0, c, k.mu);
+}
+template <typename T, int VEC, class GS>
+__global__ void __launch_bounds__(256) bn_bwd_apply_pair_kernel(const GS gs, const uint8_t* __restrict__ bits,
+                                                                 const T* __restrict__ xa, const T* __restrict__ xb,
+                                                                 T* __restrict__ dxa, T* __restrict__ dxb,
+                                                                 const float* __restrict__ coefa, const float* __restrict__ coefb,
+                                                                 long rows, int c) {
+  const BnTile<VEC> t(c);
+  if (!t.active) return;
+  BnDx<VEC> ka, kb;
+  bn_bwd_load_abk<VEC>(coefa, t.ch0, c, ka);
+  bn_bwd_load_abk<VEC>(coefb, t.ch0, c, kb);
+  const int ch0 = t.ch0, cvalid = t.cvalid;
+  const long step = t.step(), nv = c / VEC, bv = ch0 / VEC;
+  long r = t.row0();
+  for (; r + step < rows; r += 2 * step) {
+    const long o0 = r * c + ch0, o1 = o0 + step * c;
+    float g0[VEC], a0[VEC], b0[VEC], g1[VEC], a1[VEC], b1[VEC];
+    gs.template load<VEC>(r, ch0, g0, cvalid);
+    load_vec<T, VEC>(xa + o0, a0, cvalid);
+    load_vec<T, VEC>(xb + o0, b0, cvalid);
+    const unsigned y0 = bits[r * nv + bv];
+    gs.template load<VEC>(r + step, ch0, g1, cvalid);
+    load_vec<T, VEC>(xa + o1, a1, cvalid);
+    load_vec<T, VEC>(xb + o1, b1, cvalid);
+    const unsigned y1 = bits[(r + step) * nv + bv];
+    bn_bwd_pair_row<T, VEC>(dxa, dxb, o0, ka, kb, cvalid, y0, g0, a0, b0);
+    bn_bwd_pair_row<T, VEC>(dxa, dxb, o1, ka, kb, cvalid, y1, g1, a1, b1);
+  }
+  if (r < rows) {
+    const long o0 = r * c + ch0;
+    float g0[VEC], a0[VEC], b0[VEC];
+    gs.template load<VEC>(r, ch0, g0, cvalid);
+    load_vec<T, VEC>(xa + o0, a0, cvalid);
+    load_vec<T, VEC>(xb + o0, b0, cvalid);
+    bn_bwd_pair_row<T, VEC>(dxa, dxb, o0, ka, kb, cvalid, bits[r * nv + bv], g0, a0, b0);
+  }
 }
 
 template <typename F>
@@ -759,6 +949,14 @@
 };
 
 template <typename T, int VEC>
+static const float* bn_fwd_stats(const BnArgs& a, int& rb) {
+  rb = a.pre_nrb;
+  if (a.pre) return a.pre;
+  rb = bn_rb<VEC>(a.rows, a.c);
+  hipLaunchKernelGGL((bn_stats_kernel<T, VEC>), bn_grid<VEC>(rb, a.c), dim3(256), 0, a.st, (const T*)a.x, a.w.part, a.rows, a.c);
+  return a.w.part;
+}
+template <typename T, int VEC>
 static void bn_fwd_coefs(const BnArgs& a, bool apply_too = false) {
   const int c = a.c;
   float *scale = a.w.coef, *shift = a.w.coef + c;
@@ -767,13 +965,8 @@
                        shift, a.smean, a.sinv, a.eps);
     return;
   }
-  int rb = a.pre_nrb;
-  const float* part = a.pre;
-  if (!part) {
-    rb = bn_rb<VEC>(a.rows, c);
-    hipLaunchKernelGGL((bn_stats_kernel<T, VEC>), bn_grid<VEC>(rb, c), dim3(256), 0, a.st, (const T*)a.x, a.w.part, a.rows, c);
-    part = a.w.part;
-  }
+  int rb;
+  const float* part = bn_fwd_stats<T, VEC>(a, rb);
   if (apply_too)
     hipLaunchKernelGGL(bn_finalize_apply_kernel<T>, dim3(c), dim3(256), 0, a.st, part, rb, c, a.rows, a.gamma, a.beta, a.rmean,
                        a.rvar, a.smean, a.sinv, scale, shift, a.momentum, a.eps, a.nbt, (const T*)a.x, (const T*)a.res, (T*)a.y,
@@ -935,6 +1128,140 @@
                             size_t ws_bytes, void* stream) {
   return rtsds_bn_bwd_ld(dy, c, x, y, dx, dres, dgamma, dbeta, rows, c, gamma, beta, save_mean, save_invstd, training, act,
                          accumulate_params, dtype, ws, ws_bytes, stream);
+}
+
+static bool bn_bits_ok(long rows, int c, int dtype) {
+  return rows > 0 && c > 0 && c % 8 == 0 && c <= 65535 * 256 && (dtype == RTSDS_BF16 || dtype == RTSDS_F32);
+}
+extern "C" size_t rtsds_bn_bits_bytes(long rows, int c, int dtype) {
+  if (!bn_bits_ok(rows, c, dtype)) return 0;
+  return (size_t)rows * (c / (dtype == RTSDS_BF16 ? 8 : 4));
+}
+extern "C" size_t rtsds_bn_pair_workspace(long rows, int c) { return 2 * rtsds_bn_workspace(rows, c); }
+template <typename F>
+static int bn_bits_dispatch(int dtype, F f) {
+  if (dtype == RTSDS_BF16) f(BnKind<bf16, 8>());
+  else if (dtype == RTSDS_F32) f(BnKind<float, 4>());
+  else return RTSDS_ERR_UNSUPPORTED;
+  return RTSDS_OK;
+}
+
+static int bn_params_fwd(BnArgs& a, const rtsds_bn_params* p) {
+  return bn_fwd_args(a, p->gamma, p->beta, p->running_mean, p->running_var, p->num_batches_tracked, p->save_mean, p->save_invstd,
+                     p->momentum, p->eps, 1, p->stats_part, p->stats_nrb);
+}
+template <typename T, int VEC>
+static void bn_bits_fwd_launch(const BnArgs& a, const BnArgs* b, uint8_t* bits) {
+  const int c = a.c;
+  const dim3 grid = bn_grid<VEC>(bn_apply_rb<VEC>(a.rows, c), c);
+  if (!b) {
+    bn_fwd_coefs<T, VEC>(a);
+    hipLaunchKernelGGL((bn_apply_bits_kernel<T, VEC, false>), grid, dim3(256), 0, a.st, (const T*)a.x, (const T*)a.res, (T*)a.y, bits,
+                       a.w.coef, a.w.coef + c, (const float*)nullptr, (const float*)nullptr, a.rows, c);
+    return;
+  }
+  BnFin f[2];
+  const BnArgs* ab[2] = {&a, b};
+  for (int i = 0; i < 2; ++i) {
+    const BnArgs& q = *ab[i];
+    int rb;
+    const float* part = bn_fwd_stats<T, VEC>(q, rb);
+    f[i] = BnFin{part, rb, q.gamma, q.beta, q.rmean, q.rvar, q.smean, q.sinv, q.w.coef, q.w.coef + c, q.momentum, q.eps, q.nbt};
+  }
+  hipLaunchKernelGGL(bn_finalize_pair_kernel, dim3(c, 2), dim3(256), 0, a.st, f[0], f[1], c, a.rows);
+  hipLaunchKernelGGL((bn_apply_bits_kernel<T, VEC, true>), grid, dim3(256), 0, a.st, (const T*)a.x, (const T*)b->x, (T*)a.y, bits,
+                     a.w.coef, a.w.coef + c, b->w.coef, b->w.coef + c, a.rows, c);
+}
+template <typename T, int VEC>
+static void bn_bits_bwd_launch(const BnArgs& a, const BnArgs* b, const uint8_t* bits) {
+  const T* x = (const T*)a.x;
+  const long rows = a.rows;
+  const int c = a.c;
+  const GradDirect<T> gs{(const T*)a.dy, (int)(a.ldy ? a.ldy : c)};
+  const int rb = bn_bwd_rb<VEC>(rows, c);
+  const dim3 sgrid = bn_grid<VEC>(rb, c), agrid = bn_grid<VEC>(bn_apply_rb<VEC>(rows, c), c);
+  if (!b) {
+    hipLaunchKernelGGL((bn_bwd_stats_bits_kernel<T, VEC, GradDirect<T>, false>), sgrid, dim3(256), 0, a.st, gs, x, bits, a.gamma,
+                       a.beta, a.smean, a.sinv, a.w.part, rows, c, (T*)a.dres, (const T*)nullptr, (const float*)nullptr,
+                       (float*)nullptr);
+    hipLaunchKernelGGL(bn_bwd_finalize_rb_kernel, dim3(rt_cdiv(c, 16)), dim3(256), 0, a.st, a.w.part, rb, c, rows, a.gamma, a.beta,
+                       a.smean, a.sinv, a.dgamma, a.dbeta, a.w.coef, 1, a.accumulate);
+    const GradDirect<T> gg{(const T*)a.dres, c};
+    hipLaunchKernelGGL((bn_bwd_apply_kernel<T, VEC, GradDirect<T>, RTSDS_ACT_NONE>), agrid, dim3(256), 0, a.st, gg, x,
+                       (const T*)nullptr, (T*)a.dx, (T*)nullptr, a.w.coef, rows, c, 0);
+    return;
+  }
+  hipLaunchKernelGGL((bn_bwd_stats_bits_kernel<T, VEC, GradDirect<T>, true>), sgrid, dim3(256), 0, a.st, gs, x, bits, a.gamma, a.beta,
+                     a.smean, a.sinv, a.w.part, rows, c, (T*)nullptr, (const T*)b->x, b->smean, b->w.part);
+  const BnBwdFin fa{a.w.part, a.gamma, a.beta, a.smean, a.sinv, a.dgamma, a.dbeta, a.w.coef, a.accumulate};
+  const BnBwdFin fb{b->w.part, b->gamma, b->beta, b->smean, b->sinv, b->dgamma, b->dbeta, b->w.coef, b->accumulate};
+  hipLaunchKernelGGL(bn_bwd_finalize_pair_kernel, dim3(rt_cdiv(c, 16), 2), dim3(256), 0, a.st, fa, fb, rb, c, rows);
+  hipLaunchKernelGGL((bn_bwd_apply_pair_kernel<T, VEC, GradDirect<T>>), agrid, dim3(256), 0, a.st, gs, bits, x, (const T*)b->x,
+                     (T*)a.dx, (T*)b->dx, a.w.coef, b->w.coef, rows, c);
+}
+
+extern "C" int rtsds_bn_fwd_bits(const void* x, const void* res, void* y, uint8_t* bits, long rows, int c, const float* gamma,
+                                 const float* beta, float* running_mean, float* running_var, long long* num_batches_tracked,
+                                 float* save_mean, float* save_invstd, float momentum, float eps, const float* stats_part,
+                                 int stats_nrb, int dtype, void* ws, size_t ws_bytes, void* stream) {
+  if (rows <= 0 || c <= 0 || !x || !res || !y || !bits) return RTSDS_ERR_SHAPE;
+  if (!bn_bits_ok(rows, c, dtype)) return RTSDS_ERR_UNSUPPORTED;
+  if (ws_bytes < rtsds_bn_workspace(rows, c)) return RTSDS_ERR_WORKSPACE;
+  BnArgs a(rows, c, ws, stream);
+  if (int rc = bn_fwd_args(a, gamma, beta, running_mean, running_var, num_batches_tracked, save_mean, save_invstd, momentum, eps, 1,
+                           stats_part, stats_nrb))
+    return rc;
+  a.x = x, a.res = res, a.y = y, a.ldy = c, a.act = RTSDS_ACT_RELU;
+  if (int rc = bn_bits_dispatch(dtype, [&](auto k) { bn_bits_fwd_launch<typename decltype(k)::T, decltype(k)::VEC>(a, nullptr, bits); }))
+    return rc;
+  RET_LAUNCH();
+}
+extern "C" int rtsds_bn_bwd_bits(const void* dy, long ldy, const void* x, const uint8_t* bits, void* dx, void* dres, float* dgamma,
+                                 float* dbeta, long rows, int c, const float* gamma, const float* beta, const float* save_mean,
+                                 const float* save_invstd, int accumulate_params, int dtype, void* ws, size_t ws_bytes,
+                                 void* stream) {
+  if (rows <= 0 || c <= 0 || ldy < c || ldy > (1L << 30) || !dy || !x || !bits || !dx || !dres) return RTSDS_ERR_SHAPE;
+  if (!bn_bits_ok(rows, c, dtype)) return RTSDS_ERR_UNSUPPORTED;
+  if (ldy != c && !(dtype == RTSDS_BF16 && ldy % 8 == 0)) return RTSDS_ERR_UNSUPPORTED;
+  if (ws_bytes < rtsds_bn_workspace(rows, c)) return RTSDS_ERR_WORKSPACE;
+  BnArgs a(rows, c, ws, stream);
+  bn_bwd_args(a, x, dx, dgamma, dbeta, gamma, beta, save_mean, save_invstd, 1, RTSDS_ACT_RELU, accumulate_params);
+  a.dy = dy, a.ldy = ldy, a.dres = dres;
+  if (int rc = bn_bits_dispatch(dtype, [&](auto k) { bn_bits_bwd_launch<typename decltype(k)::T, decltype(k)::VEC>(a, nullptr, bits); }))
+    return rc;
+  RET_LAUNCH();
+}
+extern "C" int rtsds_bn_pair_fwd(const void* xa, const void* xb, void* y, uint8_t* bits, long rows, int c,
+                                 const rtsds_bn_params* pa, const rtsds_bn_params* pb, int dtype, void* ws, size_t ws_bytes,
+                                 void* stream) {
+  if (rows <= 0 || c <= 0 || !xa || !xb || !y || !bits || !pa || !pb) return RTSDS_ERR_SHAPE;
+  if (!bn_bits_ok(rows, c, dtype)) return RTSDS_ERR_UNSUPPORTED;
+  if (ws_bytes < rtsds_bn_pair_workspace(rows, c)) return RTSDS_ERR_WORKSPACE;
+  BnArgs a(rows, c, ws, stream), b(rows, c, (char*)ws + rtsds_bn_workspace(rows, c), stream);
+  if (int rc = bn_params_fwd(a, pa)) return rc;
+  if (int rc = bn_params_fwd(b, pb)) return rc;
+  a.x = xa, a.y = y, a.ldy = c, a.act = RTSDS_ACT_RELU, b.x = xb;
+  if (int rc = bn_bits_dispatch(dtype, [&](auto k) { bn_bits_fwd_launch<typename decltype(k)::T, decltype(k)::VEC>(a, &b, bits); }))
+    return rc;
+  RET_LAUNCH();
+}
+extern "C" int rtsds_bn_pair_bwd(const void* dy, long ldy, const void* xa, const void* xb, const uint8_t* bits, void* dxa, void* dxb,
+                                 long rows, int c, const rtsds_bn_params* pa, const rtsds_bn_params* pb, int dtype, void* ws,
+                                 size_t ws_bytes, void* stream) {
+  if (rows <= 0 || c <= 0 || ldy < c || ldy > (1L << 30) || !dy || !xa || !xb || !bits || !dxa || !dxb || !pa || !pb)
+    return RTSDS_ERR_SHAPE;
+  if (!bn_bits_ok(rows, c, dtype)) return RTSDS_ERR_UNSUPPORTED;
+  if (ldy != c && !(dtype == RTSDS_BF16 && ldy % 8 == 0)) return RTSDS_ERR_UNSUPPORTED;
+  if (ws_bytes < rtsds_bn_pair_workspace(rows, c)) return RTSDS_ERR_WORKSPACE;
+  BnArgs a(rows, c, ws, stream), b(rows, c, (char*)ws + rtsds_bn_workspace(rows, c), stream);
+  bn_bwd_args(a, xa, dxa, pa->dgamma, pa->dbeta, pa->gamma, pa->beta, pa->save_mean, pa->save_invstd, 1, RTSDS_ACT_RELU,
+              pa->accumulate);
+  bn_bwd_args(b, xb, dxb, pb->dgamma, pb->dbeta, pb->gamma, pb->beta, pb->save_mean, pb->save_invstd, 1, RTSDS_ACT_NONE,
+              pb->accumulate);
+  a.dy = dy, a.ldy = ldy;
+  if (int rc = bn_bits_dispatch(dtype, [&](auto k) { bn_bits_bwd_launch<typename decltype(k)::T, decltype(k)::VEC>(a, &b, bits); }))
+    return rc;
+  RET_LAUNCH();
 }
 
 extern "C" int rtsds_bn_fwd_gap(const void* x, void* y, float* gap_part, int n, long hw, int c, const float* gamma, const float* beta,
diff --git a/rtsds_amd/csrc/bn_dev.h b/rtsds_amd/csrc/bn_dev.h
--- a/rtsds_amd/csrc/bn_dev.h
+++ b/rtsds_amd/csrc/bn_dev.h
@@ -41,6 +41,20 @@
   }
 }
 
+template <typename T, int VEC>
+RT_DEV unsigned bn_y_bits(const float* v) {
+  static_assert(VEC <= 8, "one byte per channel vector");
+  unsigned b = 0;
+#pragma unroll
+  for (int j = 0; j < VEC; ++j) b |= (to_f(from_f<T>(v[j])) > 0.f ? 1u : 0u) << j;
+  return b;
+}
+template <int VEC>
+RT_DEV void bn_bits_y(unsigned b, float* yv) {
+#pragma unroll
+  for (int j = 0; j < VEC; ++j) yv[j] = (b >> j) & 1u ? 1.f : 0.f;
+}
+
 template <int VEC> struct BnDx {
   float a[VEC], b[VEC], k[VEC], mu[VEC], sc[VEC], sh[VEC];
 };
diff --git a/rtsds_amd/functional.py b/rtsds_amd/functional.py
--- a/rtsds_amd/functional.py
+++ b/rtsds_amd/functional.py
@@ -3,7 +3,8 @@
 import numpy as np
 import torch
 
-from ._lib import ACT_RELU, ACT_SIGMOID, INPUT_PADDED, UPCE_SET_CORRECT, WEIGHT_PACKED, ConvDesc, SplitReduceDesc, lib
+from ._lib import (ACT_RELU, ACT_SIGMOID, INPUT_PADDED, UPCE_SET_CORRECT, WEIGHT_PACKED, BnParams, ConvDesc,
+                   SplitReduceDesc, lib)
 from .runtime import (CL, bump_params_epoch, collective, dcode, dp_world, empty_nhwc, nhwc, params_epoch,
                       register_fold, require_hip, side_enabled, side_fork, stream, workspace)
 
@@ -55,8 +56,11 @@
 
 
 def _bn_param_grads(ctx, c, device):
-    need_g, need_b = ctx.needs_input_grad[1], ctx.needs_input_grad[2]
-    sinks = _sinks(ctx.gamma if need_g else None, ctx.beta if need_b else None) if (need_g or need_b) else None
+    return _bn_grads_of(ctx.gamma, ctx.beta, ctx.needs_input_grad[1], ctx.needs_input_grad[2], c, device)
+
+
+def _bn_grads_of(gamma, beta, need_g, need_b, c, device):
+    sinks = _sinks(gamma if need_g else None, beta if need_b else None) if (need_g or need_b) else None
     if sinks is not None:
         return sinks[0], sinks[1], 1
     dg = torch.empty(c, dtype=torch.float32, device=device) if need_g else None
@@ -526,6 +530,15 @@
     ctx_link.bn = (x, coef, act)
 
 
+RES_BN_PAIR = True
+RES_BN_BITS = False
+
+
+def _res_bits_ok(x, res, training, act):
+    return (training and res is not None and act == ACT_RELU and x.shape[1] % 8 == 0
+            and x.dtype in (torch.bfloat16, torch.float32) and res.dtype == x.dtype and res.shape == x.shape)
+
+
 class BatchNormFn(torch.autograd.Function):
 
     @staticmethod
@@ -549,14 +562,23 @@
         sm = torch.empty(c, dtype=torch.float32, device=x.device)
         si = torch.empty(c, dtype=torch.float32, device=x.device)
         ws = workspace(lib.rtsds_bn_workspace(rows, c), x.device)
-        lib.rtsds_bn_fwd_ld(_P(x), _P(res), _P(y), ld, rows, c, _P(gamma), _P(beta), _P(running_mean),
-                            _P(running_var), _P(nbt), _P(sm), _P(si), float(momentum), float(eps), int(training),
-                            act, _P(stats) if training else None, int(stats_nrb or 0), dcode(x), _P(ws),
-                            ws.numel(), stream())
+        bits = None
+        if RES_BN_BITS and _res_bits_ok(x, res, training, act) and ctx.needs_input_grad[0] \
+                and ctx.needs_input_grad[3]:
+            bits = torch.empty(lib.rtsds_bn_bits_bytes(rows, c, dcode(x)), dtype=torch.uint8, device=x.device)
+            lib.rtsds_bn_fwd_bits(_P(x), _P(res), _P(y), _P(bits), rows, c, _P(gamma), _P(beta), _P(running_mean),
+                                  _P(running_var), _P(nbt), _P(sm), _P(si), float(momentum), float(eps), _P(stats),
+                                  int(stats_nrb or 0), dcode(x), _P(ws), ws.numel(), stream())
+        else:
+            lib.rtsds_bn_fwd_ld(_P(x), _P(res), _P(y), ld, rows, c, _P(gamma), _P(beta), _P(running_mean),
+                                _P(running_var), _P(nbt), _P(sm), _P(si), float(momentum), float(eps), int(training),
+                                act, _P(stats) if training else None, int(stats_nrb or 0), dcode(x), _P(ws),
+                                ws.numel(), stream())
         ctx.meta = (rows, c, int(training), act, res is not None)
         ctx.gamma, ctx.beta = gamma, beta
         ctx.res_join = res_join
-        ctx.save_for_backward(x, y if keep_y else None, gamma, beta, sm, si)
+        ctx.has_bits = bits is not None
+        ctx.save_for_backward(x, bits if bits is not None else (y if keep_y else None), gamma, beta, sm, si)
         ctx.link = None
         if link is not None and BN_BWD_LINK and training and res is None and act in (0, 1, 2) \
                 and x.dtype == torch.bfloat16 and c % 8 == 0:
@@ -585,7 +607,10 @@
         dg, db, acc = _bn_param_grads(ctx, c, x.device)
         ws = workspace(lib.rtsds_bn_workspace(rows, c), x.device)
         link = ctx.link
-        if link is not None and link.part is not None and dy.dtype == x.dtype:
+        if ctx.has_bits:
+            lib.rtsds_bn_bwd_bits(_P(dy), ldy, _P(x), _P(y), _P(dx), _P(dres), _P(dg), _P(db), rows, c, _P(gamma),
+                                  _P(beta), _P(sm), _P(si), acc, dcode(x), _P(ws), ws.numel(), stream())
+        elif link is not None and link.part is not None and dy.dtype == x.dtype:
             lib.rtsds_bn_bwd_part(_P(dy), _P(x), _P(dx), _P(dg), _P(db), rows, c, _P(gamma), _P(beta), _P(sm),
                                   _P(si), training, act, acc, _P(link.part), link.nrb, dcode(x), _P(ws), ws.numel(),
                                   stream())
@@ -647,6 +672,67 @@
         wg_link = wg_link.take(x, training and residual is None, act)
     return BatchNormFn.apply(x, gamma, beta, residual, running_mean, running_var, training,
                              momentum, eps, act, stats, nrb, num_batches_tracked, res_join, link, out, wg_link)
+
+
+class BatchNormPairFn(torch.autograd.Function):
+
+    @staticmethod
+    def forward(ctx, xa, xb, ga, ba, gb, bb, pa, pb):
+        require_hip(xa)
+        xa, xb = nhwc(xa), nhwc(xb)
+        n, c, h, w = xa.shape
+        rows = n * h * w
+        y = torch.empty_like(xa, memory_format=CL)
+        bits = torch.empty(lib.rtsds_bn_bits_bytes(rows, c, dcode(xa)), dtype=torch.uint8, device=xa.device)
+        sv = [torch.empty(c, dtype=torch.float32, device=xa.device) for _ in range(4)]
+        ws = workspace(lib.rtsds_bn_pair_workspace(rows, c), xa.device)
+        qa = BnParams(_P(ga), _P(ba), _P(pa[0]), _P(pa[1]), _P(pa[2]), _P(sv[0]), _P(sv[1]), float(pa[3]), float(pa[4]),
+                      _P(pa[5]), int(pa[6] or 0), 0, None, None)
+        qb = BnParams(_P(gb), _P(bb), _P(pb[0]), _P(pb[1]), _P(pb[2]), _P(sv[2]), _P(sv[3]), float(pb[3]), float(pb[4]),
+                      _P(pb[5]), int(pb[6] or 0), 0, None, None)
+        lib.rtsds_bn_pair_fwd(_P(xa), _P(xb), _P(y), _P(bits), rows, c, ctypes.byref(qa), ctypes.byref(qb), dcode(xa),
+                              _P(ws), ws.numel(), stream())
+        ctx.meta = (rows, c)
+        ctx.params = (ga, ba, gb, bb)
+        ctx.save_for_backward(xa, xb, bits, ga, ba, gb, bb, *sv)
+        return y
+
+    @staticmethod
+    def backward(ctx, dy):
+        xa, xb, bits, ga, ba, gb, bb, sma, sia, smb, sib = ctx.saved_tensors
+        rows, c = ctx.meta
+        ldy = _channel_slice_pitch(dy)
+        if not ldy:
+            dy = nhwc(dy)
+            ldy = c
+        need = ctx.needs_input_grad
+        dxa = torch.empty_like(xa, memory_format=CL)
+        dxb = torch.empty_like(xb, memory_format=CL)
+        dga, dba, acca = _bn_grads_of(ctx.params[0], ctx.params[1], need[2], need[3], c, xa.device)
+        dgb, dbb, accb = _bn_grads_of(ctx.params[2], ctx.params[3], need[4], need[5], c, xa.device)
+        ws = workspace(lib.rtsds_bn_pair_workspace(rows, c), xa.device)
+        qa = BnParams(_P(ga), _P(ba), None, None, None, _P(sma), _P(sia), 0.0, 0.0, None, 0, acca, _P(dga), _P(dba))
+        qb = BnParams(_P(gb), _P(bb), None, None, None, _P(smb), _P(sib), 0.0, 0.0, None, 0, accb, _P(dgb), _P(dbb))
+        lib.rtsds_bn_pair_bwd(_P(dy), ldy, _P(xa), _P(xb), _P(bits), _P(dxa), _P(dxb), rows, c, ctypes.byref(qa),
+                              ctypes.byref(qb), dcode(xa), _P(ws), ws.numel(), stream())
+        if acca:
+            dga = dba = None
+        if accb:
+            dgb = dbb = None
+        return dxa, dxb, dga, dba, dgb, dbb, None, None
+
+
+def batch_norm_pair(xa, bn_a, xb, bn_b, training, act=ACT_RELU):
+    ga, ba, rma, rva, moma, epsa, nbta = bn_a
+    gb, bb, rmb, rvb, momb, epsb, nbtb = bn_b
+    if RES_BN_PAIR and xa.dim() == 4 and _res_bits_ok(xa, xb, training, act) and torch.is_grad_enabled() \
+            and xa.requires_grad and xb.requires_grad and xa.is_cuda:
+        sa, na = _bn_epilogue_stats(xa, training, rma)
+        sb, nb = _bn_epilogue_stats(xb, training, rmb)
+        return BatchNormPairFn.apply(xa, xb, ga, ba, gb, bb, (rma, rva, nbta, moma, epsa, sa, na),
+                                     (rmb, rvb, nbtb, momb, epsb, sb, nb))
+    skip = batch_norm(xb, gb, bb, rmb, rvb, training, momb, epsb, 0, None, nbtb)
+    return batch_norm(xa, ga, ba, rma, rva, training, moma, epsa, act, skip, nbta)
 
 
 def pack_input(x, dtype):
diff --git a/rtsds_amd/models/bisenet/build_contextpath.py b/rtsds_amd/models/bisenet/build_contextpath.py
--- a/rtsds_amd/models/bisenet/build_contextpath.py
+++ b/rtsds_amd/models/bisenet/build_contextpath.py
@@ -3,7 +3,8 @@
 
 from rtsds_amd import functional as F
 from rtsds_amd.functional import BnBwdLink
-from rtsds_amd.nn import BatchNorm2d, Conv2d, MaxPool2d, ReLU, conv_bn, conv_bn_relu_maxpool, grad_join
+from rtsds_amd.nn import (BatchNorm2d, Conv2d, MaxPool2d, ReLU, conv_bn, conv_bn_relu_maxpool, downsample_branch, grad_join,
+                          res_block_tail)
 from rtsds_amd.runtime import grad_cut
 
 
@@ -22,13 +23,13 @@
 
     def forward(self, x):
         join = grad_join(x, 2)
-        skip = x
+        skip, ds_bn = x, None
         if self.downsample is not None:
-            skip = conv_bn(self.downsample[0], self.downsample[1], x, join=join)
+            skip, ds_bn = downsample_branch(self.downsample, x, join)
         link = BnBwdLink()
         t = conv_bn(self.conv1, self.bn1, x, "relu", join=join, out_link=link)
-        return conv_bn(self.conv2, self.bn2, t, "relu", skip,
-                       res_join=join if self.downsample is None else None, in_link=link)
+        return res_block_tail(self.conv2, self.bn2, t, skip, ds_bn,
+                              res_join=join if self.downsample is None else None, in_link=link)
 
 
 class Bottleneck(nn.Module):
@@ -48,14 +49,14 @@
 
     def forward(self, x):
         join = grad_join(x, 2)
-        skip = x
+        skip, ds_bn = x, None
         if self.downsample is not None:
-            skip = conv_bn(self.downsample[0], self.downsample[1], x, join=join)
+            skip, ds_bn = downsample_branch(self.downsample, x, join)
         l1, l2 = BnBwdLink(), BnBwdLink()
         t = conv_bn(self.conv1, self.bn1, x, "relu", join=join, out_link=l1)
         t = conv_bn(self.conv2, self.bn2, t, "relu", in_link=l1, out_link=l2)
-        return conv_bn(self.conv3, self.bn3, t, "relu", skip,
-                       res_join=join if self.downsample is None else None, in_link=l2)
+        return res_block_tail(self.conv3, self.bn3, t, skip, ds_bn,
+                              res_join=join if self.downsample is None else None, in_link=l2)
 
 
 class ResNet(nn.Module):
diff --git a/rtsds_amd/models/deeplabv2/deeplabv2.py b/rtsds_amd/models/deeplabv2/deeplabv2.py
--- a/rtsds_amd/models/deeplabv2/deeplabv2.py
+++ b/rtsds_amd/models/deeplabv2/deeplabv2.py
@@ -3,7 +3,8 @@
 
 from rtsds_amd import functional as F
 from rtsds_amd.functional import BnBwdLink
-from rtsds_amd.nn import BatchNorm2d, Conv2d, MaxPool2d, ReLU, conv_bn, conv_bn_relu_maxpool, grad_join, to_input
+from rtsds_amd.nn import (BatchNorm2d, Conv2d, MaxPool2d, ReLU, conv_bn, conv_bn_relu_maxpool, downsample_branch, grad_join,
+                          res_block_tail, to_input)
 from rtsds_amd.nn import _shadow
 from rtsds_amd.runtime import grad_cut
 
@@ -34,12 +35,12 @@
 
     def forward(self, x):
         join = grad_join(x, 2)
-        skip = x if self.downsample is None else conv_bn(self.downsample[0], self.downsample[1], x, join=join)
+        skip, ds_bn = (x, None) if self.downsample is None else downsample_branch(self.downsample, x, join)
         l1, l2 = BnBwdLink(), BnBwdLink()
         t = conv_bn(self.conv1, self.bn1, x, "relu", join=join, out_link=l1)
         t = conv_bn(self.conv2, self.bn2, t, "relu", in_link=l1, out_link=l2)
-        return conv_bn(self.conv3, self.bn3, t, "relu", skip,
-                       res_join=join if self.downsample is None else None, in_link=l2)
+        return res_block_tail(self.conv3, self.bn3, t, skip, ds_bn,
+                              res_join=join if self.downsample is None else None, in_link=l2)
 
 
 class ClassifierModule(nn.Module):
diff --git a/rtsds_amd/nn.py b/rtsds_amd/nn.py
--- a/rtsds_amd/nn.py
+++ b/rtsds_amd/nn.py
@@ -130,6 +130,36 @@
               res_join=res_join, link=out_link, out=out, wg_link=wg)
 
 
+def _bn_pair_args(bn):
+    track = bn.track_running_stats
+    return (bn.weight, bn.bias, bn.running_mean if track else None, bn.running_var if track else None, bn.momentum,
+            bn.eps, bn.num_batches_tracked if (bn.training and track) else None)
+
+
+def _bn_pair_ok(conv, bn, x):
+    return (F.RES_BN_PAIR and (bn.training or not bn.track_running_stats) and bn.momentum is not None
+            and torch.is_grad_enabled() and (x.requires_grad or conv.weight.requires_grad)
+            and conv.out_channels % 8 == 0 and conv.in_channels != 3 and x.dtype in (torch.bfloat16, torch.float32))
+
+
+def downsample_branch(ds, x, join):
+    conv, bn = ds[0], ds[1]
+    if len(ds) == 2 and _bn_pair_ok(conv, bn, x):
+        return conv(x, bn_stats=True, join=join), bn
+    return conv_bn(conv, bn, x, join=join), None
+
+
+def res_block_tail(conv, bn, t, skip, ds_bn=None, res_join=None, in_link=None):
+    if ds_bn is None:
+        return conv_bn(conv, bn, t, "relu", skip, res_join=res_join, in_link=in_link)
+    if not _bn_pair_ok(conv, bn, t):
+        return conv_bn(conv, bn, t, "relu", ds_bn(skip), in_link=in_link)
+    xa = conv(t, bn_stats=True, bn_link=in_link)
+    if xa.shape[0] * xa.shape[2] * xa.shape[3] == 1:
+        raise ValueError(f"Expected more than 1 value per channel when training, got input size {tuple(xa.shape)}")
+    return F.batch_norm_pair(xa, _bn_pair_args(bn), skip, _bn_pair_args(ds_bn), True)
+
+
 def conv_bn_relu_maxpool(conv, bn, pool, x):
     use_batch = bn.training or not bn.track_running_stats
     k = pool.kernel_size if isinstance(pool.kernel_size, int) else pool.kernel_size[0]
```

Result: faster. 1872 images/s, median of 6 (+1.7%).
